# Tejasvanvekar/Sparse-optimal-control-of-Viscous-Chan-hilliard-via-Gradient-descent--1D-2D

Hardware: AMD Instinct MI355X
Metric: PGD iterations/sec (fwd Newton + adjoint + prox), 2D 512^2 grid (higher is better)
Workload: dtype f64; 1 GPU; 2D 512x512, 1000 time steps, batch 8 trajectories per GPU (8 total), seeds 42+i, targets build_targets 1/1, u0 = 0; grid=512, batch_per_gpu=8, contexts_per_gpu=2, parallelism=batch-shard x1, collective=cabi-rccl

## Files before the change

### sparse-optimal-control-of-viscous-chan-hilliard-via-gradient-descent--1d-2d_amd/csrc/vch_engine2d.hip

```cpp
#include "vch_common.h"
#include "vch_kernels2d.h"
#include "vch_gemm.h"
#include "vch_fft.h"
#include <algorithm>
#include <atomic>
#include <chrono>
#include <cmath>

thread_local char g_vch_err[512] = "";

extern "C" const char *vch_last_error(void) { return g_vch_err; }
extern "C" int vch_abi_version(void) { return 3; }
extern "C" int vch_device_count(void) {
    int n = 0;
    if (hipGetDeviceCount(&n) != hipSuccess) return -1;
    return n;
}

constexpr int J_RING = 64;

struct GuessPolicy {
    static constexpr int PROBE_EVERY = 8;
    int order, probe, since, next_dir;
    bool climbing;
    double r_base;
    void reset() { order = 1; probe = 0; since = 0; next_dir = 1; climbing = true; r_base = 1e300; }
    int choose(int avail, int cap) const { return std::max(0, std::min(std::min(order + probe, cap), avail)); }
    void report(double r, int used, int cap) {
        if (used < 1) return;
        if (climbing) {
            if (r > 0.7) {
                order = std::max(1, used - 1);
                r_base = 1e300;
                if (used > 1) climbing = false;
                return;
            }
            if (r_base < 1e299 && r > 0.5 * r_base) {
                order = std::max(1, used - 1);
                climbing = false;
                return;
            }
            r_base = r;
            order = used;
            if (used >= cap) climbing = false;
            else order = used + 1;
            return;
        }
        if (probe == 0) {
            r_base = r;
            if (r > 0.7 && order > 1) { --order; since = 0; return; }
            if (++since >= PROBE_EVERY) {
                since = 0;
                probe = next_dir;
                next_dir = -next_dir;
                if (order + probe < 1 || order + probe > cap) probe = 0;
            }
            return;
        }
        if (probe > 0 ? r < 0.5 * r_base : r <= r_base) order = used;
        probe = 0;
    }
};

struct vch2d_ctx {
    vch2d_params prm;
    int B, Mmax, device;
    Geom G;
    Phys P;
    double hx, hy;
    hipStream_t stream;
    hipEvent_t ev0, ev1;
    dim3 grid;
    int nblk;
    long slot_stride;
    double *phi_s, *mu_s, *Rphi_s, *rhs_s, *D_s;
    double *w, *wnew, *mu0, *cphi, *cmu, *x, *r, *dmu, *t1, *t2;
    double *cg_p[2], *cg_v, *cg_q;
    double *cg_z2;
    double *xf;
    int cg_last;
    bool cheb_on;
    int spec_form[4];
    bool debug_guess;
    bool adj_guess_off, adj_safe;
    long redo_iters;
    bool fused_on;
    int fused_mode;
    unsigned *fin_counter;
    int cheb_enq, spec_chn[4], cheb_margin, cheb_max;
    double pgd_adj_tol;
    double eta1_factor;
    double cg_scale_ratio;
    double *dprev[GUESS_RING], *x0g;
    bool guess_on;
    int guess_wr, guess_step;
    int guess_max;
    std::vector<GuessPolicy> pol1, pol2;
    std::vector<int> used1, used2, run2;
    GuessPolicy pol1_all, pol2_all;
    int run2_all;
    GuessArgs gtab1, gtab2;
    unsigned gmask1, gmask2;
    double *dprev2[GUESS_RING];
    bool guess2_on;
    double *gpart2;
    double *gpart3;
    double *gpart;
    int gnblk;
    double *tmp[6];
    double *wts_mass, *W_cost;
    double *part;
    double *part_mass;
    bool post_fold;
    bool post_pending;
    double *post_hist;
    TrajState *st, *st_host;
    TrajState *st_pub;
    unsigned long long *seq_pub, seq_next;
    bool look_spin;
    int *frozen_dev;
    double *hist_dev, *hist_host;
    double *Q1f, *Q2f, *Q1s, *Q2s, *mf, *ms;
    bool use_fft;
    int cols_c;
    FftAxis fax, sax;
    FftAxis fax_h, sax_h;
    double2 *tw_fh = nullptr, *tw_sh = nullptr;
    bool half_f = false, half_s = false;
    double2 *tw_f, *tw_s;
    double *phi_hist, *u_hist, *u_trial, *phi_trial, *phiQ, *r_hist, *p_hist, *q_hist;
    double *phiT, *phi0;
    double *cost_part, *cost_lvl;
    double *cost_lvl_host;
    double *alpha_dev;
    int M_res;
    int u_rows_res;
    bool pgd_ready;
    bool ramp;
    double rampT;
    std::vector<double> t_hist, dt, xg, yg, tfrac;
    double *tfrac_dev;
    vch_opt_params opt;
    std::vector<double> pgd_cost, pgd_alpha_prev, pgd_J;
    std::vector<int> pgd_plateau, pgd_done, pgd_k;
    std::vector<std::vector<double>> pgd_cost_hist;
    std::vector<double> pgd_denQ2, pgd_denT2, pgd_trk, pgd_trm;
    double pgd_rms;
    int pgd_err_n;
    double *J_dev;
    double *J_ring_dev, *J_ring_host;
    std::atomic<long> pgd_iter_total;
    long tot_launch, tot_sync;
    bool prof_on;
    std::vector<hipEvent_t> prof_ev;
    std::vector<int> prof_cls;
    size_t prof_used;
    int lin_maxit;
    double lin_tol;
    double lin_eta;
    bool spec;
    int spec_slots, spec_cgb[4];
    long n_launch, n_sync;
};

enum { PC_SCHUR_P = 0, PC_GEMM = 1, PC_RESIDUAL = 2, PC_ADJ_Q = 3, PC_CG_UPDATE = 4, PC_ADJ_RHS = 5, PC_COST = 6,
       PC_PROX = 7, PC_DCT_R0 = 8, PC_DCT_C = 9, PC_DCT_R3 = 10, PC_SCHUR_P1 = 11, PC_CG_ROWS = 12, PC_CG_ROWS1 = 13,
       PC_NOOP = 14, PC_GUESS = 15, PC_ADJ_GUESS = 16, PC_CHEB_ROWS = 17, PC_CHEB_ROWS0 = 18, PC_RESIDUAL0 = 19,
       PC_NCLS = 20 };

__global__ void k_noop() {}

static bool launch_begin(vch2d_ctx *c, int cls) {
    const bool rec = cls >= 0 && c->prof_on && c->prof_used + 2 <= c->prof_ev.size();
    if (rec) hipEventRecord(c->prof_ev[c->prof_used], c->stream);
    return rec;
}
static void launch_end(vch2d_ctx *c, int cls, bool rec) {
    c->n_launch++;
    if (rec) {
        hipEventRecord(c->prof_ev[c->prof_used + 1], c->stream);
        c->prof_cls.push_back(cls);
        c->prof_used += 2;
    }
}
#define LAUNCHC(cls, kern, grid, block, ...) LAUNCH_LDS(cls, kern, grid, block, 0, __VA_ARGS__)

static int dalloc(double **p, size_t n, hipStream_t s) {
    *p = nullptr;
    HIPCHK(hipMalloc((void **)p, n * sizeof(double)));
    HIPCHK(hipMemsetAsync(*p, 0, n * sizeof(double), s));
    return 0;
}

static int h2d(vch2d_ctx *c, double *dev, const double *host, long nplanes) {
    HIPCHK(hipMemcpy2DAsync(dev, (size_t)c->G.pitch * 8, host, (size_t)c->G.nf * 8, (size_t)c->G.nf * 8,
                            (size_t)c->G.ns * nplanes, hipMemcpyHostToDevice, c->stream));
    return 0;
}
static int d2h(vch2d_ctx *c, double *host, const double *dev, long nplanes) {
    HIPCHK(hipMemcpy2DAsync(host, (size_t)c->G.nf * 8, dev, (size_t)c->G.pitch * 8, (size_t)c->G.nf * 8,
                            (size_t)c->G.ns * nplanes, hipMemcpyDeviceToHost, c->stream));
    HIPCHK(hipStreamSynchronize(c->stream));
    return 0;
}
static int h2d_hist(vch2d_ctx *c, double *dev, const double *host, int rows) {
    const long hs = (long)(c->Mmax + 1) * c->G.plane;
    for (int b = 0; b < c->B; ++b)
        VCHCHK(h2d(c, dev + b * hs, host + (long)b * rows * c->G.nf * c->G.ns, rows));
    return 0;
}
static int d2h_hist(vch2d_ctx *c, double *host, const double *dev, int rows) {
    const long hs = (long)(c->Mmax + 1) * c->G.plane;
    for (int b = 0; b < c->B; ++b) {
        HIPCHK(hipMemcpy2DAsync(host + (long)b * rows * c->G.nf * c->G.ns, (size_t)c->G.nf * 8, dev + b * hs,
                                (size_t)c->G.pitch * 8, (size_t)c->G.nf * 8, (size_t)c->G.ns * rows,
                                hipMemcpyDeviceToHost, c->stream));
    }
    HIPCHK(hipStreamSynchronize(c->stream));
    return 0;
}
static int ensure_hist(vch2d_ctx *c, double **p) {
    if (*p) return 0;
    size_t n = (size_t)c->B * (c->Mmax + 1) * c->G.plane;
    hipError_t e = hipMalloc((void **)p, n * sizeof(double));
    if (e != hipSuccess) {
        *p = nullptr;
        return vch_fail(VCH_ERR_NOMEM, "hipMalloc of a %.2f GB history failed: %s", n * 8e-9, hipGetErrorString(e));
    }
    HIPCHK(hipMemsetAsync(*p, 0, n * sizeof(double), c->stream));
    return 0;
}
static inline long hist_stride(const vch2d_ctx *c) { return (long)(c->Mmax + 1) * c->G.plane; }

__global__ void k_publish_state(const unsigned *__restrict__ st, int nwords, unsigned *__restrict__ dst,
                                unsigned long long *seq, unsigned long long val) {
    for (int i = threadIdx.x; i < nwords; i += blockDim.x) dst[i] = st[i];
    __threadfence_system();
    __syncthreads();
    if (threadIdx.x == 0) __hip_atomic_store(seq, val, __ATOMIC_RELEASE, __HIP_MEMORY_SCOPE_SYSTEM);
}

static int sync_state(vch2d_ctx *c, bool full = true) {
    c->n_sync++;
    if (full || !c->look_spin) {
        HIPCHK(hipMemcpyAsync(c->st_host, c->st, sizeof(TrajState) * c->B, hipMemcpyDeviceToHost, c->stream));
        HIPCHK(hipStreamSynchronize(c->stream));
        return 0;
    }
    const unsigned long long want = ++c->seq_next;
    static_assert(sizeof(TrajState) % 4 == 0, "TrajState is copied in 32-bit words");
    hipLaunchKernelGGL(k_publish_state, dim3(1), dim3(256), 0, c->stream, (const unsigned *)c->st,
                       (int)(sizeof(TrajState) / 4 * c->B), (unsigned *)c->st_pub, c->seq_pub, want);
    HIPCHK(hipGetLastError());
    const auto t0 = std::chrono::steady_clock::now();
    for (unsigned spins = 1; __atomic_load_n(c->seq_pub, __ATOMIC_ACQUIRE) != want; ++spins) {
        __builtin_ia32_pause();
        if ((spins & 0x3fff) == 0) {
            const hipError_t q = hipStreamQuery(c->stream);
            if (q != hipSuccess && q != hipErrorNotReady) return vch_fail(VCH_ERR_HIP, "sync_state: %s", hipGetErrorString(q));
            if (q == hipSuccess && __atomic_load_n(c->seq_pub, __ATOMIC_ACQUIRE) != want)
                return vch_fail(VCH_ERR_STATE, "sync_state: stream drained but the state was not published");
            if (std::chrono::steady_clock::now() - t0 > std::chrono::seconds(120))
                return vch_fail(VCH_ERR_STATE, "sync_state: no state from the device after 120 s");
        }
    }
    memcpy(c->st_host, c->st_pub, sizeof(TrajState) * c->B);
    return 0;
}

static void dct_tables(int N, double h, std::vector<double> &Q1, std::vector<double> &Q2, std::vector<double> &m) {
    const int n = N + 1;
    Q1.assign((size_t)n * n, 0.0);
    Q2.assign((size_t)n * n, 0.0);
    m.assign(n, 0.0);
    const long double pi = 3.14159265358979323846264338327950288L;
    const long double sc = sqrtl(2.0L / N), is2 = 1.0L / sqrtl(2.0L);
    for (int j = 0; j < n; ++j) {
        long double sj = (j == 0 || j == N) ? is2 : 1.0L;
        for (int k = 0; k < n; ++k) {
            long double sk = (k == 0 || k == N) ? is2 : 1.0L;
            long long jk = ((long long)j * k) % (2LL * N);
            long double cv = cosl(pi * (long double)jk / (long double)N);
            Q1[(size_t)j * n + k] = (double)(sc * sj * sj * sk * cv);
            Q2[(size_t)j * n + k] = (double)(sc * sj * cv);
        }
        m[j] = (double)((2.0L - 2.0L * cosl(pi * j / (long double)N)) / ((long double)h * h));
    }
}

extern "C" vch2d_ctx *vch2d_create(const vch2d_params *p, int batch, int max_steps, int device) {
    if (!p || p->Nx < 2 || p->Ny < 2 || batch < 1 || max_steps < 1 || !(p->Lx > 0) || !(p->Ly > 0)) {
        vch_fail(VCH_ERR_ARG, "vch2d_create: bad arguments (Nx,Ny >= 2, batch >= 1, max_steps >= 1)");
        return nullptr;
    }
    if (hipSetDevice(device) != hipSuccess) {
        (void)hipGetLastError();
        vch_fail(VCH_ERR_HIP, "hipSetDevice(%d) failed", device);
        return nullptr;
    }
    vch2d_ctx *c = new vch2d_ctx();
    c->prm = *p;
    c->B = batch;
    c->Mmax = max_steps;
    c->device = device;
    c->hx = p->Lx / p->Nx;
    c->hy = p->Ly / p->Ny;
    Geom &G = c->G;
    G.nf = p->Nx + 1;
    G.ns = p->Ny + 1;
    G.pitch = (G.nf + 7) / 8 * 8;
    G.plane = (long)G.ns * G.pitch;
    G.tiles_f = (G.nf + TX - 1) / TX;
    G.tiles_s = (G.ns + TY - 1) / TY;
    G.ax = 1.0 / (c->hx * c->hx);
    G.ay = 1.0 / (c->hy * c->hy);
    c->P = Phys{p->tau, p->gamma, p->c1, p->c2, p->kappa, p->Lx * p->Ly};
    c->grid = dim3(G.tiles_f, G.tiles_s, batch);
    c->nblk = G.tiles_f * G.tiles_s;
    c->slot_stride = (long)batch * G.plane;
    c->M_res = -1;
    c->u_rows_res = 0;
    c->pgd_ready = false;
    c->prof_on = false;
    c->prof_used = 0;
    c->lin_maxit = 4000;
    c->lin_tol = 1e-15;
    if (const char *e = getenv("VCH_LIN_TOL")) c->lin_tol = atof(e);
    c->lin_eta = 0.05 * NEWTON_TOL;
    if (const char *e = getenv("VCH_LIN_ETA")) c->lin_eta = atof(e);
    c->cols_c = 1024;
    if (const char *e = getenv("VCH_COLS_C")) c->cols_c = atoi(e);
    c->spec = getenv("VCH_NO_SPEC") == nullptr;
    c->spec_slots = 2;
    for (int &n : c->spec_cgb) n = 12;
    c->cheb_on = !(getenv("VCH_CHEB") && atoi(getenv("VCH_CHEB")) == 0);
    for (int &f : c->spec_form) f = 3;
    c->debug_guess = getenv("VCH_DEBUG_GUESS") != nullptr;
    c->adj_guess_off = c->adj_safe = false;
    c->redo_iters = 0;
    c->cheb_enq = -1;
    c->fused_mode = getenv("VCH_FUSED") ? atoi(getenv("VCH_FUSED")) : 2;
    c->fused_on = c->fused_mode != 0;
    c->post_fold = true;
    if (const char *e = getenv("VCH_POST_FOLD")) c->post_fold = atoi(e) != 0;
    c->post_pending = false;
    c->post_hist = nullptr;
    c->fin_counter = nullptr;
    for (int &n : c->spec_chn) n = 2;
    c->cheb_margin = 1;
    if (const char *e = getenv("VCH_CHEB_MARGIN")) c->cheb_margin = std::max(0, atoi(e));
    c->cheb_max = 6;
    if (const char *e = getenv("VCH_CHEB_MAX")) c->cheb_max = std::max(0, atoi(e));
    c->pgd_adj_tol = 1e-12;
    if (const char *e = getenv("VCH_ADJ_TOL")) c->pgd_adj_tol = atof(e);
    c->eta1_factor = 1e-2;
    if (const char *e = getenv("VCH_ETA1")) c->eta1_factor = atof(e);
    c->cg_scale_ratio = 4.0;
    if (const char *e = getenv("VCH_CG_SCALE")) c->cg_scale_ratio = atof(e);
    c->n_launch = c->n_sync = 0;
    auto fail = [&](const char *what) {
        vch_fail(VCH_ERR_HIP, "vch2d_create: %s failed: %s", what, hipGetErrorString(hipGetLastError()));
        return (vch2d_ctx *)nullptr;
    };
    if (hipStreamCreate(&c->stream) != hipSuccess) return fail("hipStreamCreate");
    hipEventCreate(&c->ev0);
    hipEventCreate(&c->ev1);
    const size_t bp = (size_t)batch * G.plane;
    double **two[] = {&c->phi_s, &c->mu_s, &c->Rphi_s, &c->rhs_s, &c->D_s};
    for (auto q : two)
        if (dalloc(q, 2 * bp, c->stream)) return fail("hipMalloc");
    double **one[] = {&c->w, &c->wnew, &c->mu0, &c->cphi, &c->cmu, &c->x, &c->r, &c->dmu, &c->t1, &c->t2,
                      &c->cg_p[0], &c->cg_p[1], &c->cg_v, &c->cg_q, &c->cg_z2, &c->xf, &c->dprev[0], &c->dprev[1], &c->dprev[2], &c->dprev[3], &c->dprev[4], &c->dprev[5], &c->dprev[6], &c->dprev[7], &c->dprev2[0], &c->dprev2[1], &c->dprev2[2], &c->dprev2[3], &c->dprev2[4], &c->dprev2[5], &c->dprev2[6], &c->dprev2[7], &c->x0g, &c->tmp[0], &c->tmp[1], &c->tmp[2], &c->tmp[3], &c->tmp[4], &c->tmp[5], &c->phiT, &c->phi0};
    for (auto q : one)
        if (dalloc(q, bp, c->stream)) return fail("hipMalloc");
    if (dalloc(&c->wts_mass, G.plane, c->stream) || dalloc(&c->W_cost, G.plane, c->stream)) return fail("hipMalloc");
    if (dalloc(&c->part, (size_t)batch * c->nblk * NPART, c->stream)) return fail("hipMalloc");
    if (dalloc(&c->part_mass, (size_t)batch * c->nblk * NPART, c->stream)) return fail("hipMalloc");
    c->gnblk = ((G.nf + GN - 1) / GN) * ((G.ns + GM - 1) / GM);
    if (dalloc(&c->gpart, 2 * (size_t)batch * (c->gnblk + G.ns), c->stream)) return fail("hipMalloc");
    c->gpart2 = c->gpart + (size_t)batch * (c->gnblk + G.ns);
    if (dalloc(&c->gpart3, 4 * (size_t)batch * (c->gnblk + G.ns), c->stream)) return fail("hipMalloc");
    if (dalloc(&c->hist_dev, (size_t)batch * HIST_CAP, c->stream)) return fail("hipMalloc");
    if (dalloc(&c->alpha_dev, batch, c->stream) || dalloc(&c->J_dev, 5 * (size_t)batch, c->stream)) return fail("hipMalloc");
    if (dalloc(&c->J_ring_dev, (size_t)J_RING * 5 * batch, c->stream)) return fail("hipMalloc");
    if (hipHostMalloc((void **)&c->J_ring_host, sizeof(double) * J_RING * 5 * batch) != hipSuccess) return fail("hipHostMalloc");
    c->pgd_iter_total = 0;
    c->tot_launch = c->tot_sync = 0;
    if (hipMalloc((void **)&c->st, sizeof(TrajState) * batch) != hipSuccess) return fail("hipMalloc");
    hipMemsetAsync(c->st, 0, sizeof(TrajState) * batch, c->stream);
    if (hipMalloc((void **)&c->frozen_dev, sizeof(int) * batch) != hipSuccess) return fail("hipMalloc");
    if (hipMalloc((void **)&c->fin_counter, sizeof(unsigned) * batch) != hipSuccess) return fail("hipMalloc");
    hipMemsetAsync(c->fin_counter, 0, sizeof(unsigned) * batch, c->stream);
    if (hipHostMalloc((void **)&c->st_host, sizeof(TrajState) * batch) != hipSuccess) return fail("hipHostMalloc");
    c->st_pub = nullptr;
    c->seq_pub = nullptr;
    c->seq_next = 0;
    c->look_spin = !(getenv("VCH_LOOK_SPIN") && atoi(getenv("VCH_LOOK_SPIN")) == 0);
    if (c->look_spin) {
        if (hipHostMalloc((void **)&c->st_pub, sizeof(TrajState) * batch, hipHostMallocMapped | hipHostMallocCoherent) != hipSuccess ||
            hipHostMalloc((void **)&c->seq_pub, 64, hipHostMallocMapped | hipHostMallocCoherent) != hipSuccess) {
            (void)hipGetLastError();
            if (c->st_pub) hipHostFree(c->st_pub);
            c->st_pub = nullptr;
            c->seq_pub = nullptr;
            c->look_spin = false;
        } else {
            *c->seq_pub = 0;
        }
    }
    if (hipHostMalloc((void **)&c->hist_host, sizeof(double) * batch * HIST_CAP) != hipSuccess) return fail("hipHostMalloc");
    c->phi_hist = c->u_hist = c->u_trial = c->phi_trial = c->phiQ = c->r_hist = c->p_hist = c->q_hist = nullptr;
    c->cost_part = c->cost_lvl = nullptr;
    c->cost_lvl_host = nullptr;
    c->tfrac_dev = nullptr;
    {
        std::vector<double> wm((size_t)G.plane, 0.0);
        const int nx1 = p->Nx + 1, ny1 = p->Ny + 1;
        for (int i = 0; i < nx1; ++i)
            for (int j = 0; j < ny1; ++j) {
                long f = (long)i * ny1 + j;
                double wi = (i == 0 || i == nx1 - 1) ? 0.5 : 1.0, wj = (j == 0 || j == ny1 - 1) ? 0.5 : 1.0;
                wm[(f / G.nf) * G.pitch + (f % G.nf)] = c->hx * c->hy * (wi * wj);
            }
        if (hipMemcpy(c->wts_mass, wm.data(), wm.size() * 8, hipMemcpyHostToDevice) != hipSuccess) return fail("hipMemcpy");
    }
    {
        std::vector<double> Q1, Q2, m;
        auto up = [&](double **d, const std::vector<double> &v) {
            if (hipMalloc((void **)d, v.size() * 8) != hipSuccess) return false;
            return hipMemcpy(*d, v.data(), v.size() * 8, hipMemcpyHostToDevice) == hipSuccess;
        };
        dct_tables(p->Nx, c->hx, Q1, Q2, m);
        if (!up(&c->Q1f, Q1) || !up(&c->Q2f, Q2) || !up(&c->mf, m)) return fail("DCT table upload");
        dct_tables(p->Ny, c->hy, Q1, Q2, m);
        if (!up(&c->Q1s, Q1) || !up(&c->Q2s, Q2) || !up(&c->ms, m)) return fail("DCT table upload");
    }
    {
        auto pow2 = [](int n) { return n >= 16 && n <= 2048 && (n & (n - 1)) == 0; };
        c->use_fft = pow2(p->Nx) && pow2(p->Ny) && getenv("VCH_FORCE_GEMM_DCT") == nullptr;
        c->tw_f = c->tw_s = nullptr;
        if (c->use_fft) {
            auto mk = [&](int N, double2 **tw, FftAxis &ax) {
                const int L = 2 * N;
                std::vector<double2> t(L);
                const long double pi = 3.14159265358979323846264338327950288L;
                for (int m = 0; m < L; ++m) {
                    long double a = -2.0L * pi * m / L;
                    t[m] = make_double2((double)cosl(a), (double)sinl(a));
                }
                if (hipMalloc((void **)tw, sizeof(double2) * L) != hipSuccess) return false;
                if (hipMemcpy(*tw, t.data(), sizeof(double2) * L, hipMemcpyHostToDevice) != hipSuccess) return false;
                int lg = 0;
                while ((1 << lg) < L) ++lg;
                ax = FftAxis{N, L, lg, *tw};
                return true;
            };
            if (!mk(p->Nx, &c->tw_f, c->fax) || !mk(p->Ny, &c->tw_s, c->sax)) return fail("FFT twiddle upload");
            const bool want_half = getenv("VCH_DCT_HALF") != nullptr;
            if (want_half && p->Nx == HN) {
                if (!mk(HN / 2, &c->tw_fh, c->fax_h)) return fail("FFT twiddle upload");
                c->half_f = true;
            }
            if (want_half && p->Ny == HN) {
                if (!mk(HN / 2, &c->tw_sh, c->sax_h)) return fail("FFT twiddle upload");
                c->half_s = true;
            }
            if (c->half_f) {
                c->gnblk = (G.ns + 3) / 4;
            } else {
                const int Cc = c->fax.L <= 1024 ? 1024 : c->fax.L;
                const int rpw = 2 * (Cc >> c->fax.logL);
                c->gnblk = (G.ns + rpw - 1) / rpw;
            }
        }
    }
    c->guess_on = c->use_fft && !c->half_f && !c->half_s && !(getenv("VCH_GUESS") && atoi(getenv("VCH_GUESS")) == 0);
    memset(&c->gtab1, 0, sizeof(c->gtab1));
    memset(&c->gtab2, 0, sizeof(c->gtab2));
    c->gmask1 = c->gmask2 = 0;
    c->pol1.resize(batch);
    c->pol2.resize(batch);
    c->used1.assign(batch, 0);
    c->used2.assign(batch, 0);
    c->run2.assign(batch, 0);
    c->run2_all = 0;
    c->guess2_on = !(getenv("VCH_GUESS2") && atoi(getenv("VCH_GUESS2")) == 0);
    c->guess_wr = -1;
    c->guess_step = 0;
    c->guess_max = 6;
    if (const char *e = getenv("VCH_GUESS_MAX")) c->guess_max = std::max(1, std::min(GUESS_ORD, atoi(e)));
    if (hipStreamSynchronize(c->stream) != hipSuccess) return fail("hipStreamSynchronize");
    return c;
}

extern "C" void vch2d_destroy(vch2d_ctx *c) {
    if (!c) return;
    hipSetDevice(c->device);
    hipStreamSynchronize(c->stream);
    double *all[] = {c->phi_s, c->mu_s, c->Rphi_s, c->rhs_s, c->D_s, c->w, c->wnew, c->mu0, c->cphi, c->cmu, c->x,
                     c->r, c->dmu, c->t1, c->t2, c->cg_p[0], c->cg_p[1], c->cg_v, c->cg_q, c->cg_z2, c->xf, c->dprev[0], c->dprev[1], c->dprev[2], c->dprev[3], c->dprev[4], c->dprev[5], c->dprev[6], c->dprev[7], c->dprev2[0], c->dprev2[1], c->dprev2[2], c->dprev2[3], c->dprev2[4], c->dprev2[5], c->dprev2[6], c->dprev2[7], c->x0g, c->gpart, c->gpart3, c->tmp[0], c->tmp[1], c->tmp[2], c->tmp[3], c->tmp[4], c->tmp[5],
                     c->phiT, c->phi0, c->wts_mass, c->W_cost, c->part, c->part_mass, c->hist_dev, c->alpha_dev, c->J_dev, c->Q1f,
                     c->Q2f, c->Q1s, c->Q2s, c->mf, c->ms, c->phi_hist, c->u_hist, c->u_trial, c->phi_trial, c->phiQ,
                     c->r_hist, c->p_hist, c->q_hist, c->cost_part, c->cost_lvl, c->tfrac_dev};
    for (double *q : all)
        if (q) hipFree(q);
    hipFree(c->st);
    hipFree(c->frozen_dev);
    if (c->fin_counter) hipFree(c->fin_counter);
    if (c->tw_fh) hipFree(c->tw_fh);
    if (c->tw_sh) hipFree(c->tw_sh);
    if (c->tw_f) hipFree(c->tw_f);
    if (c->tw_s) hipFree(c->tw_s);
    hipHostFree(c->st_host);
    if (c->st_pub) hipHostFree(c->st_pub);
    if (c->seq_pub) hipHostFree(c->seq_pub);
    hipHostFree(c->hist_host);
    hipHostFree(c->J_ring_host);
    hipFree(c->J_ring_dev);
    if (c->cost_lvl_host) hipHostFree(c->cost_lvl_host);
    for (hipEvent_t e : c->prof_ev) hipEventDestroy(e);
    hipEventDestroy(c->ev0);
    hipEventDestroy(c->ev1);
    hipStreamDestroy(c->stream);
    delete c;
}

extern "C" int vch2d_batch(const vch2d_ctx *c) { return c ? c->B : VCH_ERR_ARG; }

template <class F>
static int with_plan(const FftAxis &ax, F &&f) {
    using std::integral_constant;
    if (ax.logL == 10) return f(integral_constant<int, 1024>(), integral_constant<int, 10>());
    if (ax.logL == 9) return f(integral_constant<int, 1024>(), integral_constant<int, 9>());
    if (ax.logL < 10) return f(integral_constant<int, 1024>(), integral_constant<int, 0>());
    if (ax.logL == 11) return f(integral_constant<int, 2048>(), integral_constant<int, 11>());
    return f(integral_constant<int, 4096>(), integral_constant<int, 0>());
}

template <int EPI>
static int dct_rows(vch2d_ctx *c, const double *in, long in_slot_stride, double *out, const SpecArgs &sp, int gate) {
    return with_plan(c->fax, [&](auto C, auto LG) {
        const int rpw = 2 * (C >> c->fax.logL);
        LAUNCHC(EPI >= 3 ? PC_DCT_R3 : PC_DCT_R0, (k_dct_rows<EPI, C, LG>), dim3((c->G.ns + rpw - 1) / rpw, 1, c->B),
                dim3(FftThreads<C, LG>::T), c->G, c->fax, in, in_slot_stride, out, 1.0, sp, c->st, gate);
        return 0;
    });
}

template <int C, int LOGL>
static int dct_cols_plan(vch2d_ctx *c, const SpecArgs &sp, double scale, int gate) {
    const int cpw = 2 * (C >> c->sax.logL);
    LAUNCHC(PC_DCT_C, (k_dct_cols<C, LOGL>), dim3((c->G.nf + cpw - 1) / cpw, 1, c->B), dim3(FftThreads<C, LOGL>::T), c->G,
            c->sax, (const double *)c->t1, c->t2, scale, sp, c->st, gate);
    return 0;
}
static int dct_cols(vch2d_ctx *c, const SpecArgs &sp, double scale, int gate) {
    const int wide = c->sax.logL == 10 ? c->cols_c : 0;
    if (wide == 4096) return dct_cols_plan<4096, 10>(c, sp, scale, gate);
    if (wide == 2048) return dct_cols_plan<2048, 10>(c, sp, scale, gate);
    return with_plan(c->sax, [&](auto C, auto LG) { return dct_cols_plan<C, LG>(c, sp, scale, gate); });
}

static int cg_rows(vch2d_ctx *c, const CgSweepArgs &a, bool first) {
    return with_plan(c->fax, [&](auto C, auto LG) {
        const int rpw = 2 * (C >> c->fax.logL);
        auto k_rows = first ? k_cg_rows_fwd<1, C, LG> : k_cg_rows_fwd<0, C, LG>;
        LAUNCHC(first ? PC_CG_ROWS1 : PC_CG_ROWS, k_rows, dim3((c->G.ns + rpw - 1) / rpw, 1, c->B), dim3(FftThreads<C, LG>::T),
                c->G, c->fax, a, c->t1, c->st);
        return 0;
    });
}

static int cheb_rows(vch2d_ctx *c, const ChebSweepArgs &a, bool first) {
    return with_plan(c->fax, [&](auto C, auto LG) {
        const int rpw = 2 * (C >> c->fax.logL);
        auto k_rows = first ? k_cheb_rows<C, LG, 1> : k_cheb_rows<C, LG, 0>;
        LAUNCHC(first ? PC_CHEB_ROWS0 : PC_CHEB_ROWS, k_rows, dim3((c->G.ns + rpw - 1) / rpw, 1, c->B), dim3(FftThreads<C, LG>::T),
                c->G, c->fax, a, (const double *)c->t2, c->t1, (const TrajState *)c->st);
        return 0;
    });
}

static int adj_rows(vch2d_ctx *c, const AdjSweepArgs &a, bool first) {
    return with_plan(c->fax, [&](auto C, auto LG) {
        const int rpw = 2 * (C >> c->fax.logL);
        auto k_rows = first ? k_adj_rows_fwd<1, C, LG> : k_adj_rows_fwd<0, C, LG>;
        LAUNCHC(PC_ADJ_Q, k_rows, dim3((c->G.ns + rpw - 1) / rpw, 1, c->B), dim3(FftThreads<C, LG>::T), c->G, c->fax, a, c->t1,
                c->st);
        return 0;
    });
}

static int precond(vch2d_ctx *c, const double *in, long in_slot_stride, double *out, int last, const double *other,
                   double c0, double c1a, double c1b, double c2, int gate) {
    const Geom &G = c->G;
// ... 1445 lines not shown
```

### sparse-optimal-control-of-viscous-chan-hilliard-via-gradient-descent--1d-2d_amd/csrc/vch_fft.h

```cpp
#pragma once
#include "vch_common.h"
#include "vch_kernels2d.h"
#include "vch_gemm.h"

struct FftAxis {
    int N, L, logL;
    const double2 *tw;
};


__device__ __forceinline__ double2 cmul(double2 a, double2 b) {
    return make_double2(a.x * b.x - a.y * b.y, a.x * b.y + a.y * b.x);
}

struct SpecArgs;
template <class SP>
__device__ __forceinline__ void spec_mult2(const SP &sp, double c1, double scale, double ma, double mb, double &fa, double &fb,
                                           int mode) {
    const double pa = sp.c0 + ma * (c1 + sp.c2 * ma), pb = sp.c0 + mb * (c1 + sp.c2 * mb);
    const double na = scale * (mode == 2 ? -(sp.c0 + sp.c2 * ma * ma) : (mode ? ma : 1.0));
    const double nb = scale * (mode == 2 ? -(sp.c0 + sp.c2 * mb * mb) : (mode ? mb : 1.0));
    const double d = pa * pb;
    double r = __builtin_amdgcn_rcp(d);
    r = fma(fma(-d, r, 1.0), r, r);
// ... 76 lines not shown
            for (int h = 0; h < 2; ++h) {
                const double2 *v = h ? cc : bb;
                const double2 t0 = make_double2(v[0].x + v[2].x, v[0].y + v[2].y), t1 = make_double2(v[0].x - v[2].x, v[0].y - v[2].y);
                const double2 t2 = make_double2(v[1].x + v[3].x, v[1].y + v[3].y);
                const double2 t3 = make_double2(v[1].y - v[3].y, -(v[1].x - v[3].x));
                o[h + 0] = make_double2(t0.x + t2.x, t0.y + t2.y);
                o[h + 2] = make_double2(t1.x + t3.x, t1.y + t3.y);
                o[h + 4] = make_double2(t0.x - t2.x, t0.y - t2.y);
                o[h + 6] = make_double2(t1.x - t3.x, t1.y - t3.y);
            }
            const int wb = fb + ((j >> lNs) << (lNs + 3)) + k;
            if (REGMODE == 1 && 3 * (ps + 1) == LOGL) {
#pragma unroll
                for (int r = 0; r < 8; ++r) xr[r] = o[r];
            } else if (EMIT && 3 * (ps + 1) == LOGL) {
                if (Emit::TO_LDS) __syncthreads();
#pragma unroll
                for (int r = 0; r < 8; ++r) emit(wb + r * Ns, o[r]);
                if (Emit::TO_LDS) __syncthreads();
            } else {
                if (!(INGEST && ps == 0)) __syncthreads();
#pragma unroll
                for (int r = 0; r < 8; ++r) buf[swz<LOGL>(wb + r * Ns)] = o[r];
                __syncthreads();
            }
        }
        logNs = 3 * NR8;
    }
    const int logQ = logL - 2, Q = L >> 2;
#pragma unroll
    for (; logNs + 2 <= logL; logNs += 2) {
        const int Ns = 1 << logNs;
        double2 v[NB4][4];
        int wbase[NB4];
        const bool shared_tw = Ns <= T;
        double2 w1 = make_double2(1.0, 0.0), w2 = w1, w3 = w1;
        if (logNs > 0 && shared_tw) {
            const int ti = (tid & (Ns - 1)) << (logL - logNs - 2);
            w1 = ax.tw[ti];
            w2 = ax.tw[2 * ti];
            w3 = ax.tw[3 * ti];
        }
#pragma unroll
        for (int i = 0; i < NB4; ++i) {
            const int idx = tid + i * T;
            const int f = idx >> logQ, j = idx & (Q - 1), k = j & (Ns - 1);
            const int fb = f * L;
            double2 a = buf[swz<LOGL>(fb + j)], b = buf[swz<LOGL>(fb + j + Q)], c = buf[swz<LOGL>(fb + j + 2 * Q)],
                    d = buf[swz<LOGL>(fb + j + 3 * Q)];
            if (logNs > 0) {
                if (!shared_tw) {
                    const int ti = k << (logL - logNs - 2);
                    w1 = ax.tw[ti];
                    w2 = ax.tw[2 * ti];
                    w3 = ax.tw[3 * ti];
                }
                b = cmul(b, w1);
                c = cmul(c, w2);
                d = cmul(d, w3);
            }
            double2 t0 = make_double2(a.x + c.x, a.y + c.y), t1 = make_double2(a.x - c.x, a.y - c.y);
            double2 t2 = make_double2(b.x + d.x, b.y + d.y);
            double2 t3 = make_double2(b.y - d.y, -(b.x - d.x));
            v[i][0] = make_double2(t0.x + t2.x, t0.y + t2.y);
            v[i][1] = make_double2(t1.x + t3.x, t1.y + t3.y);
            v[i][2] = make_double2(t0.x - t2.x, t0.y - t2.y);
            v[i][3] = make_double2(t1.x - t3.x, t1.y - t3.y);
            wbase[i] = f * L + ((j >> logNs) << (logNs + 2)) + k;
        }
        if (REGMODE == 1 && logNs + 2 == logL) {
            static_assert(REGMODE != 1 || LOGL == 9 || NB4 == 2, "two radix-4 butterflies per thread");
#pragma unroll
            for (int i = 0; i < NB4; ++i)
#pragma unroll
                for (int r = 0; r < 4; ++r) xr[(i + 2 * r) & 7] = v[i][r];
        } else if (EMIT && logNs + 2 == logL) {
            if (Emit::TO_LDS) __syncthreads();
#pragma unroll
            for (int i = 0; i < NB4; ++i)
#pragma unroll
                for (int r = 0; r < 4; ++r) emit(wbase[i] + r * Ns, v[i][r]);
            if (Emit::TO_LDS) __syncthreads();
        } else {
            __syncthreads();
#pragma unroll
            for (int i = 0; i < NB4; ++i)
#pragma unroll
                for (int r = 0; r < 4; ++r) buf[swz<LOGL>(wbase[i] + r * Ns)] = v[i][r];
            __syncthreads();
        }
    }
    if (logNs < logL) {
        const int Ns = 1 << logNs, H = L >> 1, logH = logL - 1;
        double2 v[NB2][2];
        int wbase[NB2];
#pragma unroll
        for (int i = 0; i < NB2; ++i) {
            const int idx = tid + i * T;
            const int f = idx >> logH, j = idx & (H - 1), k = j & (Ns - 1);
            const int fb = f * L;
            double2 a = buf[swz<LOGL>(fb + j)], b = cmul(buf[swz<LOGL>(fb + j + H)], ax.tw[k << (logL - logNs - 1)]);
            v[i][0] = make_double2(a.x + b.x, a.y + b.y);
            v[i][1] = make_double2(a.x - b.x, a.y - b.y);
            wbase[i] = f * L + ((j >> logNs) << (logNs + 1)) + k;
        }
        __syncthreads();
#pragma unroll
        for (int i = 0; i < NB2; ++i) {
            buf[swz<LOGL>(wbase[i])] = v[i][0];
            buf[swz<LOGL>(wbase[i] + Ns)] = v[i][1];
        }
        __syncthreads();
    }
}

template <int EPI, int C, int LOGL>
__global__ __launch_bounds__((FftThreads<C, LOGL>::T)) void k_dct_rows(Geom G, FftAxis ax, const double *__restrict__ in,
                                                  long in_slot_stride, double *__restrict__ out, double scale,
                                                  SpecArgs sp, const TrajState *__restrict__ st, int gate) {
    const int b = blockIdx.z;
    if (gate && !gate_open(st[b], gate)) return;
    __shared__ double2 buf[C];
    constexpr int T = FftThreads<C, LOGL>::T;
    const int tid = threadIdx.x;
    const int logL = LOGL ? LOGL : ax.logL, L = 1 << logL, N = L >> 1, nfft = C >> logL;
    const int row0 = blockIdx.x * 2 * nfft;
    const double *ib = in + b * G.plane + (in_slot_stride ? st[b].slot * in_slot_stride : 0);
    const int n1 = N + 1;
    const float inv_n1 = 1.0f / (float)n1;
    constexpr bool DIRECT = LOGL >= 9 && LOGL <= 11;
    if (!DIRECT) {
        for (int idx = tid; idx < nfft * n1; idx += T) {
            const int f = nfft == 1 ? 0 : (int)(((float)idx + 0.5f) * inv_n1), j = idx - f * n1;
            const int ra = row0 + 2 * f, rb = ra + 1;
            double2 v = make_double2(ra < G.ns ? ib[(long)ra * G.pitch + j] : 0.0,
                                     rb < G.ns ? ib[(long)rb * G.pitch + j] : 0.0);
            buf[swz<LOGL>(f * L + j)] = v;
            if (j > 0 && j < N) buf[swz<LOGL>(f * L + L - j)] = v;
        }
        __syncthreads();
    }
    double dot = 0.0, dot2 = 0.0, dbar = 0.0;
    const double *Dp = nullptr, *Ob = nullptr;
    int scaled = 0;
    if (EPI >= 3) {
        dbar = st[b].dbar;
        scaled = (EPI != 5) ? st[b].scaled : 0;
        Dp = sp.Dslot + st[b].slot * sp.d_slot_stride + b * G.plane;
        Ob = sp.other ? sp.other + b * G.plane : nullptr;
    }
    double *ob = out + b * G.plane;
    auto put = [&](int row, int k, double e) {
        double v = scale * e;
        const long o = (long)row * G.pitch + k;
        if (EPI == 4) v += Ob[o];
        if (EPI == 5) {
            const double dl = Dp[o] - dbar, pv = Ob[o];
            v = pv + sp.epi_c * dl * v;
            ob[o] = v;
            const double wd = wdev(row, k, G) / dl;
            dot += wd * (pv * v);
            dot2 += wd * (v * v);
            return;
        }
        ob[o] = v;
        if (EPI >= 3) {
            const double wd = wdev(row, k, G) * cg_weight(Dp[o], dbar, scaled);
            dot += wd * ((Ob ? Ob[o] : v) * v);
            dot2 += wd * (v * v);
        }
    };
    if (DIRECT) {
        struct RowEmit {
            enum { ACTIVE = 1, TO_LDS = 0 };
            decltype(put) &put_;
            int row0_, ns_;
            __device__ __forceinline__ void operator()(int idx, double2 v) const {
                constexpr int LL = 1 << (LOGL ? LOGL : 1);
                const int f = idx >> (LOGL ? LOGL : 1), k = idx & (LL - 1);
                if (k <= LL / 2) {
                    const int ra = row0_ + 2 * f;
                    if (ra < ns_) put_(ra, k, v.x);
                    if (ra + 1 < ns_) put_(ra + 1, k, v.y);
                }
            }
        };
        struct RowIngest {
            enum { ACTIVE = 1 };
            const double *ib_;
            long pitch_;
            int row0_, ns_;
            __device__ __forceinline__ double2 operator()(int idx) const {
                constexpr int LL = 1 << (LOGL ? LOGL : 1);
                const int f = idx >> (LOGL ? LOGL : 1), i = idx & (LL - 1), m = i <= LL / 2 ? i : LL - i;
                const int ra = row0_ + 2 * f;
                const double *p = ib_ + (long)ra * pitch_ + m;
                return make_double2(ra < ns_ ? p[0] : 0.0, ra + 1 < ns_ ? p[pitch_] : 0.0);
            }
        };
        fft_lds<C, LOGL>(buf, ax, RowEmit{put, row0, G.ns}, RowIngest{ib, (long)G.pitch, row0, G.ns});
    } else {
        fft_lds<C, LOGL>(buf, ax);
        for (int idx = tid; idx < 2 * nfft * n1; idx += T) {
            const int rr = nfft == 1 ? (idx >= n1 ? 1 : 0) : (int)(((float)idx + 0.5f) * inv_n1), k = idx - rr * n1;
            const int row = row0 + rr;
            if (row < G.ns) {
                const double2 c = buf[swz<LOGL>((rr >> 1) * L + k)];
                put(row, k, (rr & 1) ? c.y : c.x);
            }
        }
    }
    if (EPI >= 3) {
        dot = wave_sum(dot);
        dot2 = wave_sum(dot2);
        __syncthreads();
        double *sred = reinterpret_cast<double *>(buf);
        if ((tid & 63) == 0) {
            sred[tid >> 6] = dot;
            sred[T / 64 + (tid >> 6)] = dot2;
        }
        __syncthreads();
        if (tid == 0) {
            double tot = 0.0, tot2 = 0.0;
            for (int w = 0; w < T / 64; ++w) {
                tot += sred[w];
                tot2 += sred[T / 64 + w];
            }
            sp.gpart[(long)b * gridDim.x + blockIdx.x] = tot;
            sp.gpart2[(long)b * gridDim.x + blockIdx.x] = tot2;
        }
    }
}

struct CgSweepArgs {
    const double *z, *q, *p_old;
    double *x, *z_new, *p_new;
    const double *Dslot;
    long d_slot_stride;
    const double *gpart, *gpart2;
    double *gpart3;
    int it, maxit, nbatch;
    const double *x0;
};

template <int T>
__device__ __forceinline__ void cg_sums3(const double *__restrict__ g1, const double *__restrict__ g2,
                                         const double *__restrict__ g3, int n, int b, double *s3) {
    const int wv = threadIdx.x >> 6, lane = threadIdx.x & 63;
    for (int k = wv; k < 3; k += T / 64) {
        const double *src = k == 0 ? g1 : (k == 1 ? g2 : g3);
        double a = 0.0;
        if (src)
            for (int t = lane; t < n; t += 64) a += src[(long)b * n + t];
        a = wave_sum(a);
        if (lane == 0) s3[k] = a;
    }
    __syncthreads();
}

struct FinSolveArgs {
    const double *gpart, *gpart2, *gpart3_rd;
    int gnblk, direct, rd, maxit;
    const double *p_last;
    int cheb_enq;
};
__global__ __launch_bounds__(NTH) void k_dmu_ceiling_fin(Geom G, Phys P, TrajState *__restrict__ st, long slot_stride,
                                                         const double *__restrict__ x, FinSolveArgs f,
                                                         const double *__restrict__ phi_s, const double *__restrict__ D_s,
                                                         const double *__restrict__ Rphi_s, double *__restrict__ dmu,
                                                         double *__restrict__ x_out, double *__restrict__ part,
                                                         double *__restrict__ x_keep, double *__restrict__ x_keep2) {
    TILE_COORDS;
    if (!st[b].newton_active || st[b].need_trial) return;
    if (st[b].use_cheb) return;
    __shared__ double sx[(TY + 2) * (TX + 2)];
    __shared__ double sred[NPART * 4];
    __shared__ double s3[3];
    double *const keepp = st[b].iters == 1 ? x_keep : (st[b].iters == 2 ? x_keep2 : nullptr);
    const bool keep = keepp != nullptr;
    constexpr int W = TX + 2;
    const long pb = b * G.plane;
    const int slot = st[b].slot;
    double alpha = 0.0;
    if (f.cheb_enq >= 0) {
        if (st[b].lin_active && st[b].cheb_n > f.cheb_enq) return;
    } else if (st[b].lin_active) {
        if (!st[b].ci_active[f.rd]) {
            if (blk == 0 && threadIdx.x == 0) st[b].ci_active[f.rd ^ 1] = 0;
        } else {
            const double gamma0 = st[b].cg_gamma0, gamma_old = st[b].ci_gamma[f.rd], tol = st[b].lin_reltol;
            const int it_old = st[b].ci_it[f.rd];
            cg_sums3<NTH>(f.gpart, f.gpart2, f.direct ? f.gpart3_rd : nullptr, f.gnblk, b, s3);
            const CgNext n = cg_next(s3[0], s3[1], f.direct ? s3[2] : gamma_old, gamma0, it_old, tol, f.maxit);
            if (blk == 0 && threadIdx.x == 0) cg_record(st[b], n, f.rd ^ 1);
            alpha = n.breakdown ? 0.0 : n.alpha;
        }
    }
    if (alpha != 0.0) load_tile_axpy<1>(sx, x + pb, f.p_last + pb, alpha, G, c0, r0);
    else load_tile<1>(sx, x + pb, G, c0, r0);
    if (st[b].scaled) {
        __syncthreads();
        const double dbar = st[b].dbar;
        const double *Dp = D_s + slot * slot_stride + pb;
        for (int e = threadIdx.x; e < W * (TY + 2); e += NTH) {
            int ly = e / W, lxx = e - ly * W;
            int gr = refl(r0 - 1 + ly, G.ns), gc = refl(c0 - 1 + lxx, G.nf);
            sx[e] *= dbar / Dp[(long)gr * G.pitch + gc];
        }
    }
    __syncthreads();
    double acc[1] = {1e300};
    for (int k = 0; k < TY / 4; ++k) {
        int ly = ly0 + 4 * k, r = r0 + ly, c = c0 + lx;
        if (r < G.ns && c < G.nf) {
            int p = (ly + 1) * W + lx + 1;
            long o = pb + (long)r * G.pitch + c, os = slot * slot_stride + o;
            double d = sx[p];
            x_out[o] = d;
            if (keep) keepp[o] = d;
            dmu[o] = 2.0 * ((-0.5 * P.kappa * lap_at<W>(sx, p, G.ax, G.ay) + D_s[os] * d) + Rphi_s[os]);
            double ph = phi_s[os];
            if (d > 0.0) acc[0] = fmin(acc[0], (1.0 - DELTA_SEP - ph) / d);
            else if (d < 0.0) acc[0] = fmin(acc[0], (-1.0 + DELTA_SEP - ph) / d);
        }
    }
    const int op[1] = {1};
    block_reduce_store<1>(acc, op, sred, part + ((long)b * nblk + blk) * NPART);
}

template <int FIRST, int C, int LOGL>
__global__ __launch_bounds__((FftThreads<C, LOGL>::T)) void k_cg_rows_fwd(Geom G, FftAxis ax, CgSweepArgs a, double *__restrict__ out,
                                                                         TrajState *__restrict__ st) {
    const int b = blockIdx.z;
    __shared__ double2 buf[C];
    __shared__ double s3[4];
    constexpr int T = FftThreads<C, LOGL>::T;
    const int tid = threadIdx.x;
    const int logL = LOGL ? LOGL : ax.logL, L = 1 << logL, N = L >> 1, nfft = C >> logL;
    const int row0 = blockIdx.x * 2 * nfft, n1 = N + 1;
    const int rd = (a.it + 1) & 1, wr = a.it & 1;
    const long pb = b * G.plane;
    double alpha = 0.0, beta = 0.0;
    if (FIRST) {
        const int active = st[b].lin_active && !st[b].use_cheb;
        if (blockIdx.x == 0 && tid < 64) {
            double g = 0.0;
            if (active)
                for (int t = tid; t < (int)gridDim.x; t += 64) g += a.gpart[(long)b * gridDim.x + t];
            g = wave_sum(g);
            if (tid == 0) {
                TrajState &S = st[b];
                S.cg_pending = 0;
                if (!active) {
                    S.ci_active[0] = 0;
                } else {
                    S.cg_gamma = S.cg_gamma0 = g;
                    S.cg_beta = 0.0;
                    S.lin_it = 0;
                    S.lin_rel = 1.0;
                    S.ci_active[0] = 1;
                    S.ci_it[0] = 0;
                    S.ci_gamma[0] = g;
                }
            }
        }
        if (!active) return;
    } else {
        if (!st[b].ci_active[rd]) {
            if (blockIdx.x == 0 && tid == 0) {
                st[b].ci_active[wr] = 0;
                st[b].ci_it[wr] = st[b].ci_it[rd];
                st[b].ci_gamma[wr] = st[b].ci_gamma[rd];
            }
            return;
        }
        const double gamma0 = st[b].cg_gamma0, gamma_old = st[b].ci_gamma[rd], tol = st[b].lin_reltol;
        const int it_old = st[b].ci_it[rd], n = gridDim.x;
        cg_sums3<T>(a.gpart, a.gpart2, a.it >= 2 ? a.gpart3 + (long)rd * a.nbatch * n : nullptr, n, b, s3);
        const CgNext nx = cg_next(s3[0], s3[1], a.it >= 2 ? s3[2] : gamma_old, gamma0, it_old, tol, a.maxit);
        if (blockIdx.x == 0 && tid == 0) cg_record(st[b], nx, wr);
        alpha = nx.alpha;
        beta = nx.beta;
        if (!nx.active) {
            if (!nx.breakdown)
                for (int idx = tid; idx < 2 * nfft * n1; idx += T) {
                    const int rr = idx / n1, k = idx - rr * n1, row = row0 + rr;
                    if (row < G.ns) {
                        const long o = pb + (long)row * G.pitch + k;
                        a.x[o] += alpha * a.p_old[o];
                    }
                }
            return;
        }
    }
    const double dbar = st[b].dbar;
    const int scaled = st[b].scaled;
    const double *Dp = a.Dslot + st[b].slot * a.d_slot_stride + pb;
    const bool primed = FIRST && a.x0 && st[b].x_primed;
    double acc = 0.0;
    auto node = [&](int row, int m, bool owner) -> double {
        if (row >= G.ns) return 0.0;
        const long o = (long)row * G.pitch + m;
        const double dl = cg_weight(Dp[o], dbar, scaled);
        double pn;
        if (FIRST) {
            pn = a.z[pb + o];
            if (owner) {
                a.x[pb + o] = primed ? (scaled ? a.x0[pb + o] * (Dp[o] / dbar) : a.x0[pb + o]) : 0.0;
                a.p_new[pb + o] = pn;
            }
        } else {
            const double po = a.p_old[pb + o];
            const double zn = a.z[pb + o] - alpha * a.q[pb + o];
            pn = zn + beta * po;
            if (owner) {
                a.x[pb + o] += alpha * po;
                a.z_new[pb + o] = zn;
                a.p_new[pb + o] = pn;
                acc += wdev(row, m, G) * dl * (zn * zn);
            }
        }
        return dl * pn;
    };
    double *ob = out + pb;
    auto put = [&](int row, int k, double e) { ob[(long)row * G.pitch + k] = e; };
    constexpr bool DIRECT = LOGL >= 9 && LOGL <= 11;
    if (DIRECT) {
        struct Emit {
            enum { ACTIVE = 1, TO_LDS = 0 };
            decltype(put) &put_;
            int row0_, ns_;
            __device__ __forceinline__ void operator()(int idx, double2 v) const {
                constexpr int LL = 1 << (LOGL ? LOGL : 1);
                const int f = idx >> (LOGL ? LOGL : 1), k = idx & (LL - 1);
                if (k <= LL / 2) {
                    const int ra = row0_ + 2 * f;
                    if (ra < ns_) put_(ra, k, v.x);
                    if (ra + 1 < ns_) put_(ra + 1, k, v.y);
                }
            }
        };
        for (int idx = tid; idx < nfft * n1; idx += T) {
            const int f = nfft == 1 ? 0 : idx / n1, j = idx - f * n1;
            const int ra = row0 + 2 * f;
            const double2 v = make_double2(node(ra, j, true), node(ra + 1, j, true));
            buf[swz<LOGL>(f * L + j)] = v;
            if (j > 0 && j < N) buf[swz<LOGL>(f * L + L - j)] = v;
        }
        __syncthreads();
        fft_lds<C, LOGL>(buf, ax, Emit{put, row0, G.ns});
    } else {
        const float inv_n1 = 1.0f / (float)n1;
        for (int idx = tid; idx < nfft * n1; idx += T) {
            const int f = nfft == 1 ? 0 : (int)(((float)idx + 0.5f) * inv_n1), j = idx - f * n1;
            const int ra = row0 + 2 * f;
            const double2 v = make_double2(node(ra, j, true), node(ra + 1, j, true));
            buf[swz<LOGL>(f * L + j)] = v;
            if (j > 0 && j < N) buf[swz<LOGL>(f * L + L - j)] = v;
        }
        __syncthreads();
        fft_lds<C, LOGL>(buf, ax);
        for (int idx = tid; idx < 2 * nfft * n1; idx += T) {
            const int rr = nfft == 1 ? (idx >= n1 ? 1 : 0) : (int)(((float)idx + 0.5f) * inv_n1), k = idx - rr * n1;
            const int row = row0 + rr;
            if (row < G.ns) {
                const double2 c = buf[swz<LOGL>((rr >> 1) * L + k)];
                put(row, k, (rr & 1) ? c.y : c.x);
            }
        }
    }
    if (!FIRST) {
        acc = wave_sum(acc);
        __syncthreads();
        double *sred = reinterpret_cast<double *>(buf);
        if ((tid & 63) == 0) sred[tid >> 6] = acc;
        __syncthreads();
        if (tid == 0) {
            double tot = 0.0;
            for (int w = 0; w < T / 64; ++w) tot += sred[w];
            a.gpart3[((long)wr * a.nbatch + b) * gridDim.x + blockIdx.x] = tot;
        }
    }
}

struct ChebSweepArgs {
    const double *bt_in;
    double *bt_out;
    const double *y_cur, *y_prev;
    double *y_new;
    double *x_out;
    const double *x0;
    const double *Dslot;
    long d_slot_stride;
    double *gpart;
    int j;
    double scale;
    const double *phi_s;
    double *cmin;
    double *keep1, *keep2;
};

#ifndef CHEB_MINW
#define CHEB_MINW 1
#endif
template <int C, int LOGL, int FIRST>
__global__ __launch_bounds__((FftThreads<C, LOGL>::T), CHEB_MINW) void k_cheb_rows(Geom G, FftAxis ax, ChebSweepArgs a_, const double *__restrict__ in,
                                                                       double *__restrict__ out, const TrajState *__restrict__ st) {
    const int b = blockIdx.z;
    ChebSweepArgs a = a_;
    if (FIRST) a.j = 0;
    if (!st[b].lin_active || !st[b].use_cheb || a.j > st[b].cheb_n) return;
    const bool last = a.j == st[b].cheb_n;
    __shared__ double2 buf[C];
    constexpr int T = FftThreads<C, LOGL>::T;
    const int tid = threadIdx.x;
    const int logL = LOGL ? LOGL : ax.logL, L = 1 << logL, N = L >> 1, nfft = C >> logL;
    const int row0 = blockIdx.x * 2 * nfft, n1 = N + 1;
    const long pb = b * G.plane;
    const double theta = st[b].cheb_theta, delta = st[b].cheb_delta;
    double cj = 0.0, ej = 1.0 / theta;
    {
        double rho_prev = delta / theta;
        for (int i = 1; i <= a.j; ++i) {
            ej = 2.0 / (2.0 * theta - delta * rho_prev);
            const double rho = 0.5 * delta * ej;
            cj = rho * rho_prev;
            rho_prev = rho;
        }
    }
    const double dbar = st[b].dbar;
    const double *Dp = a.Dslot + st[b].slot * a.d_slot_stride + pb;
    const bool primed = a.x0 && st[b].x_primed;
    const bool need_norm = !(last && a.j == 0);
    double acc = 0.0, cmin = 1e300;
    const double *php = a.phi_s + st[b].slot * a.d_slot_stride + pb;
    double *const keepp = st[b].iters == 1 ? a.keep1 : (st[b].iters == 2 ? a.keep2 : nullptr);
    auto upd = [&](int row, int k, double g) -> double {
        const long o = (long)row * G.pitch + k;
        const double gg = a.scale * g;
        double z, yn, dl = 0.0;
        if (need_norm || !last) dl = Dp[o] - dbar;
        if (a.j == 0) {
            z = gg;
            yn = ej * z;
            if (!last) a.bt_out[pb + o] = gg;
        } else {
            const double yc = a.y_cur[pb + o], yp = a.j >= 2 ? a.y_prev[pb + o] : 0.0;
            z = a.bt_in[pb + o] - yc - gg;
            yn = yc + cj * (yc - yp) + ej * z;
        }
        if (need_norm) acc += wdev(row, k, G) * dl * (z * z);
        if (last) {
            const double d = primed ? a.x0[pb + o] + yn : yn, ph = php[o];
            a.x_out[pb + o] = d;
            if (keepp) keepp[pb + o] = d;
            if (d > 0.0) cmin = fmin(cmin, (1.0 - DELTA_SEP - ph) / d);
            else if (d < 0.0) cmin = fmin(cmin, (-1.0 + DELTA_SEP - ph) / d);
        } else {
            a.y_new[pb + o] = yn;
        }
        return dl * yn;
    };
    const double *ib = in + pb;
    double *ob = out + pb;
    auto put = [&](int row, int k, double e) { ob[(long)row * G.pitch + k] = e; };
    constexpr bool DIRECT = LOGL >= 9 && LOGL <= 11;
    if (DIRECT) {
        constexpr int LL = 1 << (LOGL ? LOGL : 1), LG = LOGL ? LOGL : 1;
        struct RowIngest {
            enum { ACTIVE = 1 };
            const double *ib_;
            long pitch_;
            int row0_, ns_;
            __device__ __forceinline__ double2 operator()(int idx) const {
                const int f = idx >> LG, i = idx & (LL - 1), m = i <= LL / 2 ? i : LL - i;
                const int ra = row0_ + 2 * f;
                const double *p = ib_ + (long)ra * pitch_ + m;
                return make_double2(ra < ns_ ? p[0] : 0.0, ra + 1 < ns_ ? p[pitch_] : 0.0);
            }
        };
        struct UpdEmit {
            enum { ACTIVE = 1, TO_LDS = 1 };
            decltype(upd) &upd_;
            double2 *buf_;
            int row0_, ns_;
            bool last_;
            __device__ __forceinline__ void operator()(int idx, double2 v) const {
                const int f = idx >> LG, k = idx & (LL - 1);
                if (k > LL / 2) return;
                const int ra = row0_ + 2 * f;
                double2 w = make_double2(0.0, 0.0);
                if (ra < ns_) w.x = upd_(ra, k, v.x);
                if (ra + 1 < ns_) w.y = upd_(ra + 1, k, v.y);
                if (!last_) {
                    buf_[swz<LOGL>(idx)] = w;
                    if (k > 0 && k < LL / 2) buf_[swz<LOGL>(f * LL + LL - k)] = w;
                }
            }
        };
        struct RowEmit {
            enum { ACTIVE = 1, TO_LDS = 0 };
            decltype(put) &put_;
            int row0_, ns_;
            __device__ __forceinline__ void operator()(int idx, double2 v) const {
                const int f = idx >> LG, k = idx & (LL - 1);
                if (k <= LL / 2) {
                    const int ra = row0_ + 2 * f;
                    if (ra < ns_) put_(ra, k, v.x);
                    if (ra + 1 < ns_) put_(ra + 1, k, v.y);
                }
            }
// ... 665 lines not shown
```

### sparse-optimal-control-of-viscous-chan-hilliard-via-gradient-descent--1d-2d_amd/csrc/vch_kernels2d.h

```cpp
#pragma once
#include "vch_common.h"

struct TrajState {
    int slot;
    int newton_active;
    int need_trial;
    int trial_no;
    int force_accept;
    int iters;
    int nsolves;
    int ntrials;
    int stuck;
    int frozen;
    double normR;
    double alpha;
    double best_norm, best_alpha;
    double Dmin, Dmax, dbar;
    double rho;
    double kT;
    long newton_total;
    int lin_active, lin_it;
    long lin_total;
    double lin_r0, lin_prev, lin_rel, lin_maxrel;
    double cg_gamma, cg_gamma0, cg_alpha, cg_beta;
    int lin_budget;
    double lin_reltol, lin_maxabs;
    int x_primed, guess_pad;
    double lin_rscale;
    double guess_ratio;
    double guess_ratio2;
    int step_solves, step_lin_max;
    int step_lin[4];
    double step_tol[4], step_kT[4];
    int step_chn[4];
    int cheb_n;
    int use_cheb;
    double cheb_theta, cheb_delta;
    int step_form[4];
    int scaled, scaled_pad;
    double step_R[4];
    double R1_hist[3];
    int lin_took, lin_unconv;
    int cg_pending, cg_pbuf, cg_pad;
    int ci_active[2], ci_it[2];
    double ci_gamma[2];
    double mass0, mass_err, Wint;
    double aux[4];
};

__device__ __forceinline__ bool gate_open(const TrajState &S, int gate) {
    if (gate >= 16) return S.lin_active != 0 && S.use_cheb != 0 && gate - 16 <= S.cheb_n;
    if (gate == 5) return S.lin_active != 0 && S.use_cheb == 0;
    if (gate == 8) return S.lin_active != 0 && S.use_cheb != 0;
    return gate == 1 ? S.lin_active != 0 : (gate == 4 ? S.lin_took != 0 : S.ci_active[gate - 2] != 0);
}

struct Phys {
    double tau, gamma, c1, c2, kappa;
    double LxLy;
};

__device__ __forceinline__ int refl(int i, int n) {
    i = i < 0 ? -i : i;
    i = i >= n ? 2 * (n - 1) - i : i;
    return i < 0 ? 0 : i;
}

template <int H>
__device__ __forceinline__ void load_tile(double *s, const double *__restrict__ g, const Geom &G,
                                          int c0, int r0) {
    constexpr int W = TX + 2 * H, HT = TY + 2 * H;
    for (int e = threadIdx.x; e < W * HT; e += NTH) {
        int ly = e / W, lx = e - ly * W;
        int gr = refl(r0 - H + ly, G.ns), gc = refl(c0 - H + lx, G.nf);
        s[e] = g[(long)gr * G.pitch + gc];
    }
}

template <int H>
__device__ __forceinline__ void load_tile_axpy(double *s, const double *__restrict__ a,
                                               const double *__restrict__ d, double alpha,
                                               const Geom &G, int c0, int r0) {
    constexpr int W = TX + 2 * H, HT = TY + 2 * H;
    for (int e = threadIdx.x; e < W * HT; e += NTH) {
        int ly = e / W, lx = e - ly * W;
        int gr = refl(r0 - H + ly, G.ns), gc = refl(c0 - H + lx, G.nf);
        long o = (long)gr * G.pitch + gc;
        s[e] = a[o] + alpha * d[o];
    }
}

template <int W>
__device__ __forceinline__ double lap_at(const double *s, int p, double ax, double ay) {
    double c = s[p];
    return ax * ((s[p - 1] + s[p + 1]) - 2.0 * c) + ay * ((s[p - W] + s[p + W]) - 2.0 * c);
}

__device__ __forceinline__ double reglog(double phi) {
    const double eps = 0.5 * DELTA_SEP;
    double p = fmin(fmax(phi, -1.0 + eps), 1.0 - eps);
    return log((1.0 + p) / (1.0 - p));
}

__device__ __forceinline__ double jac_diag(double phi, double tau_dt, double c1) {
    double psq = fmin(fmax(phi * phi, 0.0), 1.0 - DELTA_SEP * DELTA_SEP);
    return tau_dt + 2.0 * c1 / (1.0 - psq);
}

__device__ __forceinline__ double fpp_log(double phi, double c1, double c2) {
    double p = fmin(fmax(phi, -1.0 + 1e-8), 1.0 - 1e-8);
    return 2.0 * c1 / (1.0 - p * p) - 2.0 * c2;
}

__device__ __forceinline__ double wdev(int r, int c, const Geom &G) {
    return ((r == 0 || r == G.ns - 1) ? 0.5 : 1.0) * ((c == 0 || c == G.nf - 1) ? 0.5 : 1.0);
}

__device__ __forceinline__ double wave_sum(double v) {
    for (int o = 32; o > 0; o >>= 1) v += __shfl_down(v, o, 64);
    return v;
}
__device__ __forceinline__ double wave_min(double v) {
    for (int o = 32; o > 0; o >>= 1) v = fmin(v, __shfl_down(v, o, 64));
    return v;
}
__device__ __forceinline__ double wave_max(double v) {
    for (int o = 32; o > 0; o >>= 1) v = fmax(v, __shfl_down(v, o, 64));
    return v;
}

template <int N>
__device__ __forceinline__ void block_reduce_store(double (&v)[N], const int (&op)[N], double *sred,
                                                   double *part) {
    int lane = threadIdx.x & 63, wv = threadIdx.x >> 6;
#pragma unroll
    for (int k = 0; k < N; ++k) {
        double r = op[k] == 0 ? wave_sum(v[k]) : (op[k] == 1 ? wave_min(v[k]) : wave_max(v[k]));
        if (lane == 0) sred[k * 4 + wv] = r;
    }
    __syncthreads();
    if (threadIdx.x == 0) {
#pragma unroll
        for (int k = 0; k < N; ++k) {
            double a = sred[k * 4], b = sred[k * 4 + 1], c = sred[k * 4 + 2], d = sred[k * 4 + 3];
            part[k] = op[k] == 0 ? (a + b) + (c + d)
                                 : (op[k] == 1 ? fmin(fmin(a, b), fmin(c, d)) : fmax(fmax(a, b), fmax(c, d)));
        }
    }
}

__device__ __forceinline__ int xcd_remap(int bid, int n) {
    const int q = n >> 3, r = n & 7, xcd = bid & 7, idx = bid >> 3;
    return (xcd < r ? xcd * (q + 1) : r * (q + 1) + (xcd - r) * q) + idx;
}

#define TILE_COORDS                                   \
    const int b = blockIdx.z;                         \
    const int nblk = gridDim.x * gridDim.y;           \
    const int blk = xcd_remap(blockIdx.y * gridDim.x + blockIdx.x, nblk); \
    const int c0 = (blk / (int)gridDim.y) * TX, r0 = (blk % (int)gridDim.y) * TY; \
    const int lx = threadIdx.x & 63, ly0 = threadIdx.x >> 6; \
    (void)blk; (void)nblk; (void)lx; (void)ly0

__global__ __launch_bounds__(NTH) void k_lap(Geom G, const double *__restrict__ v, double *__restrict__ out) {
    TILE_COORDS;
    __shared__ double s[(TY + 2) * (TX + 2)];
    constexpr int W = TX + 2;
    load_tile<1>(s, v + b * G.plane, G, c0, r0);
    __syncthreads();
    for (int k = 0; k < TY / 4; ++k) {
        int ly = ly0 + 4 * k, r = r0 + ly, c = c0 + lx;
        if (r < G.ns && c < G.nf)
            out[b * G.plane + (long)r * G.pitch + c] = lap_at<W>(s, (ly + 1) * W + lx + 1, G.ax, G.ay);
    }
}

__global__ __launch_bounds__(NTH) void k_init_mu(Geom G, Phys P, const double *__restrict__ phi,
                                                 const double *__restrict__ w, double *__restrict__ mu) {
    TILE_COORDS;
    __shared__ double s[(TY + 2) * (TX + 2)];
    constexpr int W = TX + 2;
    load_tile<1>(s, phi + b * G.plane, G, c0, r0);
    __syncthreads();
    for (int k = 0; k < TY / 4; ++k) {
        int ly = ly0 + 4 * k, r = r0 + ly, c = c0 + lx;
        if (r < G.ns && c < G.nf) {
            int p = (ly + 1) * W + lx + 1;
            long o = b * G.plane + (long)r * G.pitch + c;
            double ph = s[p];
            mu[o] = -P.kappa * lap_at<W>(s, p, G.ax, G.ay) + (P.c1 * reglog(ph) - 2.0 * P.c2 * ph) - w[o];
        }
    }
}

__device__ __forceinline__ void newton_begin(TrajState &S) {
    if (S.frozen) {
        S.newton_active = S.need_trial = S.lin_active = 0;
        return;
    }
    S.newton_active = 1;
    S.need_trial = 1;
    S.trial_no = 0;
    S.force_accept = 1;
    S.iters = 0;
    S.stuck = 0;
    S.alpha = 0.0;
    S.lin_active = 0;
    S.step_solves = 0;
    S.step_lin_max = 0;
    S.step_lin[0] = S.step_lin[1] = S.step_lin[2] = S.step_lin[3] = 0;
    S.step_chn[0] = S.step_chn[1] = S.step_chn[2] = S.step_chn[3] = 0;
    S.step_form[0] = S.step_form[1] = S.step_form[2] = S.step_form[3] = 0;
    S.use_cheb = 0;
    S.scaled = 0;
    S.x_primed = 0;
    S.lin_rscale = 1.0;
    S.guess_ratio = 1.0;
    S.guess_ratio2 = 0.0;
}

__global__ __launch_bounds__(NTH) void k_prepare(Geom G, Phys P, TrajState *__restrict__ st,
                                                 long slot_stride, const double *__restrict__ phi_s,
                                                 const double *__restrict__ mu_s, const double *__restrict__ w,
                                                 const double *__restrict__ un, const double *__restrict__ unp1,
                                                 long u_stride, const double *__restrict__ wnew_in, double dt,
                                                 double *__restrict__ wnew,
                                                 double *__restrict__ mu0, double *__restrict__ cphi,
                                                 double *__restrict__ cmu) {
    TILE_COORDS;
    __shared__ double sp[(TY + 2) * (TX + 2)];
    __shared__ double sm[(TY + 2) * (TX + 2)];
    constexpr int W = TX + 2;
    if (blk == 0 && threadIdx.x == 0) newton_begin(st[b]);
    if (st[b].frozen) return;
    const int slot = st[b].slot;
    load_tile<1>(sp, phi_s + slot * slot_stride + b * G.plane, G, c0, r0);
    load_tile<1>(sm, mu_s + slot * slot_stride + b * G.plane, G, c0, r0);
    __syncthreads();
    const double gdt = P.gamma / dt;
    for (int k = 0; k < TY / 4; ++k) {
        int ly = ly0 + 4 * k, r = r0 + ly, c = c0 + lx;
        if (r < G.ns && c < G.nf) {
            int p = (ly + 1) * W + lx + 1;
            long o = (long)r * G.pitch + c;
            long ob = b * G.plane + o;
            double u0 = un ? un[b * u_stride + o] : 0.0, u1 = unp1 ? unp1[b * u_stride + o] : 0.0;
            double wo = w[ob];
            double wn = wnew_in ? wnew_in[ob] : ((gdt - 0.5) * wo + 0.5 * (u1 + u0)) / (gdt + 0.5);
            double ph = sp[p], lp = lap_at<W>(sp, p, G.ax, G.ay), lm = lap_at<W>(sm, p, G.ax, G.ay);
            wnew[ob] = wn;
            mu0[ob] = -P.kappa * lp + (P.c1 * reglog(ph) - 2.0 * P.c2 * ph) - wn;
            cphi[ob] = -(P.tau / dt) * ph - 0.5 * P.kappa * lp - 2.0 * P.c2 * ph - 0.5 * sm[p] - 0.5 * (wn + wo);
            cmu[ob] = -ph / dt - 0.5 * lm;
        }
    }
}

template <int MODE>
__global__ __launch_bounds__(NTH) void k_residual(Geom G, Phys P, const TrajState *__restrict__ st,
                                                  long slot_stride, double *__restrict__ phi_s,
                                                  double *__restrict__ mu_s, double *__restrict__ Rphi_s,
                                                  double *__restrict__ rhs_s, double *__restrict__ D_s,
                                                  const double *__restrict__ mu0, const double *__restrict__ dphi,
                                                  const double *__restrict__ dmu, const double *__restrict__ cphi,
                                                  const double *__restrict__ cmu, double dt,
                                                  double *__restrict__ part) {
    TILE_COORDS;
    const TrajState S = st[b];
    if (!S.newton_active || !S.need_trial) return;
    __shared__ double sp[(TY + 4) * (TX + 4)];
    __shared__ double sm[(TY + 2) * (TX + 2)];
    __shared__ double sr[(TY + 2) * (TX + 2)];
    __shared__ double sred[NPART * 4];
    constexpr int W2 = TX + 4, W1 = TX + 2;
    const long pb = b * G.plane;
    const int src = S.slot, dst = MODE == 0 ? S.slot : 1 - S.slot;
    if (MODE == 0) {
        load_tile<2>(sp, phi_s + src * slot_stride + pb, G, c0, r0);
        load_tile<1>(sm, mu0 + pb, G, c0, r0);
    } else {
        load_tile_axpy<2>(sp, phi_s + src * slot_stride + pb, dphi + pb, S.alpha, G, c0, r0);
        load_tile_axpy<1>(sm, mu_s + src * slot_stride + pb, dmu + pb, S.alpha, G, c0, r0);
    }
    __syncthreads();
    const double tdt = P.tau / dt;
    for (int e = threadIdx.x; e < (TY + 2) * W1; e += NTH) {
        int ly = e / W1, lxx = e - ly * W1;
        int gr = refl(r0 - 1 + ly, G.ns), gc = refl(c0 - 1 + lxx, G.nf);
        int p2 = (ly + 1) * W2 + lxx + 1;
        double ph = sp[p2];
        sr[e] = tdt * ph - 0.5 * P.kappa * lap_at<W2>(sp, p2, G.ax, G.ay) + P.c1 * reglog(ph) - 0.5 * sm[e] +
                cphi[pb + (long)gr * G.pitch + gc];
    }
    __syncthreads();
    double acc[4] = {0.0, 0.0, 1e300, -1e300};
    for (int k = 0; k < TY / 4; ++k) {
        int ly = ly0 + 4 * k, r = r0 + ly, c = c0 + lx;
        if (r < G.ns && c < G.nf) {
            int p1 = (ly + 1) * W1 + lx + 1, p2 = (ly + 2) * W2 + lx + 2;
            long o = pb + (long)r * G.pitch + c;
            double ph = sp[p2], rp = sr[p1];
            double rm = ph / dt - 0.5 * lap_at<W1>(sm, p1, G.ax, G.ay) + cmu[o];
            double rh = -rm + lap_at<W1>(sr, p1, G.ax, G.ay);
            double d = jac_diag(ph, tdt, P.c1);
            long od = dst * slot_stride + o;
            if (MODE == 1) phi_s[od] = ph;
            mu_s[od] = sm[p1];
            Rphi_s[od] = rp;
            rhs_s[od] = rh;
            D_s[od] = d;
            acc[0] += rp * rp + rm * rm;
            acc[1] += rh * rh;
            acc[2] = fmin(acc[2], d);
            acc[3] = fmax(acc[3], d);
        }
    }
    const int op[4] = {0, 0, 1, 2};
    block_reduce_store<4>(acc, op, sred, part + ((long)b * nblk + blk) * NPART);
}

__global__ __launch_bounds__(NTH) void k_residual2(Geom G, Phys P, const TrajState *__restrict__ st, long slot_stride,
                                                   double *__restrict__ phi_s, double *__restrict__ mu_s,
                                                   double *__restrict__ Rphi_s, double *__restrict__ rhs_s,
                                                   double *__restrict__ D_s, const double *__restrict__ dphi,
                                                   const double *__restrict__ cphi, const double *__restrict__ cmu, double dt,
                                                   double *__restrict__ part) {
    TILE_COORDS;
    const TrajState S = st[b];
    if (!S.newton_active || !S.need_trial) return;
    __shared__ double sp[(TY + 4) * (TX + 4)];
    __shared__ double sd[(TY + 4) * (TX + 4)];
    __shared__ double sm[(TY + 2) * (TX + 2)];
    __shared__ double sred[NPART * 4];
    constexpr int W2 = TX + 4, W1 = TX + 2;
    const long pb = b * G.plane;
    const int src = S.slot, dst = 1 - S.slot;
    const double *phi_o = phi_s + src * slot_stride + pb, *mu_o = mu_s + src * slot_stride + pb;
    const double *D_o = D_s + src * slot_stride + pb, *R_o = Rphi_s + src * slot_stride + pb;
    for (int e = threadIdx.x; e < W2 * (TY + 4); e += NTH) {
        int ly = e / W2, lxx = e - ly * W2;
        int gr = refl(r0 - 2 + ly, G.ns), gc = refl(c0 - 2 + lxx, G.nf);
        long o = (long)gr * G.pitch + gc;
        const double d = dphi[pb + o];
        sd[e] = d;
        sp[e] = phi_o[o] + S.alpha * d;
    }
    __syncthreads();
    for (int e = threadIdx.x; e < (TY + 2) * W1; e += NTH) {
        int ly = e / W1, lxx = e - ly * W1;
        int gr = refl(r0 - 1 + ly, G.ns), gc = refl(c0 - 1 + lxx, G.nf);
        int p2 = (ly + 1) * W2 + lxx + 1;
        long o = (long)gr * G.pitch + gc;
        const double dm = 2.0 * ((-0.5 * P.kappa * lap_at<W2>(sd, p2, G.ax, G.ay) + D_o[o] * sd[p2]) + R_o[o]);
        sm[e] = mu_o[o] + S.alpha * dm;
    }
    __syncthreads();
    const double tdt = P.tau / dt;
    double rm[TY / 4], mt[TY / 4];
    for (int k = 0; k < TY / 4; ++k) {
        int ly = ly0 + 4 * k, r = r0 + ly, c = c0 + lx;
        rm[k] = mt[k] = 0.0;
        if (r < G.ns && c < G.nf) {
            int p1 = (ly + 1) * W1 + lx + 1, p2 = (ly + 2) * W2 + lx + 2;
            rm[k] = sp[p2] / dt - 0.5 * lap_at<W1>(sm, p1, G.ax, G.ay) + cmu[pb + (long)r * G.pitch + c];
            mt[k] = sm[p1];
        }
    }
    __syncthreads();
    for (int e = threadIdx.x; e < (TY + 2) * W1; e += NTH) {
        int ly = e / W1, lxx = e - ly * W1;
        int gr = refl(r0 - 1 + ly, G.ns), gc = refl(c0 - 1 + lxx, G.nf);
        int p2 = (ly + 1) * W2 + lxx + 1;
        double ph = sp[p2];
        sm[e] = tdt * ph - 0.5 * P.kappa * lap_at<W2>(sp, p2, G.ax, G.ay) + P.c1 * reglog(ph) - 0.5 * sm[e] +
                cphi[pb + (long)gr * G.pitch + gc];
    }
    __syncthreads();
    double acc[4] = {0.0, 0.0, 1e300, -1e300};
    for (int k = 0; k < TY / 4; ++k) {
        int ly = ly0 + 4 * k, r = r0 + ly, c = c0 + lx;
        if (r < G.ns && c < G.nf) {
            int p1 = (ly + 1) * W1 + lx + 1, p2 = (ly + 2) * W2 + lx + 2;
            long od = dst * slot_stride + pb + (long)r * G.pitch + c;
            double ph = sp[p2], rp = sm[p1];
            double rh = -rm[k] + lap_at<W1>(sm, p1, G.ax, G.ay);
            double d = jac_diag(ph, tdt, P.c1);
            phi_s[od] = ph;
            mu_s[od] = mt[k];
            Rphi_s[od] = rp;
            rhs_s[od] = rh;
            D_s[od] = d;
            acc[0] += rp * rp + rm[k] * rm[k];
            acc[1] += rh * rh;
            acc[2] = fmin(acc[2], d);
            acc[3] = fmax(acc[3], d);
        }
    }
    const int op[4] = {0, 0, 1, 2};
    block_reduce_store<4>(acc, op, sred, part + ((long)b * nblk + blk) * NPART);
}

__global__ __launch_bounds__(NTH) void k_schur(Geom G, Phys P, const TrajState *__restrict__ st,
                                               long slot_stride, const double *__restrict__ x,
                                               const double *__restrict__ D_s, double dt, double *__restrict__ out) {
    TILE_COORDS;
    const int slot = st ? st[b].slot : 0;
    __shared__ double sx[(TY + 4) * (TX + 4)];
    __shared__ double stt[(TY + 2) * (TX + 2)];
    constexpr int W2 = TX + 4, W1 = TX + 2;
    const long pb = b * G.plane;
    load_tile<2>(sx, x + pb, G, c0, r0);
    __syncthreads();
    const double *Dp = D_s + slot * slot_stride + pb;
    for (int e = threadIdx.x; e < (TY + 2) * W1; e += NTH) {
        int ly = e / W1, lxx = e - ly * W1;
        int gr = refl(r0 - 1 + ly, G.ns), gc = refl(c0 - 1 + lxx, G.nf);
        int p2 = (ly + 1) * W2 + lxx + 1;
        stt[e] = -0.5 * P.kappa * lap_at<W2>(sx, p2, G.ax, G.ay) + Dp[(long)gr * G.pitch + gc] * sx[p2];
    }
    __syncthreads();
    const double idt = 1.0 / dt;
    for (int k = 0; k < TY / 4; ++k) {
        int ly = ly0 + 4 * k, r = r0 + ly, c = c0 + lx;
        if (r < G.ns && c < G.nf) {
            int p1 = (ly + 1) * W1 + lx + 1, p2 = (ly + 2) * W2 + lx + 2;
            out[pb + (long)r * G.pitch + c] = sx[p2] * idt - lap_at<W1>(stt, p1, G.ax, G.ay);
        }
    }
}

constexpr int GUESS_RING = 8;
constexpr int GUESS_ORD = 8;
#ifndef VCH_GUESS_BMAX
#define VCH_GUESS_BMAX 32
#endif
constexpr int GUESS_BMAX = VCH_GUESS_BMAX;
struct GuessArgs {
    const double *d[GUESS_ORD];
    double c[GUESS_BMAX][GUESS_ORD];
    int per_traj;
    __host__ __device__ const double *row(int b) const { return c[per_traj ? b : 0]; }
};
__host__ __device__ inline unsigned guess_bit(unsigned mask, int b) { return (mask >> (b & 31)) & 1u; }
__global__ __launch_bounds__(NTH) void k_guess(Geom G, Phys P, const TrajState *__restrict__ st, long slot_stride,
                                               GuessArgs ga, const double *__restrict__ D_s, double dt,
                                               double *__restrict__ rhs_s, double *__restrict__ x0, double *__restrict__ part,
                                               int which) {
    TILE_COORDS;
    const TrajState S = st[b];
    if (!S.newton_active || !S.need_trial) return;
    if (which == 1 && S.iters != 1) return;
    const double *gcf = ga.row(b);
    if (gcf[0] == 0.0) return;
    const int slot = which == 1 ? 1 - S.slot : S.slot;
    __shared__ double sx[(TY + 4) * (TX + 4)];
    __shared__ double stt[(TY + 2) * (TX + 2)];
    __shared__ double sred[4];
    constexpr int W2 = TX + 4, W1 = TX + 2;
    const long pb = b * G.plane;
    for (int e = threadIdx.x; e < W2 * (TY + 4); e += NTH) {
        int ly = e / W2, lxx = e - ly * W2;
        int gr = refl(r0 - 2 + ly, G.ns), gc = refl(c0 - 2 + lxx, G.nf);
        long o = pb + (long)gr * G.pitch + gc;
        double v = gcf[0] * ga.d[0][o];
#pragma unroll
        for (int j = 1; j < GUESS_ORD; ++j)
            if (gcf[j] != 0.0) v += gcf[j] * ga.d[j][o];
        sx[e] = isfinite(v) ? v : 0.0;
    }
    __syncthreads();
    const double *Dp = D_s + slot * slot_stride + pb;
    for (int e = threadIdx.x; e < (TY + 2) * W1; e += NTH) {
        int ly = e / W1, lxx = e - ly * W1;
        int gr = refl(r0 - 1 + ly, G.ns), gc = refl(c0 - 1 + lxx, G.nf);
        int p2 = (ly + 1) * W2 + lxx + 1;
        stt[e] = -0.5 * P.kappa * lap_at<W2>(sx, p2, G.ax, G.ay) + Dp[(long)gr * G.pitch + gc] * sx[p2];
    }
    __syncthreads();
    const double idt = 1.0 / dt;
    double acc = 0.0;
    for (int k = 0; k < TY / 4; ++k) {
        int ly = ly0 + 4 * k, r = r0 + ly, c = c0 + lx;
        if (r < G.ns && c < G.nf) {
            int p1 = (ly + 1) * W1 + lx + 1, p2 = (ly + 2) * W2 + lx + 2;
            long o = pb + (long)r * G.pitch + c, os = slot * slot_stride + o;
            const double rh = rhs_s[os] - (sx[p2] * idt - lap_at<W1>(stt, p1, G.ax, G.ay));
            rhs_s[os] = rh;
            x0[o] = sx[p2];
            acc += rh * rh;
        }
    }
    acc = wave_sum(acc);
    if ((threadIdx.x & 63) == 0) sred[threadIdx.x >> 6] = acc;
    __syncthreads();
    if (threadIdx.x == 0) {
        double *pp = part + ((long)b * nblk + blk) * NPART;
        pp[4] = pp[1];
        pp[1] = (sred[0] + sred[1]) + (sred[2] + sred[3]);
    }
}

__global__ __launch_bounds__(NTH) void k_dmu_ceiling(Geom G, Phys P, const TrajState *__restrict__ st,
                                                     long slot_stride, const double *__restrict__ x,
                                                     const double *__restrict__ phi_s,
                                                     const double *__restrict__ D_s,
                                                     const double *__restrict__ Rphi_s, double *__restrict__ dmu,
                                                     double *__restrict__ x_out, double *__restrict__ part) {
    TILE_COORDS;
    const TrajState S = st[b];
    if (!S.newton_active || S.need_trial) return;
    __shared__ double sx[(TY + 2) * (TX + 2)];
    __shared__ double sred[NPART * 4];
    constexpr int W = TX + 2;
    const long pb = b * G.plane;
    load_tile<1>(sx, x + pb, G, c0, r0);
    __syncthreads();
    double acc[1] = {1e300};
    for (int k = 0; k < TY / 4; ++k) {
        int ly = ly0 + 4 * k, r = r0 + ly, c = c0 + lx;
        if (r < G.ns && c < G.nf) {
            int p = (ly + 1) * W + lx + 1;
            long o = pb + (long)r * G.pitch + c, os = S.slot * slot_stride + o;
            double d = sx[p];
            x_out[o] = d;
            dmu[o] = 2.0 * ((-0.5 * P.kappa * lap_at<W>(sx, p, G.ax, G.ay) + D_s[os] * d) + Rphi_s[os]);
            double ph = phi_s[os];
            if (d > 0.0) acc[0] = fmin(acc[0], (1.0 - DELTA_SEP - ph) / d);
            else if (d < 0.0) acc[0] = fmin(acc[0], (-1.0 + DELTA_SEP - ph) / d);
        }
    }
    const int op[1] = {1};
    block_reduce_store<1>(acc, op, sred, part + ((long)b * nblk + blk) * NPART);
}

__global__ __launch_bounds__(NTH) void k_jac_apply(Geom G, Phys P, const double *__restrict__ phi,
                                                   const double *__restrict__ dphi, const double *__restrict__ dmu,
                                                   double dt, double *__restrict__ op_, double *__restrict__ om_) {
    TILE_COORDS;
    __shared__ double sa[(TY + 2) * (TX + 2)];
    __shared__ double sb[(TY + 2) * (TX + 2)];
    constexpr int W = TX + 2;
    const long pb = b * G.plane;
    load_tile<1>(sa, dphi + pb, G, c0, r0);
    load_tile<1>(sb, dmu + pb, G, c0, r0);
    __syncthreads();
    for (int k = 0; k < TY / 4; ++k) {
        int ly = ly0 + 4 * k, r = r0 + ly, c = c0 + lx;
        if (r < G.ns && c < G.nf) {
            int p = (ly + 1) * W + lx + 1;
            long o = pb + (long)r * G.pitch + c;
            double d = jac_diag(phi[o], P.tau / dt, P.c1);
            op_[o] = -0.5 * P.kappa * lap_at<W>(sa, p, G.ax, G.ay) + d * sa[p] - 0.5 * sb[p];
            om_[o] = sa[p] / dt - 0.5 * lap_at<W>(sb, p, G.ax, G.ay);
        }
    }
}

__global__ __launch_bounds__(NTH) void k_residual_plain(Geom G, Phys P, const double *__restrict__ pn,
                                                        const double *__restrict__ po, const double *__restrict__ mn,
                                                        const double *__restrict__ mo, const double *__restrict__ wn,
                                                        const double *__restrict__ wo, double dt,
                                                        double *__restrict__ Rp, double *__restrict__ Rm,
                                                        double *__restrict__ part) {
    TILE_COORDS;
    __shared__ double s[4][(TY + 2) * (TX + 2)];
    __shared__ double sred[NPART * 4];
    constexpr int W = TX + 2;
    const long pb = b * G.plane;
    load_tile<1>(s[0], pn + pb, G, c0, r0);
    load_tile<1>(s[1], po + pb, G, c0, r0);
    load_tile<1>(s[2], mn + pb, G, c0, r0);
    load_tile<1>(s[3], mo + pb, G, c0, r0);
    __syncthreads();
    double acc[1] = {0.0};
    for (int k = 0; k < TY / 4; ++k) {
        int ly = ly0 + 4 * k, r = r0 + ly, c = c0 + lx;
        if (r < G.ns && c < G.nf) {
            int p = (ly + 1) * W + lx + 1;
            long o = pb + (long)r * G.pitch + c;
            double rp = (P.tau * (s[0][p] - s[1][p]) / dt) -
                        0.5 * P.kappa * (lap_at<W>(s[0], p, G.ax, G.ay) + lap_at<W>(s[1], p, G.ax, G.ay)) +
                        (P.c1 * reglog(s[0][p]) + (-2.0 * P.c2 * s[1][p])) - 0.5 * (s[2][p] + s[3][p]) -
                        0.5 * (wn[o] + wo[o]);
            double rm = (s[0][p] - s[1][p]) / dt - 0.5 * (lap_at<W>(s[2], p, G.ax, G.ay) + lap_at<W>(s[3], p, G.ax, G.ay));
            Rp[o] = rp;
            Rm[o] = rm;
            acc[0] += rp * rp + rm * rm;
        }
    }
    const int op[1] = {0};
    block_reduce_store<1>(acc, op, sred, part + ((long)b * nblk + blk) * NPART);
}

__global__ __launch_bounds__(NTH) void k_mass(Geom G, const TrajState *__restrict__ st, long slot_stride,
                                              const double *__restrict__ phi_s, const double *__restrict__ wts,
                                              int do_clip, double *__restrict__ part) {
    TILE_COORDS;
    __shared__ double sred[NPART * 4];
    if (st[b].frozen) return;
    const int slot = st[b].slot;
    const double hi = 1.0 - DELTA_SEP;
    double acc[2] = {0.0, 0.0};
    for (int k = 0; k < TY / 4; ++k) {
        int r = r0 + ly0 + 4 * k, c = c0 + lx;
        if (r < G.ns && c < G.nf) {
            long o = (long)r * G.pitch + c;
            double ph = phi_s[slot * slot_stride + b * G.plane + o];
            if (do_clip) ph = fmin(fmax(ph, -hi), hi);
            double w = wts[o];
            acc[0] += w * ph;
            if (fabs(ph) < hi - 5e-3) acc[1] += w;
        }
    }
    const int op[2] = {0, 0};
    block_reduce_store<2>(acc, op, sred, part + ((long)b * nblk + blk) * NPART);
}

__device__ __forceinline__ void post_sums(const double *__restrict__ part, int nblk, int b, double *sm2) {
    if (threadIdx.x < 64) {
        double a0 = 0.0, a1 = 0.0;
        for (int t = threadIdx.x; t < nblk; t += 64) {
            a0 += part[((long)b * nblk + t) * NPART];
            a1 += part[((long)b * nblk + t) * NPART + 1];
        }
        a0 = wave_sum(a0);
        a1 = wave_sum(a1);
        if (threadIdx.x == 0) {
            sm2[0] = a0;
            sm2[1] = a1;
        }
    }
}
struct PostFix {
    double shift, hi;
    bool fix, interior_ok;
    __device__ __forceinline__ PostFix(const double *sm2, double mass0, double LxLy) {
        const double mass_err = sm2[0] - mass0, Wint = sm2[1];
        hi = 1.0 - DELTA_SEP;
        fix = fabs(mass_err) > 1e-16;
        interior_ok = Wint > 0.0;
        shift = fix ? (interior_ok ? mass_err / Wint : mass_err / LxLy) : 0.0;
    }
    __device__ __forceinline__ double apply(double v) const {
        double ph = fmin(fmax(v, -hi), hi);
        if (fix) {
            if (interior_ok) {
                if (fabs(ph) < hi - 5e-3) ph -= shift;
            } else {
                ph = fmin(fmax(ph - shift, -hi), hi);
            }
        }
        return ph;
    }
};
struct PostArgs {
    const double *part;
    double *hist;
    long hist_stride;
};

__global__ __launch_bounds__(NTH) void k_post(Geom G, Phys P, const TrajState *__restrict__ st, long slot_stride,
                                              double *__restrict__ phi_s, double *__restrict__ hist_level,
                                              long hist_stride, const double *__restrict__ part) {
    TILE_COORDS;
    const TrajState S = st[b];
    if (S.frozen) return;
    __shared__ double sm[2];
    post_sums(part, nblk, b, sm);
    __syncthreads();
    const PostFix pf(sm, S.mass0, P.LxLy);
    for (int k = 0; k < TY / 4; ++k) {
        int r = r0 + ly0 + 4 * k, c = c0 + lx;
        if (r < G.ns && c < G.nf) {
            long o = (long)r * G.pitch + c;
            long os = S.slot * slot_stride + b * G.plane + o;
            const double ph = pf.apply(phi_s[os]);
            phi_s[os] = ph;
            if (hist_level) hist_level[b * hist_stride + o] = ph;
        }
    }
}

__global__ __launch_bounds__(NTH) void k_adj_rhs(Geom G, Phys P, const double *__restrict__ p,
                                                 const double *__restrict__ q, const double *__restrict__ phin,
                                                 const double *__restrict__ phin1, const double *__restrict__ qn,
                                                 const double *__restrict__ qn1, long hist_stride, double dt,
                                                 double b1, double *__restrict__ rhs, double *__restrict__ Dn,
                                                 double *__restrict__ part) {
    TILE_COORDS;
    __shared__ double sq[(TY + 2) * (TX + 2)];
    __shared__ double sred[NPART * 4];
    constexpr int W = TX + 2;
    const long pb = b * G.plane;
    load_tile<1>(sq, q + pb, G, c0, r0);
    __syncthreads();
    double acc[3] = {1e300, -1e300, 0.0};
    for (int k = 0; k < TY / 4; ++k) {
        int ly = ly0 + 4 * k, r = r0 + ly, c = c0 + lx;
        if (r < G.ns && c < G.nf) {
            int pp = (ly + 1) * W + lx + 1;
            long o = (long)r * G.pitch + c, oh = b * hist_stride + o;
            double f0 = phin[oh], f1 = phin1[oh];
            double t0 = qn ? qn[oh] : 0.0, t1 = qn1 ? qn1[oh] : 0.0;
            double src = 0.5 * dt * b1 * ((f0 - t0) + (f1 - t1));
            double dplus = fpp_log(f1, P.c1, P.c2), dn = fpp_log(f0, P.c1, P.c2);
            double v = p[pb + o] + (P.tau - 0.5 * dt * dplus) * sq[pp] + 0.5 * dt * lap_at<W>(sq, pp, G.ax, G.ay) + src;
            rhs[pb + o] = v;
            Dn[pb + o] = dn;
            acc[0] = fmin(acc[0], dn);
            acc[1] = fmax(acc[1], dn);
            acc[2] += v * v;
        }
    }
    const int op[3] = {1, 2, 0};
    block_reduce_store<3>(acc, op, sred, part + ((long)b * nblk + blk) * NPART);
}

template <int MODE>
__global__ __launch_bounds__(NTH) void k_adj_op(Geom G, Phys P, const TrajState *__restrict__ st,
                                                const double *__restrict__ x, const double *__restrict__ Dn,
                                                const double *__restrict__ rhs, double dt,
                                                double *__restrict__ out, double *__restrict__ part) {
    TILE_COORDS;
    if (MODE == 1 && !st[b].lin_active) return;
    const double dbar = MODE == 1 ? st[b].dbar : 0.0;
    __shared__ double sx[(TY + 4) * (TX + 4)];
    __shared__ double stt[(TY + 2) * (TX + 2)];
    __shared__ double sred[NPART * 4];
    constexpr int W2 = TX + 4, W1 = TX + 2;
    const long pb = b * G.plane;
    load_tile<2>(sx, x + pb, G, c0, r0);
    __syncthreads();
    for (int e = threadIdx.x; e < (TY + 2) * W1; e += NTH) {
        int ly = e / W1, lxx = e - ly * W1;
        stt[e] = -lap_at<W2>(sx, (ly + 1) * W2 + lxx + 1, G.ax, G.ay);
    }
    __syncthreads();
    double acc[2] = {0.0, 0.0};
    const double sgn = MODE == 2 ? -1.0 : 1.0;
    for (int k = 0; k < TY / 4; ++k) {
        int ly = ly0 + 4 * k, r = r0 + ly, c = c0 + lx;
        if (r < G.ns && c < G.nf) {
            int p1 = (ly + 1) * W1 + lx + 1, p2 = (ly + 2) * W2 + lx + 2;
            long o = pb + (long)r * G.pitch + c;
            double t = stt[p1], mt = -lap_at<W1>(stt, p1, G.ax, G.ay);
            double ax_ = sx[p2] + (P.tau + sgn * 0.5 * dt * Dn[o]) * t + sgn * 0.5 * dt * mt;
            if (MODE == 1) {
                double rr = rhs[o] - ax_;
                out[o] = rr;
                acc[0] += wdev(r, c, G) / (Dn[o] - dbar) * (rr * rr);
                acc[1] += rr * rr;
            } else {
                out[o] = ax_;
            }
        }
    }
    if (MODE == 1) {
        const int op[2] = {0, 0};
        block_reduce_store<2>(acc, op, sred, part + ((long)b * nblk + blk) * NPART);
    }
}

__global__ __launch_bounds__(NTH) void k_adj_finish(Geom G, const double *__restrict__ p,
                                                    const double *__restrict__ q_old, double *__restrict__ q_new,
                                                    double *__restrict__ r_cur, double gb, double gs,
                                                    double *__restrict__ r_hist, double *__restrict__ p_hist,
                                                    double *__restrict__ q_hist, long hist_stride) {
    TILE_COORDS;
    __shared__ double s[(TY + 2) * (TX + 2)];
    constexpr int W = TX + 2;
    const long pb = b * G.plane;
    load_tile<1>(s, p + pb, G, c0, r0);
    __syncthreads();
    for (int k = 0; k < TY / 4; ++k) {
        int ly = ly0 + 4 * k, r = r0 + ly, c = c0 + lx;
        if (r < G.ns && c < G.nf) {
            int pp = (ly + 1) * W + lx + 1;
            long o = (long)r * G.pitch + c, oh = b * hist_stride + o;
            double qn = -lap_at<W>(s, pp, G.ax, G.ay);
            double rn = q_old ? gb * r_cur[pb + o] + gs * (qn + q_old[pb + o]) : 0.0;
            q_new[pb + o] = qn;
            r_cur[pb + o] = rn;
            if (r_hist) r_hist[oh] = rn;
            if (p_hist) p_hist[oh] = s[pp];
            if (q_hist) q_hist[oh] = qn;
        }
    }
}

__global__ __launch_bounds__(NTH) void k_scaled_diff(Geom G, const double *__restrict__ x, long xs,
                                                     const double *__restrict__ y, long ys, double a,
                                                     double *__restrict__ out, double *__restrict__ part) {
    TILE_COORDS;
    __shared__ double sred[NPART * 4];
    double acc[1] = {0.0};
    for (int k = 0; k < TY / 4; ++k) {
        int r = r0 + ly0 + 4 * k, c = c0 + lx;
        if (r < G.ns && c < G.nf) {
            long o = (long)r * G.pitch + c;
            double v = a * (x[b * xs + o] - (y ? y[b * ys + o] : 0.0));
            out[b * G.plane + o] = v;
            acc[0] += v * v;
        }
    }
    const int op[1] = {0};
    block_reduce_store<1>(acc, op, sred, part + ((long)b * nblk + blk) * NPART);
}

__global__ __launch_bounds__(NTH) void k_copy_plane(Geom G, const double *__restrict__ src, long ss,
                                                    double *__restrict__ dst, long ds) {
    TILE_COORDS;
    for (int k = 0; k < TY / 4; ++k) {
        int r = r0 + ly0 + 4 * k, c = c0 + lx;
        if (r < G.ns && c < G.nf) {
            long o = (long)r * G.pitch + c;
            dst[b * ds + o] = src[b * ss + o];
        }
    }
}

__global__ __launch_bounds__(NTH) void k_cost(Geom G, int tiles_f, const double *__restrict__ phi,
                                              const double *__restrict__ u, const double *__restrict__ pq,
                                              const double *__restrict__ pt, const double *__restrict__ phi0,
                                              const double *__restrict__ tfrac, long hist_stride, int last_level,
                                              const double *__restrict__ W, double *__restrict__ part) {
    const int b = blockIdx.z, lvl = blockIdx.y;
    const int tf = blockIdx.x % tiles_f, ts = blockIdx.x / tiles_f;
    const int c0 = tf * TX, r0 = ts * TY;
    const int lx = threadIdx.x & 63, ly0 = threadIdx.x >> 6;
    __shared__ double sred[NPART * 4];
    double acc[4] = {0.0, 0.0, 0.0, 0.0};
    const long lb = b * hist_stride + (long)lvl * G.plane;
    const double tf_ = tfrac ? tfrac[lvl] : 0.0;
    for (int k = 0; k < TY / 4; ++k) {
        int r = r0 + ly0 + 4 * k, c = c0 + lx;
        if (r < G.ns && c < G.nf) {
            long o = (long)r * G.pitch + c;
            double w = W[o], ph = phi[lb + o];
            double uu = u ? u[lb + o] : 0.0;
            double tq;
            if (pq) tq = pq[lb + o];
            else if (tfrac) tq = (1.0 - tf_) * phi0[b * G.plane + o] + tf_ * pt[b * G.plane + o];
            else tq = 0.0;
            double e = ph - tq;
            acc[0] += w * (e * e);
            acc[2] += w * (uu * uu);
            acc[3] += w * fabs(uu);
            if (lvl == last_level) {
                double e2 = ph - (pt ? pt[b * G.plane + o] : 0.0);
                acc[1] += w * (e2 * e2);
            }
        }
    }
    const int op[4] = {0, 0, 0, 0};
    block_reduce_store<4>(acc, op, sred, part + (((long)b * gridDim.y + lvl) * gridDim.x + blockIdx.x) * 4);
}

__global__ __launch_bounds__(NTH) void k_energy(Geom G, int A0, int A1, double c1, double c2, double eps,
                                                const double *__restrict__ phi, const double *__restrict__ w,
                                                long hist_stride, double *__restrict__ part) {
    __shared__ double sred[NPART * 4];
    const int b = blockIdx.z, lvl = blockIdx.y;
    const long base = b * hist_stride + (long)lvl * G.plane;
    const double *ph = phi + base;
    const double *wp = w ? w + base : nullptr;
    auto at = [&](const double *p, int f) { return p[(long)(f / G.nf) * G.pitch + (f % G.nf)]; };
    double acc[4] = {0.0, 0.0, 0.0, 0.0};
    const int total = A0 * A1;
    for (int k = 0; k < 4; ++k) {
        const int f = blockIdx.x * 1024 + k * NTH + threadIdx.x;
        if (f < total) {
            const int i = f / A1, j = f - i * A1;
            const double a = at(ph, f);
            if (i + 1 < A0) { const double d = at(ph, f + A1) - a; acc[0] += d * d; }
            if (j + 1 < A1) { const double d = at(ph, f + 1) - a; acc[1] += d * d; }
            const double wt = ((i == 0 || i == A0 - 1) ? 0.5 : 1.0) * ((j == 0 || j == A1 - 1) ? 0.5 : 1.0);
            const double p = fmin(fmax(a, -1.0 + eps), 1.0 - eps);
            const double psi = c1 * ((1.0 + p) * log(1.0 + p) + (1.0 - p) * log(1.0 - p)) - c2 * (p * p);
            acc[2] += wt * psi;
            if (wp) acc[3] += wt * at(wp, f) * a;
        }
    }
    const int op[4] = {0, 0, 0, 0};
    block_reduce_store<4>(acc, op, sred, part + (((long)b * gridDim.y + lvl) * gridDim.x + blockIdx.x) * 4);
}

__global__ void k_cost_fin(int ntiles, const double *__restrict__ part, double *__restrict__ out) {
    const long idx = (long)blockIdx.x;
    double a[4] = {0, 0, 0, 0};
    for (int t = threadIdx.x; t < ntiles; t += 64)
        for (int k = 0; k < 4; ++k) a[k] += part[(idx * ntiles + t) * 4 + k];
    for (int k = 0; k < 4; ++k) {
        double v = wave_sum(a[k]);
        if (threadIdx.x == 0) out[idx * 4 + k] = v;
    }
}

__global__ __launch_bounds__(NTH) void k_grad_prox(Geom G, int tiles_f, const double *__restrict__ u,
                                                   const double *__restrict__ r, long hist_stride,
                                                   const double *__restrict__ alpha, double b3, double ks,
                                                   double umin, double umax, double *__restrict__ uout,
                                                   double *__restrict__ part) {
    const int b = blockIdx.z, lvl = blockIdx.y;
    const int tf = blockIdx.x % tiles_f, ts = blockIdx.x / tiles_f;
    const int c0 = tf * TX, r0 = ts * TY;
    const int lx = threadIdx.x & 63, ly0 = threadIdx.x >> 6;
    __shared__ double sred[NPART * 4];
    const double al = alpha[b];
    const long lb = b * hist_stride + (long)lvl * G.plane;
    double acc[2] = {0.0, 0.0};
    for (int k = 0; k < TY / 4; ++k) {
        int rr = r0 + ly0 + 4 * k, c = c0 + lx;
        if (rr < G.ns && c < G.nf) {
            long o = lb + (long)rr * G.pitch + c;
            double uu = u[o];
            double v = uu - al * (r[o] + b3 * uu);
            double sgn = v > 0.0 ? 1.0 : (v < 0.0 ? -1.0 : 0.0);
            double s = sgn * fmax(fabs(v) - al * ks, 0.0);
            double un = fmin(fmax(s, umin), umax);
            uout[o] = un;
            acc[0] += (un - uu) * (un - uu);
            acc[1] += uu * uu;
        }
    }
    if (part) {
        const int op[2] = {0, 0};
        block_reduce_store<2>(acc, op, sred, part + (((long)b * gridDim.y + lvl) * gridDim.x + blockIdx.x) * 4);
    }
}

__device__ __forceinline__ void fin_reduce(const double *part, int nblk, int b, double (&out)[NPART],
                                           const int (&op)[NPART], int n) {
    double a[NPART];
#pragma unroll
    for (int k = 0; k < NPART; ++k) a[k] = op[k] == 0 ? 0.0 : (op[k] == 1 ? 1e300 : -1e300);
    for (int t = threadIdx.x; t < nblk; t += 64) {
        const double *p = part + ((long)b * nblk + t) * NPART;
#pragma unroll
        for (int k = 0; k < NPART; ++k)
            if (k < n) {
                const double v = p[k];
                a[k] = op[k] == 0 ? a[k] + v : (op[k] == 1 ? fmin(a[k], v) : fmax(a[k], v));
            }
    }
#pragma unroll
    for (int k = 0; k < NPART; ++k)
        if (k < n) out[k] = op[k] == 0 ? wave_sum(a[k]) : (op[k] == 1 ? wave_min(a[k]) : wave_max(a[k]));
}

__device__ __forceinline__ void traj_copy_in(TrajState &dst, const TrajState *src) {
    const unsigned *s = reinterpret_cast<const unsigned *>(src);
    unsigned *d = reinterpret_cast<unsigned *>(&dst);
    for (int i = threadIdx.x; i < (int)(sizeof(TrajState) / 4); i += 64) d[i] = s[i];
    __syncthreads();
}
__device__ __forceinline__ void traj_copy_out(TrajState *dst, const TrajState &src) {
    __syncthreads();
    const unsigned *s = reinterpret_cast<const unsigned *>(&src);
    unsigned *d = reinterpret_cast<unsigned *>(dst);
    for (int i = threadIdx.x; i < (int)(sizeof(TrajState) / 4); i += 64) d[i] = s[i];
}

constexpr int HIST_CAP = 512;
constexpr double NEWTON_TOL = 1e-6;
constexpr int NEWTON_MAXIT = 500;
constexpr double ARMIJO_ETA = 1e-4;
constexpr int ARMIJO_TRIALS = 12;

__global__ void k_set_frozen(TrajState *st, const int *__restrict__ flags, int B) {
    int b = blockIdx.x * blockDim.x + threadIdx.x;
    if (b < B) st[b].frozen = flags[b];
}

__device__ __forceinline__ void cg_setup(TrajState &S, double g0, double cscale, double tol) {
    const double range = S.Dmax - S.Dmin;
    S.dbar = S.Dmin - fmax(1e-12, 0.05 * fmin(range, fabs(S.Dmin) + 1.0));
    const double den = cscale * S.dbar + g0;
    double kT = den > 0.0 ? 1.0 + cscale * (S.Dmax - S.dbar) / den : 1e12;
    const double sq = sqrt(kT);
    const double rate = (sq - 1.0) / (sq + 1.0);
    S.kT = kT;
    S.rho = rate;
    double k = rate > 1e-300 ? log(2.0 / tol) / -log(rate) : 1.0;
    S.lin_budget = (int)fmin(4000.0, ceil(k) + 2.0);
}

__device__ __forceinline__ double newton_lin_tol(double r0, double lin_tol, double eta) {
    if (!(eta > 0.0) || !(r0 > 0.0)) return lin_tol;
    if (r0 > 1e8) return fmax(lin_tol, 1e-12);
    return fmin(fmax(lin_tol, eta / r0), 0.5);
}

struct SolveOpts {
    int cheb_max;
    double scale_ratio;
    double eta1_factor;
};

__device__ __forceinline__ double cg_weight(double D, double dbar, int scaled) {
    const double dl = D - dbar;
    return scaled ? dl / D : dl;
}

constexpr int CHEB_NCAP = 200;
__device__ __forceinline__ void cheb_plan(TrajState &S, double tol) {
    const double kT = S.kT > 1.0 ? S.kT : 1.0;
    S.cheb_theta = 0.5 * (kT + 1.0);
    S.cheb_delta = 0.5 * (kT - 1.0);
    int n = 0;
    if (S.cheb_delta > 0.0) {
        const double sigma = S.cheb_theta / S.cheb_delta;
        double tkm1 = 1.0, tk = sigma;
        while (n < CHEB_NCAP && !(1.0 / tk <= tol)) {
            const double tn = 2.0 * sigma * tk - tkm1;
            tkm1 = tk;
            tk = tn;
            ++n;
        }
    }
    S.cheb_n = n;
}
__device__ __forceinline__ double cheb_last_factor(double theta, double delta, int n) {
    if (!(delta > 0.0)) return 0.0;
    const double sigma = theta / delta;
    double tkm1 = 1.0, tk = sigma;
    for (int k = 0; k < n; ++k) {
        const double tn = 2.0 * sigma * tk - tkm1;
        tkm1 = tk;
        tk = tn;
        if (!(tk < 1e280)) return 1.0 / (2.0 * sigma);
    }
    return tkm1 / tk;
}

template <int MODE>
__device__ __forceinline__ void fin_residual_update(TrajState &S, const double (&v)[NPART], bool primed, double *__restrict__ hist,
                                                    double kappa, double dt, double lin_tol, double eta, SolveOpts so);

template <int MODE>
__global__ void k_fin_residual(TrajState *st, const double *__restrict__ part, int nblk,
                               double *__restrict__ hist, double kappa, double dt, double lin_tol, double eta, int guess,
                               SolveOpts so) {
    const int b = blockIdx.x;
    __shared__ TrajState S;
    traj_copy_in(S, st + b);
    if (MODE == 2) {
        if (S.frozen) return;
        if (threadIdx.x == 0) {
            newton_begin(S);
            S.slot = 1 - S.slot;
        }
        __syncthreads();
    }
    if (!S.newton_active || !S.need_trial) return;
    double v[NPART];
    const int op[NPART] = {0, 0, 1, 2, 0, 0};
    const bool primed = guess_bit((unsigned)guess, b) && (MODE != 1 || S.iters == 1);
    fin_reduce(part, nblk, b, v, op, primed ? 5 : 4);
    if (threadIdx.x == 0)
        fin_residual_update<(MODE == 1 ? 1 : 0)>(S, v, primed, hist + (long)b * HIST_CAP, kappa, dt, lin_tol, eta, so);
    traj_copy_out(st + b, S);
}

template <int MODE>
__device__ __forceinline__ void fin_residual_update(TrajState &S, const double (&v)[NPART], bool primed, double *__restrict__ hist,
                                                    double kappa, double dt, double lin_tol, double eta, SolveOpts so) {
    const double nt = sqrt(v[0]);
    bool accept;
    if (MODE == 0) {
        accept = true;
    } else {
        S.ntrials++;
        if (S.force_accept) {
            accept = true;
        } else {
            if (nt < S.best_norm) { S.best_norm = nt; S.best_alpha = S.alpha; }
            accept = nt <= (1.0 - ARMIJO_ETA * S.alpha) * S.normR;
        }
    }
    if (accept) {
        if (MODE == 1) S.slot = 1 - S.slot;
        S.normR = nt;
        S.need_trial = 0;
        S.force_accept = 0;
        if (S.iters < HIST_CAP) hist[S.iters] = nt;
        if (S.iters < 4) S.step_R[S.iters] = nt;
        if (S.iters == 1) {
            S.R1_hist[2] = S.R1_hist[1];
            S.R1_hist[1] = S.R1_hist[0];
            S.R1_hist[0] = nt;
        }
        S.iters++;
        S.newton_total++;
        if (!(nt >= NEWTON_TOL) || S.iters > NEWTON_MAXIT) {
            if (S.iters > NEWTON_MAXIT) S.iters = NEWTON_MAXIT;
            S.newton_active = 0;
            return;
        }
        S.Dmin = v[2];
        S.Dmax = v[3];
        S.lin_r0 = sqrt(v[1]);
        S.x_primed = primed ? 1 : 0;
        S.lin_rscale = (primed && v[4] > 0.0) ? fmin(1.0, sqrt(v[1] / v[4])) : 1.0;
        if (MODE == 0) S.guess_ratio = (primed && v[4] > 0.0) ? sqrt(v[1] / v[4]) : 1.0;
        else if (primed) S.guess_ratio2 = v[4] > 0.0 ? sqrt(v[1] / v[4]) : 1.0;
        double eta_eff = eta;
        if (MODE == 0 && eta > 0.0 && so.eta1_factor > 0.0 && S.R1_hist[0] > 0.0 && S.R1_hist[1] > 0.0 && S.R1_hist[2] > 0.0)
            eta_eff = fmax(eta, so.eta1_factor * fmin(S.R1_hist[0], fmin(S.R1_hist[1], S.R1_hist[2])));
        S.lin_reltol = newton_lin_tol(S.lin_r0, lin_tol, eta_eff);
        cg_setup(S, 2.0 * sqrt(0.5 * kappa / dt), 1.0, S.lin_reltol);
        cheb_plan(S, S.lin_reltol);
        S.use_cheb = (so.cheb_max >= 0 && S.cheb_n <= so.cheb_max) ? 1 : 0;
        S.scaled = (!S.use_cheb && so.scale_ratio > 0.0 && S.Dmax > so.scale_ratio * S.Dmin) ? 1 : 0;
        S.lin_active = 1;
        S.lin_it = 0;
        S.lin_prev = 1e300;
        S.lin_rel = 1.0;
        S.nsolves++;
        S.step_solves++;
        if (S.step_solves <= 4) {
            S.step_tol[S.step_solves - 1] = S.lin_reltol;
            S.step_kT[S.step_solves - 1] = S.kT;
            S.step_chn[S.step_solves - 1] = S.cheb_n;
            S.step_form[S.step_solves - 1] = S.use_cheb;
        }
    } else {
        S.alpha *= 0.5;
        S.trial_no++;
        if (S.trial_no >= ARMIJO_TRIALS) {
            if (S.best_norm < S.normR) {
                S.alpha = S.best_alpha;
                S.force_accept = 1;
            } else {
                S.stuck = 1;
                S.need_trial = 0;
                while (S.iters < NEWTON_MAXIT) {
                    if (S.iters < HIST_CAP) hist[S.iters] = S.normR;
                    S.iters++;
                }
                S.newton_active = 0;
            }
        }
    }
}

struct EvalFin {
    unsigned *counter;
    double *hist;
    double kappa, lin_tol, eta;
    SolveOpts so;
};

__device__ __forceinline__ void store_agent(double *p, double v) { __hip_atomic_store(p, v, __ATOMIC_RELAXED, __HIP_MEMORY_SCOPE_AGENT); }
__device__ __forceinline__ double load_agent(const double *p) {
    return __hip_atomic_load(p, __ATOMIC_RELAXED, __HIP_MEMORY_SCOPE_AGENT);
}

__device__ __forceinline__ void fin_reduce_agent(const double *part, int nblk, int b, double (&out)[NPART], const int (&op)[NPART], int n) {
    double a[NPART];
#pragma unroll
    for (int k = 0; k < NPART; ++k) a[k] = op[k] == 0 ? 0.0 : (op[k] == 1 ? 1e300 : -1e300);
    for (int t = threadIdx.x; t < nblk; t += 64) {
        const double *p = part + ((long)b * nblk + t) * NPART;
#pragma unroll
        for (int k = 0; k < NPART; ++k)
            if (k < n) {
                const double v = load_agent(p + k);
                a[k] = op[k] == 0 ? a[k] + v : (op[k] == 1 ? fmin(a[k], v) : fmax(a[k], v));
            }
    }
#pragma unroll
    for (int k = 0; k < NPART; ++k)
        if (k < n) out[k] = op[k] == 0 ? wave_sum(a[k]) : (op[k] == 1 ? wave_min(a[k]) : wave_max(a[k]));
}

#ifndef EVAL_MINBLK
#define EVAL_MINBLK 5
#endif
template <int MODE, bool FIN_INSIDE>
__global__ __launch_bounds__(NTH, EVAL_MINBLK) void k_eval(Geom G, Phys P, TrajState *st, long slot_stride, double *phi_s, double *mu_s,
                                              double *Rphi_s, double *rhs_s, double *D_s, const double *dphi, double *cphi,
                                              double *cmu, double dt, double *part, const double *w, const double *un,
                                              const double *unp1, long u_stride, double *wnew, GuessArgs ga, double *x0,
                                              EvalFin fin, PostArgs post) {
    TILE_COORDS;
    const int S_slot = st[b].slot, S_iters = MODE == 0 ? 0 : st[b].iters;
    const double S_alpha = MODE == 0 ? 0.0 : st[b].alpha;
    if (MODE == 0) {
        if (st[b].frozen) {
            if (blk == 0 && threadIdx.x == 0) st[b].newton_active = st[b].need_trial = st[b].lin_active = 0;
            return;
        }
    } else {
        if (!st[b].newton_active || !st[b].need_trial) return;
    }
    __shared__ double sp[(TY + 4) * (TX + 4)];
    __shared__ double sd[MODE == 2 ? (TY + 4) * (TX + 4) : 1];
    __shared__ double sm[(TY + 2) * (TX + 2)];
    __shared__ double sr[MODE == 0 ? (TY + 2) * (TX + 2) : 1];
    __shared__ double sred[NPART * 4];
    __shared__ int s_last;
    constexpr int W2 = TX + 4, W1 = TX + 2;
    const long pb = b * G.plane;
    const int src = S_slot, dst = 1 - S_slot;
    const double tdt = P.tau / dt;
    const double *gcf = ga.row(b);
    const bool do_guess = gcf[0] != 0.0 && (MODE == 0 || S_iters == 1);
    double rm[TY / 4], rh[TY / 4];
    double acc[5] = {0.0, 0.0, 1e300, -1e300, 0.0};
    if (MODE == 0) {
        constexpr int N1 = (TY + 2) * W1, I1 = (N1 + NTH - 1) / NTH;
        if (post.part) {
            __shared__ double s_post[2];
            constexpr int I2 = (W2 * (TY + 4) + NTH - 1) / NTH;
            double raw[I2];
#pragma unroll
            for (int i = 0; i < I2; ++i) {
                const int e = threadIdx.x + i * NTH;
                raw[i] = 0.0;
                if (e < W2 * (TY + 4)) {
                    int ly = e / W2, lxx = e - ly * W2;
                    int gr = refl(r0 - 2 + ly, G.ns), gc = refl(c0 - 2 + lxx, G.nf);
                    raw[i] = phi_s[src * slot_stride + pb + (long)gr * G.pitch + gc];
                }
            }
            post_sums(post.part, nblk, (int)b, s_post);
            __syncthreads();
            const PostFix pf(s_post, st[b].mass0, P.LxLy);
#pragma unroll
            for (int i = 0; i < I2; ++i) {
                const int e = threadIdx.x + i * NTH;
                if (e < W2 * (TY + 4)) sp[e] = pf.apply(raw[i]);
            }
        } else {
            load_tile<2>(sp, phi_s + src * slot_stride + pb, G, c0, r0);
        }
        load_tile<1>(sm, mu_s + src * slot_stride + pb, G, c0, r0);
        double vW[I1], vU0[I1], vU1[I1];
#pragma unroll
        for (int i = 0; i < I1; ++i) {
            const int e = threadIdx.x + i * NTH;
            vW[i] = vU0[i] = vU1[i] = 0.0;
            if (e < N1) {
                int ly = e / W1, lxx = e - ly * W1;
                int gr = refl(r0 - 1 + ly, G.ns), gc = refl(c0 - 1 + lxx, G.nf);
                long o = (long)gr * G.pitch + gc;
                vW[i] = w[pb + o];
                vU0[i] = un ? un[b * u_stride + o] : 0.0;
                vU1[i] = unp1 ? unp1[b * u_stride + o] : 0.0;
            }
        }
        __syncthreads();
        for (int k = 0; k < TY / 4; ++k) {
            int ly = ly0 + 4 * k, r = r0 + ly, c = c0 + lx;
            rm[k] = 0.0;
            if (r < G.ns && c < G.nf) {
                int p1 = (ly + 1) * W1 + lx + 1, p2 = (ly + 2) * W2 + lx + 2;
                const double cm = -sp[p2] / dt - 0.5 * lap_at<W1>(sm, p1, G.ax, G.ay);
                cmu[pb + (long)r * G.pitch + c] = cm;
                rm[k] = cm;
            }
        }
        __syncthreads();
        const double gdt = P.gamma / dt;
#pragma unroll
        for (int i = 0; i < I1; ++i) {
            const int e = threadIdx.x + i * NTH;
            if (e >= N1) continue;
            int ly = e / W1, lxx = e - ly * W1;
            int rr = r0 - 1 + ly, cc = c0 - 1 + lxx;
            int gr = refl(rr, G.ns), gc = refl(cc, G.nf);
            int p2 = (ly + 1) * W2 + lxx + 1;
            long o = (long)gr * G.pitch + gc, ob = pb + o;
            const double u0 = vU0[i], u1 = vU1[i], wo = vW[i];
            const double wn = ((gdt - 0.5) * wo + 0.5 * (u1 + u0)) / (gdt + 0.5);
            const double ph = sp[p2], lp = lap_at<W2>(sp, p2, G.ax, G.ay);
            const double m0 = -P.kappa * lp + (P.c1 * reglog(ph) - 2.0 * P.c2 * ph) - wn;
            const double cp = -(P.tau / dt) * ph - 0.5 * P.kappa * lp - 2.0 * P.c2 * ph - 0.5 * sm[e] - 0.5 * (wn + wo);
            sr[e] = tdt * ph - 0.5 * P.kappa * lp + P.c1 * reglog(ph) - 0.5 * m0 + cp;
            sm[e] = m0;
            if (ly >= 1 && ly <= TY && lxx >= 1 && lxx <= TX && rr < G.ns && cc < G.nf) {
                wnew[ob] = wn;
                cphi[ob] = cp;
            }
        }
        __syncthreads();
        for (int k = 0; k < TY / 4; ++k) {
            int ly = ly0 + 4 * k, r = r0 + ly, c = c0 + lx;
            rh[k] = 0.0;
            if (r < G.ns && c < G.nf) {
                int p1 = (ly + 1) * W1 + lx + 1, p2 = (ly + 2) * W2 + lx + 2;
                long od = dst * slot_stride + pb + (long)r * G.pitch + c;
                const double ph = sp[p2], rp = sr[p1];
                const double rmv = ph / dt - 0.5 * lap_at<W1>(sm, p1, G.ax, G.ay) + rm[k];
                const double rhv = -rmv + lap_at<W1>(sr, p1, G.ax, G.ay);
                const double d = jac_diag(ph, tdt, P.c1);
                phi_s[od] = ph;
                if (post.part && post.hist) post.hist[b * post.hist_stride + (long)r * G.pitch + c] = ph;
                mu_s[od] = sm[p1];
                Rphi_s[od] = rp;
                D_s[od] = d;
                rh[k] = rhv;
                acc[0] += rp * rp + rmv * rmv;
                acc[2] = fmin(acc[2], d);
                acc[3] = fmax(acc[3], d);
            }
        }
    } else {
        const double *phi_o = phi_s + src * slot_stride + pb, *mu_o = mu_s + src * slot_stride + pb;
        const double *D_o = D_s + src * slot_stride + pb, *R_o = Rphi_s + src * slot_stride + pb;
        constexpr int N1 = (TY + 2) * W1, I1 = (N1 + NTH - 1) / NTH;
        double pd[(W2 * (TY + 4) + NTH - 1) / NTH], pp[(W2 * (TY + 4) + NTH - 1) / NTH];
        {
            int i = 0;
#pragma unroll
            for (int e = threadIdx.x; e < W2 * (TY + 4); e += NTH, ++i) {
                int ly = e / W2, lxx = e - ly * W2;
                int gr = refl(r0 - 2 + ly, G.ns), gc = refl(c0 - 2 + lxx, G.nf);
                long o = (long)gr * G.pitch + gc;
                pd[i] = dphi[pb + o];
                pp[i] = phi_o[o];
            }
        }
        double vD[I1], vR[I1], vM[I1], vC[I1], vcm[TY / 4];
#pragma unroll
        for (int i = 0; i < I1; ++i) {
            const int e = threadIdx.x + i * NTH;
            vD[i] = vR[i] = vM[i] = vC[i] = 0.0;
            if (e < N1) {
                int ly = e / W1, lxx = e - ly * W1;
                int gr = refl(r0 - 1 + ly, G.ns), gc = refl(c0 - 1 + lxx, G.nf);
                long o = (long)gr * G.pitch + gc;
                vD[i] = D_o[o];
                vR[i] = R_o[o];
                vM[i] = mu_o[o];
                vC[i] = cphi[pb + o];
            }
        }
#pragma unroll
        for (int k = 0; k < TY / 4; ++k) {
            int r = r0 + ly0 + 4 * k, c = c0 + lx;
            vcm[k] = (r < G.ns && c < G.nf) ? cmu[pb + (long)r * G.pitch + c] : 0.0;
        }
        {
            int i = 0;
#pragma unroll
            for (int e = threadIdx.x; e < W2 * (TY + 4); e += NTH, ++i) {
                sd[e] = pd[i];
                sp[e] = pp[i] + S_alpha * pd[i];
            }
        }
        __syncthreads();
#pragma unroll
        for (int i = 0; i < I1; ++i) {
            const int e = threadIdx.x + i * NTH;
            if (e < N1) {
                int ly = e / W1, lxx = e - ly * W1;
                int p2 = (ly + 1) * W2 + lxx + 1;
                const double Dv = vD[i], Rv = vR[i], Mv = vM[i];
                const double dm = 2.0 * ((-0.5 * P.kappa * lap_at<W2>(sd, p2, G.ax, G.ay) + Dv * sd[p2]) + Rv);
                sm[e] = Mv + S_alpha * dm;
            }
        }
        __syncthreads();
        double mt[TY / 4];
        for (int k = 0; k < TY / 4; ++k) {
            int ly = ly0 + 4 * k, r = r0 + ly, c = c0 + lx;
            rm[k] = mt[k] = 0.0;
            if (r < G.ns && c < G.nf) {
                int p1 = (ly + 1) * W1 + lx + 1, p2 = (ly + 2) * W2 + lx + 2;
                const double cm = vcm[k];
                rm[k] = sp[p2] / dt - 0.5 * lap_at<W1>(sm, p1, G.ax, G.ay) + cm;
                mt[k] = sm[p1];
            }
        }
        __syncthreads();
#pragma unroll
        for (int i = 0; i < I1; ++i) {
            const int e = threadIdx.x + i * NTH;
            if (e < N1) {
                int ly = e / W1, lxx = e - ly * W1;
                int p2 = (ly + 1) * W2 + lxx + 1;
                const double cp = vC[i];
                double ph = sp[p2];
                sm[e] = tdt * ph - 0.5 * P.kappa * lap_at<W2>(sp, p2, G.ax, G.ay) + P.c1 * reglog(ph) - 0.5 * sm[e] + cp;
            }
        }
        __syncthreads();
        for (int k = 0; k < TY / 4; ++k) {
            int ly = ly0 + 4 * k, r = r0 + ly, c = c0 + lx;
            rh[k] = 0.0;
            if (r < G.ns && c < G.nf) {
                int p1 = (ly + 1) * W1 + lx + 1, p2 = (ly + 2) * W2 + lx + 2;
                long od = dst * slot_stride + pb + (long)r * G.pitch + c;
                double ph = sp[p2], rp = sm[p1];
                double rhv = -rm[k] + lap_at<W1>(sm, p1, G.ax, G.ay);
                double d = jac_diag(ph, tdt, P.c1);
                phi_s[od] = ph;
                mu_s[od] = mt[k];
                Rphi_s[od] = rp;
                D_s[od] = d;
                rh[k] = rhv;
                acc[0] += rp * rp + rm[k] * rm[k];
                acc[2] = fmin(acc[2], d);
                acc[3] = fmax(acc[3], d);
            }
        }
    }
    if (do_guess) {
        double *X = MODE == 0 ? sp : sd;
        double *STT = MODE == 0 ? sr : sp;
        __syncthreads();
        for (int e = threadIdx.x; e < (TY + 2) * W1; e += NTH) {
            int ly = e / W1, lxx = e - ly * W1;
            sm[e] = jac_diag(sp[(ly + 1) * W2 + lxx + 1], tdt, P.c1);
        }
        __syncthreads();
        for (int e = threadIdx.x; e < W2 * (TY + 4); e += NTH) {
            int ly = e / W2, lxx = e - ly * W2;
            int gr = refl(r0 - 2 + ly, G.ns), gc = refl(c0 - 2 + lxx, G.nf);
            long o = pb + (long)gr * G.pitch + gc;
            double v = gcf[0] * ga.d[0][o];
#pragma unroll
            for (int j = 1; j < GUESS_ORD; ++j)
                if (gcf[j] != 0.0) v += gcf[j] * ga.d[j][o];
            X[e] = isfinite(v) ? v : 0.0;
        }
        __syncthreads();
        for (int e = threadIdx.x; e < (TY + 2) * W1; e += NTH) {
            int ly = e / W1, lxx = e - ly * W1;
            int p2 = (ly + 1) * W2 + lxx + 1;
            STT[e] = -0.5 * P.kappa * lap_at<W2>(X, p2, G.ax, G.ay) + sm[e] * X[p2];
        }
        double xv[TY / 4];
        for (int k = 0; k < TY / 4; ++k) xv[k] = X[(ly0 + 4 * k + 2) * W2 + lx + 2];
        __syncthreads();
        const double idt = 1.0 / dt;
        for (int k = 0; k < TY / 4; ++k) {
            int ly = ly0 + 4 * k, r = r0 + ly, c = c0 + lx;
            if (r < G.ns && c < G.nf) {
                int p1 = (ly + 1) * W1 + lx + 1;
                const double full = rh[k];
                const double defl = full - (xv[k] * idt - lap_at<W1>(STT, p1, G.ax, G.ay));
                x0[pb + (long)r * G.pitch + c] = xv[k];
                acc[4] += full * full;
                rh[k] = defl;
            }
        }
    }
    for (int k = 0; k < TY / 4; ++k) {
        int r = r0 + ly0 + 4 * k, c = c0 + lx;
        if (r < G.ns && c < G.nf) {
            rhs_s[dst * slot_stride + pb + (long)r * G.pitch + c] = rh[k];
            acc[1] += rh[k] * rh[k];
        }
    }
    {
        const int lane = threadIdx.x & 63, wv = threadIdx.x >> 6;
        const int op5[5] = {0, 0, 1, 2, 0};
#pragma unroll
        for (int k = 0; k < 5; ++k) {
            double r_ = op5[k] == 0 ? wave_sum(acc[k]) : (op5[k] == 1 ? wave_min(acc[k]) : wave_max(acc[k]));
            if (lane == 0) sred[k * 4 + wv] = r_;
        }
        __syncthreads();
        if (threadIdx.x == 0) {
            double *pp = part + ((long)b * nblk + blk) * NPART;
#pragma unroll
            for (int k = 0; k < 5; ++k) {
                const double a = sred[k * 4], bb = sred[k * 4 + 1], cc = sred[k * 4 + 2], dd = sred[k * 4 + 3];
                const double v = op5[k] == 0 ? (a + bb) + (cc + dd)
                                             : (op5[k] == 1 ? fmin(fmin(a, bb), fmin(cc, dd)) : fmax(fmax(a, bb), fmax(cc, dd)));
                if (FIN_INSIDE) store_agent(pp + k, v);
                else pp[k] = v;
            }
            if (FIN_INSIDE) {
                asm volatile("s_waitcnt vmcnt(0)" ::: "memory");
                const unsigned old = __hip_atomic_fetch_add(fin.counter + b, 1u, __ATOMIC_RELAXED, __HIP_MEMORY_SCOPE_AGENT);
                s_last = old == (unsigned)(nblk - 1) ? 1 : 0;
            }
        }
        if (!FIN_INSIDE) return;
        __syncthreads();
        if (!s_last || threadIdx.x >= 64) return;
    }
    if (FIN_INSIDE) {
        double v[NPART];
        const int op[NPART] = {0, 0, 1, 2, 0, 0};
        fin_reduce_agent(part, nblk, b, v, op, do_guess ? 5 : 4);
        if (threadIdx.x != 0) return;
        __hip_atomic_store(fin.counter + b, 0u, __ATOMIC_RELAXED, __HIP_MEMORY_SCOPE_AGENT);
        TrajState S = st[b];
        if (MODE == 0) {
            newton_begin(S);
            S.slot = dst;
        }
        fin_residual_update<(MODE == 0 ? 0 : 1)>(S, v, do_guess, fin.hist + (long)b * HIST_CAP, fin.kappa, dt, fin.lin_tol, fin.eta,
                                                 fin.so);
        st[b] = S;
    }
}

__device__ __forceinline__ double fin_sum1(const double *part, int n, int b, int stride, int k) {
    double a = 0.0;
    for (int t = threadIdx.x; t < n; t += 64) a += part[((long)b * n + t) * stride + k];
    return wave_sum(a);
}

__global__ void k_fin_cg_init(TrajState *st, const double *__restrict__ gpart, int gnblk) {
    const int b = blockIdx.x;
    TrajState &S = st[b];
    if (threadIdx.x == 0) {
        S.cg_pending = 0;
        if (!S.lin_active) S.ci_active[0] = 0;
    }
    if (!S.lin_active) return;
    double g = fin_sum1(gpart, gnblk, b, 1, 0);
    if (threadIdx.x != 0) return;
    S.cg_gamma = S.cg_gamma0 = g;
    S.cg_beta = 0.0;
    S.lin_it = 0;
    S.lin_rel = 1.0;
    S.ci_active[0] = S.lin_active;
    S.ci_it[0] = 0;
    S.ci_gamma[0] = g;
}

struct CgNext {
    int active, breakdown, it;
    double alpha, beta, gamma, rel;
};
__device__ __forceinline__ CgNext cg_next(double pq, double qq, double gamma, double gamma0, int it_old, double tol,
                                          int maxit) {
    CgNext n;
    n.it = it_old;
    if (!(pq > 0.0) || !(gamma > 0.0)) {
        n.active = 0; n.breakdown = 1; n.alpha = 0.0; n.beta = 0.0; n.gamma = fmax(gamma, 0.0);
        n.rel = gamma0 > 0.0 ? sqrt(fmax(gamma, 0.0) / gamma0) : 0.0;
        return n;
    }
    n.breakdown = 0;
    n.alpha = gamma / pq;
    double gn = n.alpha * n.alpha * qq - gamma;
    if (gn > 1e-13 * gamma) {
        n.beta = gn / gamma;
    } else {
        gn = 1e-13 * gamma;
        n.beta = 0.0;
    }
    n.gamma = gn;
    n.it = it_old + 1;
    n.rel = sqrt(gn / gamma0);
    n.active = (n.rel > tol && n.it < maxit) ? 1 : 0;
    return n;
}

__device__ __forceinline__ void cg_sums(const double *__restrict__ gpart, const double *__restrict__ gpart2, int gnblk,
                                        const double *__restrict__ part, int nblk, int pslot, int direct, int b,
                                        double *s3 ) {
    const int wv = threadIdx.x >> 6, lane = threadIdx.x & 63;
    if (wv < 3) {
        const double *src = wv == 0 ? gpart : (wv == 1 ? gpart2 : part + pslot);
        const int n = wv == 2 ? nblk : gnblk, stride = wv == 2 ? NPART : 1;
        double a = 0.0;
        if (wv < 2 || direct)
            for (int t = lane; t < n; t += 64) a += src[((long)b * n + t) * stride];
        a = wave_sum(a);
        if (lane == 0) s3[wv] = a;
    }
    __syncthreads();
}

__device__ __forceinline__ void cg_record(TrajState &S, const CgNext &n, int wr) {
    S.cg_alpha = n.alpha;
    S.cg_beta = n.beta;
    S.cg_gamma = n.gamma;
    S.lin_rel = n.rel;
    if (!n.breakdown) {
        S.lin_it = n.it;
        S.lin_total++;
    }
    if (!n.active && n.rel * S.lin_rscale > S.lin_maxrel) S.lin_maxrel = n.rel * S.lin_rscale;
    if (!n.active) S.lin_maxabs = fmax(S.lin_maxabs, n.rel * S.lin_r0);
    if (n.it > S.step_lin_max) S.step_lin_max = n.it;
    if (S.step_solves >= 1 && S.step_solves <= 4 && n.it > S.step_lin[S.step_solves - 1]) S.step_lin[S.step_solves - 1] = n.it;
    S.ci_active[wr] = n.active;
    S.ci_it[wr] = n.it;
    S.ci_gamma[wr] = n.gamma;
}

__global__ void k_fin_cg_step(TrajState *st, const double *__restrict__ gpart, const double *__restrict__ gpart2,
                              int gnblk, const double *__restrict__ part, int nblk, int pslot, int direct, int pbuf,
                              int rd, double tol, int maxit) {
    const int b = blockIdx.x;
    TrajState &S = st[b];
    __shared__ double s3[3];
    if (!S.lin_active) return;
    if (!S.ci_active[rd]) {
        if (threadIdx.x == 0) { S.lin_active = 0; S.cg_pending = 0; }
        return;
    }
    cg_sums(gpart, gpart2, gnblk, part, nblk, pslot, direct, b, s3);
    if (threadIdx.x != 0) return;
    const CgNext n = cg_next(s3[0], s3[1], direct ? s3[2] : S.ci_gamma[rd], S.cg_gamma0, S.ci_it[rd], S.lin_reltol, maxit);
    cg_record(S, n, rd ^ 1);
    S.cg_pending = n.breakdown ? 0 : 1;
    S.cg_pbuf = pbuf;
    S.lin_active = n.active;
}

__global__ void k_cg_publish(TrajState *st, int rd, int B) {
    const int b = blockIdx.x * blockDim.x + threadIdx.x;
    if (b < B && st[b].lin_active && !st[b].ci_active[rd]) st[b].lin_active = 0;
}

__global__ void k_fin_cg_alpha(TrajState *st, const double *__restrict__ part, int n, int stride, int k) {
    const int b = blockIdx.x;
    TrajState &S = st[b];
    if (!S.lin_active) return;
    double pq = fin_sum1(part, n, b, stride, k);
    if (threadIdx.x != 0) return;
    if (!(pq > 0.0)) {
        S.lin_active = 0;
        S.cg_alpha = 0.0;
        if (S.lin_rel > S.lin_maxrel) S.lin_maxrel = S.lin_rel;
        return;
    }
    S.cg_alpha = S.cg_gamma / pq;
}

__global__ void k_fin_cg_beta(TrajState *st, const double *__restrict__ part, int nblk, int mode, double tol,
                              int maxit, int init) {
    const int b = blockIdx.x;
    TrajState &S = st[b];
    if (!S.lin_active) return;
    double gn = fin_sum1(part, nblk, b, NPART, 0);
    double rr = mode == 1 ? fin_sum1(part, nblk, b, NPART, 1) : 0.0;
    if (threadIdx.x != 0) return;
    if (init) {
        S.cg_gamma = S.cg_gamma0 = gn;
        S.cg_beta = 0.0;
        S.lin_it = 0;
    } else {
        S.cg_beta = S.cg_gamma > 0.0 ? gn / S.cg_gamma : 0.0;
        S.cg_gamma = gn;
        S.lin_it++;
        S.lin_total++;
    }
    S.lin_rel = mode == 1 ? (S.lin_r0 > 0.0 ? sqrt(rr) / S.lin_r0 : 0.0)
                          : (S.cg_gamma0 > 0.0 ? sqrt(gn / S.cg_gamma0) : 0.0);
    if (!(S.lin_rel > tol) || S.lin_it >= maxit) {
        S.lin_active = 0;
        if (S.lin_rel > S.lin_maxrel) S.lin_maxrel = S.lin_rel;
    }
}

struct ChebFin {
    int enq, gnblk;
    const double *g0, *gn;
    const double *cmin;
};
__global__ void k_fin_ceiling(TrajState *st, const double *__restrict__ part, int nblk, int strict, int fin_copy, ChebFin cheb) {
    const int b = blockIdx.x;
    __shared__ TrajState S;
    traj_copy_in(S, st + b);
    if (!S.newton_active || S.need_trial) return;
    if ((cheb.enq >= 0) != (S.use_cheb != 0)) return;
    int lin_active = S.lin_active;
    if (cheb.enq >= 0 && lin_active) {
        if (S.cheb_n > cheb.enq) return;
        double rel = 1.0;
        if (S.cheb_n >= 1) {
            const double g0 = fin_sum1(cheb.g0, cheb.gnblk, b, 1, 0), gn = fin_sum1(cheb.gn, cheb.gnblk, b, 1, 0);
            rel = g0 > 0.0 ? sqrt(fmax(gn, 0.0) / g0) : 0.0;
        }
        if (threadIdx.x == 0) {
            rel *= cheb_last_factor(S.cheb_theta, S.cheb_delta, S.cheb_n);
            S.lin_rel = rel;
            S.lin_it = S.cheb_n;
            S.lin_total += S.cheb_n;
            if (rel * S.lin_rscale > S.lin_maxrel) S.lin_maxrel = rel * S.lin_rscale;
            S.lin_maxabs = fmax(S.lin_maxabs, rel * S.lin_r0);
            if (S.cheb_n > S.step_lin_max) S.step_lin_max = S.cheb_n;
            if (S.step_solves >= 1 && S.step_solves <= 4) S.step_lin[S.step_solves - 1] = S.cheb_n;
        }
        lin_active = 0;
    }
    if (fin_copy >= 0 && lin_active) {
        lin_active = fin_copy == 0 ? S.ci_active[0] : S.ci_active[1];
        if (strict && lin_active) {
            if (threadIdx.x == 0) st[b].lin_active = lin_active;
            return;
        }
    }
    if (strict && lin_active) return;
    double v[NPART];
    const int op[NPART] = {1, 0, 0, 0, 0, 0};
    if (cheb.enq >= 0 && cheb.cmin) {
        double a = 1e300;
        for (int t = threadIdx.x; t < cheb.gnblk; t += 64) a = fmin(a, cheb.cmin[(long)b * cheb.gnblk + t]);
        v[0] = wave_min(a);
    } else {
        fin_reduce(part, nblk, b, v, op, 1);
    }
    if (threadIdx.x == 0) {
        double amax = 2.0;
        if (v[0] < 1e299) amax = fmin(amax, 0.9 * v[0]);
        if (!isfinite(amax) || amax <= 0.0) amax = 1.0;
        S.alpha = fmin(1.0, amax);
        if (lin_active && S.lin_rel > S.lin_maxrel) S.lin_maxrel = S.lin_rel;
        S.lin_active = 0;
        S.need_trial = 1;
        S.trial_no = 0;
        S.force_accept = 0;
        S.best_norm = 1e300;
        S.best_alpha = S.alpha;
    }
    traj_copy_out(st + b, S);
}

__global__ void k_fin_mass(TrajState *st, const double *__restrict__ part, int nblk, int init) {
    const int b = blockIdx.x;
    TrajState &S = st[b];
    if (S.frozen) return;
    double v[NPART];
    const int op[NPART] = {0, 0, 0, 0, 0, 0};
    fin_reduce(part, nblk, b, v, op, 2);
    if (threadIdx.x != 0) return;
    if (init) {
        S.mass0 = v[0];
        S.mass_err = 0.0;
    } else {
        S.mass_err = v[0] - S.mass0;
    }
    S.Wint = v[1];
}

__global__ void k_fin_lin_begin(TrajState *st, const double *__restrict__ part, int nblk, int mode,
                                double tau, double kappa, double dt, double lin_tol) {
    const int b = blockIdx.x;
    TrajState &S = st[b];
    if (threadIdx.x == 0 && S.lin_active) {
        S.lin_unconv++;
        if (S.lin_rel > S.lin_maxrel) S.lin_maxrel = S.lin_rel;
    }
    double v[NPART];
    const int op0[NPART] = {1, 2, 0, 0, 0, 0};
    const int op1[NPART] = {0, 0, 0, 0, 0, 0};
    const int op2[NPART] = {0, 0, 1, 2, 0, 0};
    if (mode == 0) fin_reduce(part, nblk, b, v, op0, 3);
    else if (mode == 1) fin_reduce(part, nblk, b, v, op1, 1);
    else fin_reduce(part, nblk, b, v, op2, 4);
    if (threadIdx.x != 0) return;
    double dmin = 0.0, dmax = 0.0, r0;
    if (mode == 0) { dmin = v[0]; dmax = v[1]; r0 = sqrt(v[2]); }
    else if (mode == 1) { r0 = sqrt(v[0]); }
    else { dmin = v[2]; dmax = v[3]; r0 = sqrt(v[1]); }
    S.Dmin = dmin;
    S.Dmax = dmax;
    if (mode == 2) cg_setup(S, 2.0 * sqrt(0.5 * kappa / dt), 1.0, lin_tol);
    else cg_setup(S, tau + 2.0 * sqrt(0.5 * dt), 0.5 * dt, lin_tol);
    S.lin_r0 = r0;
    S.lin_active = (mode == 2 || r0 > 0.0) ? 1 : 0;
    S.lin_it = 0;
    S.lin_prev = 1e300;
    S.lin_rel = 1.0;
    S.lin_reltol = lin_tol;
    S.use_cheb = 0;
    S.scaled = 0;
    S.nsolves++;
}

__global__ __launch_bounds__(NTH) void k_solve_setup(Geom G, Phys P, const double *__restrict__ a,
                                                     const double *__restrict__ bv, const double *__restrict__ phi,
                                                     double dt, double *__restrict__ Rphi, double *__restrict__ rhs,
                                                     double *__restrict__ D, double *__restrict__ part) {
    TILE_COORDS;
    __shared__ double s[(TY + 2) * (TX + 2)];
    __shared__ double sred[NPART * 4];
    constexpr int W = TX + 2;
    const long pb = b * G.plane;
    load_tile<1>(s, a + pb, G, c0, r0);
    __syncthreads();
    double acc[4] = {0.0, 0.0, 1e300, -1e300};
    for (int k = 0; k < TY / 4; ++k) {
        int ly = ly0 + 4 * k, r = r0 + ly, c = c0 + lx;
        if (r < G.ns && c < G.nf) {
            int p = (ly + 1) * W + lx + 1;
            long o = pb + (long)r * G.pitch + c;
            double rh = bv[o] - lap_at<W>(s, p, G.ax, G.ay);
            double d = jac_diag(phi[o], P.tau / dt, P.c1);
            Rphi[o] = -s[p];
            rhs[o] = rh;
            D[o] = d;
            acc[1] += rh * rh;
            acc[2] = fmin(acc[2], d);
            acc[3] = fmax(acc[3], d);
        }
    }
    const int op[4] = {0, 0, 1, 2};
    block_reduce_store<4>(acc, op, sred, part + ((long)b * nblk + blk) * NPART);
}

__global__ __launch_bounds__(NTH) void k_adj_setup(Geom G, Phys P, const double *__restrict__ phi,
                                                   const double *__restrict__ rhs, double *__restrict__ Dn,
                                                   double *__restrict__ part) {
    TILE_COORDS;
    __shared__ double sred[NPART * 4];
    double acc[3] = {1e300, -1e300, 0.0};
    for (int k = 0; k < TY / 4; ++k) {
        int r = r0 + ly0 + 4 * k, c = c0 + lx;
        if (r < G.ns && c < G.nf) {
            long o = b * G.plane + (long)r * G.pitch + c;
            double d = phi ? fpp_log(phi[o], P.c1, P.c2) : 0.0;
            Dn[o] = d;
            acc[0] = fmin(acc[0], d);
            acc[1] = fmax(acc[1], d);
            if (rhs) acc[2] += rhs[o] * rhs[o];
        }
    }
    const int op[3] = {1, 2, 0};
    block_reduce_store<3>(acc, op, sred, part + ((long)b * nblk + blk) * NPART);
}

__global__ __launch_bounds__(NTH) void k_solve_w(Geom G, const double *__restrict__ w, const double *__restrict__ un,
                                                 const double *__restrict__ unp1, double gdt, double *__restrict__ out) {
    TILE_COORDS;
    for (int k = 0; k < TY / 4; ++k) {
        int r = r0 + ly0 + 4 * k, c = c0 + lx;
        if (r < G.ns && c < G.nf) {
            long o = b * G.plane + (long)r * G.pitch + c;
            double u0 = un ? un[o] : 0.0, u1 = unp1 ? unp1[o] : 0.0;
            out[o] = ((gdt - 0.5) * w[o] + 0.5 * (u1 + u0)) / (gdt + 0.5);
        }
    }
}

__global__ __launch_bounds__(NTH) void k_adj_guess(Geom G, double *__restrict__ x, GuessArgs ga, double *__restrict__ keep) {
    TILE_COORDS;
    for (int k = 0; k < TY / 4; ++k) {
        int r = r0 + ly0 + 4 * k, c = c0 + lx;
        if (r < G.ns && c < G.nf) {
            const long o = b * G.plane + (long)r * G.pitch + c;
            const double p1 = x[o];
            const double *gcf = ga.row(b);
            double v = gcf[0] * p1;
#pragma unroll
            for (int j = 1; j < GUESS_ORD; ++j)
                if (gcf[j] != 0.0) v += gcf[j] * ga.d[j][o];
            keep[o] = p1;
            x[o] = isfinite(v) ? v : p1;
        }
    }
}

__global__ void k_reset_longest(TrajState *st, int B) {
    const int b = blockIdx.x * blockDim.x + threadIdx.x;
    if (b < B) st[b].step_lin_max = 0;
}

__global__ __launch_bounds__(NTH) void k_fill(Geom G, double *__restrict__ x, double v) {
    TILE_COORDS;
    for (int k = 0; k < TY / 4; ++k) {
        int r = r0 + ly0 + 4 * k, c = c0 + lx;
        if (r < G.ns && c < G.nf) x[b * G.plane + (long)r * G.pitch + c] = v;
    }
}

__global__ __launch_bounds__(NTH) void k_ramp(Geom G, int tiles_f, const double *__restrict__ phi0,
                                              const double *__restrict__ phiT, const double *__restrict__ tfrac,
                                              long hist_stride, double *__restrict__ pq) {
    const int b = blockIdx.z, lvl = blockIdx.y;
    const int c0 = (blockIdx.x % tiles_f) * TX, r0 = (blockIdx.x / tiles_f) * TY;
    const int lx = threadIdx.x & 63, ly0 = threadIdx.x >> 6;
    const double tp = tfrac[lvl];
    for (int k = 0; k < TY / 4; ++k) {
        int r = r0 + ly0 + 4 * k, c = c0 + lx;
        if (r < G.ns && c < G.nf) {
            long o = (long)r * G.pitch + c;
            pq[b * hist_stride + (long)lvl * G.plane + o] = (1 - tp) * phi0[b * G.plane + o] + tp * phiT[b * G.plane + o];
        }
    }
}



template <int FIRST>
__global__ __launch_bounds__(NTH) void k_schur_p(Geom G, Phys P, TrajState *__restrict__ st,
                                                 long slot_stride, const double *__restrict__ z,
                                                 const double *__restrict__ q, const double *__restrict__ p_old,
                                                 const double *__restrict__ D_s, double dt,
                                                 double *__restrict__ x, double *__restrict__ z_new,
                                                 double *__restrict__ p_new, double *__restrict__ v,
                                                 double *__restrict__ part, const double *__restrict__ gpart,
                                                 const double *__restrict__ gpart2, int gnblk, int it, double tol,
                                                 int maxit) {
    TILE_COORDS;
    __shared__ double sx[(TY + 4) * (TX + 4)];
    __shared__ double stt[(TY + 2) * (TX + 2)];
    __shared__ double sred[NPART * 4];
    constexpr int W2 = TX + 4, W1 = TX + 2;
    const long pb = b * G.plane;
    const int rd = (it + 1) & 1, wr = it & 1;
    const int slot = st[b].slot;
    const double dbar = st[b].dbar;
    double alpha = 0.0, beta = 0.0;
    if (FIRST) {
        if (!st[b].ci_active[0]) return;
        load_tile<2>(sx, z + pb, G, c0, r0);
    } else {
        const int was_active = st[b].ci_active[rd];
        if (!was_active) {
            if (blk == 0 && threadIdx.x == 0) {
                st[b].ci_active[wr] = 0;
                st[b].ci_it[wr] = st[b].ci_it[rd];
                st[b].ci_gamma[wr] = st[b].ci_gamma[rd];
            }
            return;
        }
        const double gamma0 = st[b].cg_gamma0, gamma_old = st[b].ci_gamma[rd];
        const int it_old = st[b].ci_it[rd];
        cg_sums(gpart, gpart2, gnblk, part, nblk, rd, it >= 2, b, sred);
        const CgNext n = cg_next(sred[0], sred[1], it >= 2 ? sred[2] : gamma_old, gamma0, it_old, st[b].lin_reltol, maxit);
        __syncthreads();
        if (blk == 0 && threadIdx.x == 0) cg_record(st[b], n, wr);
        alpha = n.alpha;
        beta = n.beta;
        if (!n.active) {
            if (!n.breakdown)
                for (int k = 0; k < TY / 4; ++k) {
                    int r = r0 + ly0 + 4 * k, c = c0 + lx;
                    if (r < G.ns && c < G.nf) {
                        long o = pb + (long)r * G.pitch + c;
                        x[o] += alpha * p_old[o];
                    }
                }
            return;
        }
        for (int e = threadIdx.x; e < W2 * (TY + 4); e += NTH) {
            int ly = e / W2, lxx = e - ly * W2;
            int gr = refl(r0 - 2 + ly, G.ns), gc = refl(c0 - 2 + lxx, G.nf);
            long o = pb + (long)gr * G.pitch + gc;
            sx[e] = (z[o] - alpha * q[o]) + beta * p_old[o];
        }
    }
    __syncthreads();
    const double *Dp = D_s + slot * slot_stride + pb;
    for (int e = threadIdx.x; e < (TY + 2) * W1; e += NTH) {
        int ly = e / W1, lxx = e - ly * W1;
        int gr = refl(r0 - 1 + ly, G.ns), gc = refl(c0 - 1 + lxx, G.nf);
        int p2 = (ly + 1) * W2 + lxx + 1;
        stt[e] = -0.5 * P.kappa * lap_at<W2>(sx, p2, G.ax, G.ay) + Dp[(long)gr * G.pitch + gc] * sx[p2];
    }
    __syncthreads();
    const double idt = 1.0 / dt;
    double acc[1] = {0.0};
    for (int k = 0; k < TY / 4; ++k) {
        int ly = ly0 + 4 * k, r = r0 + ly, c = c0 + lx;
        if (r < G.ns && c < G.nf) {
            int p1 = (ly + 1) * W1 + lx + 1, p2 = (ly + 2) * W2 + lx + 2;
            long o = pb + (long)r * G.pitch + c;
            if (!FIRST) {
                double po = p_old[o];
                double zn = z[o] - alpha * q[o];
                x[o] += alpha * po;
                z_new[o] = zn;
                acc[0] += wdev(r, c, G) * (Dp[(long)r * G.pitch + c] - dbar) * (zn * zn);
            } else {
                x[o] = 0.0;
            }
            p_new[o] = sx[p2];
            v[o] = sx[p2] * idt - lap_at<W1>(stt, p1, G.ax, G.ay);
        }
    }
    if (!FIRST) {
        const int op[1] = {0};
        block_reduce_store<1>(acc, op, sred, part + ((long)b * nblk + blk) * NPART + wr);
    }
}

__global__ __launch_bounds__(NTH) void k_cg_finish(Geom G, const TrajState *__restrict__ st,
                                                   const double *__restrict__ p0, const double *__restrict__ p1,
                                                   double *__restrict__ x) {
    TILE_COORDS;
    const TrajState S = st[b];
    if (!S.cg_pending) return;
    const double *p = S.cg_pbuf ? p1 : p0;
    for (int k = 0; k < TY / 4; ++k) {
        int r = r0 + ly0 + 4 * k, c = c0 + lx;
        if (r < G.ns && c < G.nf) {
            long o = b * G.plane + (long)r * G.pitch + c;
            x[o] += S.cg_alpha * p[o];
        }
    }
}

template <int FIRST>
__global__ __launch_bounds__(NTH) void k_cg_dir(Geom G, const TrajState *__restrict__ st,
                                                const double *__restrict__ r, double *__restrict__ ph) {
    TILE_COORDS;
    const TrajState S = st[b];
    if (!S.lin_active) return;
    for (int k = 0; k < TY / 4; ++k) {
        int rr = r0 + ly0 + 4 * k, c = c0 + lx;
        if (rr < G.ns && c < G.nf) {
            long o = b * G.plane + (long)rr * G.pitch + c;
            ph[o] = FIRST ? r[o] : r[o] + S.cg_beta * ph[o];
        }
    }
}

__global__ __launch_bounds__(NTH) void k_adj_q(Geom G, Phys P, const TrajState *__restrict__ st,
                                               const double *__restrict__ pv, const double *__restrict__ Dn,
                                               const double *__restrict__ ph, double dt, double *__restrict__ q,
                                               double *__restrict__ part) {
    TILE_COORDS;
    const TrajState S = st[b];
    if (!S.lin_active) return;
    __shared__ double sx[(TY + 4) * (TX + 4)];
    __shared__ double stt[(TY + 2) * (TX + 2)];
    __shared__ double sred[NPART * 4];
    constexpr int W2 = TX + 4, W1 = TX + 2;
    const long pb = b * G.plane;
    load_tile<2>(sx, pv + pb, G, c0, r0);
    __syncthreads();
    for (int e = threadIdx.x; e < (TY + 2) * W1; e += NTH) {
        int ly = e / W1, lxx = e - ly * W1;
        stt[e] = -lap_at<W2>(sx, (ly + 1) * W2 + lxx + 1, G.ax, G.ay);
    }
    __syncthreads();
    double acc[1] = {0.0};
    for (int k = 0; k < TY / 4; ++k) {
        int ly = ly0 + 4 * k, r = r0 + ly, c = c0 + lx;
        if (r < G.ns && c < G.nf) {
            int p1 = (ly + 1) * W1 + lx + 1, p2 = (ly + 2) * W2 + lx + 2;
            long o = pb + (long)r * G.pitch + c;
            double d = Dn[o];
            double qv = sx[p2] + (P.tau + 0.5 * dt * d) * stt[p1] - 0.5 * dt * lap_at<W1>(stt, p1, G.ax, G.ay);
            q[o] = qv;
            acc[0] += wdev(r, c, G) / (d - S.dbar) * (ph[o] * qv);
        }
    }
    const int op[1] = {0};
    block_reduce_store<1>(acc, op, sred, part + ((long)b * nblk + blk) * NPART);
}

__global__ __launch_bounds__(NTH) void k_cg_update_adj(Geom G, const TrajState *__restrict__ st,
                                                       const double *__restrict__ pv, const double *__restrict__ q,
                                                       const double *__restrict__ Dn, double *__restrict__ x,
                                                       double *__restrict__ r, double *__restrict__ part) {
    TILE_COORDS;
    const TrajState S = st[b];
    if (!S.lin_active) return;
    __shared__ double sred[NPART * 4];
    double acc[2] = {0.0, 0.0};
    for (int k = 0; k < TY / 4; ++k) {
        int rr = r0 + ly0 + 4 * k, c = c0 + lx;
        if (rr < G.ns && c < G.nf) {
            long o = b * G.plane + (long)rr * G.pitch + c;
            x[o] += S.cg_alpha * pv[o];
            double rn = r[o] - S.cg_alpha * q[o];
            r[o] = rn;
            acc[0] += wdev(rr, c, G) / (Dn[o] - S.dbar) * (rn * rn);
            acc[1] += rn * rn;
        }
    }
    const int op[2] = {0, 0};
    block_reduce_store<2>(acc, op, sred, part + ((long)b * nblk + blk) * NPART);
}
```

Baseline: 5.226 PGD iterations/s.

## Walk stencil halo tiles by wavefront rows with scalar row bases

Replaces the flat element-index halo loops (which need integer division and per-element reflection) with a tile walker that maps each wavefront to a tile row. The row reflection and base pointer become wave-uniform and live in scalar registers via readfirstlane, with only a 32-bit per-lane byte offset. The few halo columns past lane 63 go into one extra slot. The per-element index arithmetic and 64-bit address math in every stencil kernel are meant to shrink. It adds a 4 GiB plane-size guard and static assumptions (TX=64, NTH=256).

Result: no change. 5.200 PGD iterations/s (-0.5%).

```diff
diff --git a/sparse-optimal-control-of-viscous-chan-hilliard-via-gradient-descent--1d-2d_amd/csrc/vch_engine2d.hip b/sparse-optimal-control-of-viscous-chan-hilliard-via-gradient-descent--1d-2d_amd/csrc/vch_engine2d.hip
--- a/sparse-optimal-control-of-viscous-chan-hilliard-via-gradient-descent--1d-2d_amd/csrc/vch_engine2d.hip
+++ b/sparse-optimal-control-of-viscous-chan-hilliard-via-gradient-descent--1d-2d_amd/csrc/vch_engine2d.hip
@@ -291,6 +291,10 @@
 extern "C" vch2d_ctx *vch2d_create(const vch2d_params *p, int batch, int max_steps, int device) {
     if (!p || p->Nx < 2 || p->Ny < 2 || batch < 1 || max_steps < 1 || !(p->Lx > 0) || !(p->Ly > 0)) {
         vch_fail(VCH_ERR_ARG, "vch2d_create: bad arguments (Nx,Ny >= 2, batch >= 1, max_steps >= 1)");
+        return nullptr;
+    }
+    if (((long)p->Ny + 1) * (((long)p->Nx + 8) / 8 * 8) >= (1L << 29)) {
+        vch_fail(VCH_ERR_ARG, "vch2d_create: grid too large (a padded plane must stay below 4 GiB)");
         return nullptr;
     }
     if (hipSetDevice(device) != hipSuccess) {
diff --git a/sparse-optimal-control-of-viscous-chan-hilliard-via-gradient-descent--1d-2d_amd/csrc/vch_fft.h b/sparse-optimal-control-of-viscous-chan-hilliard-via-gradient-descent--1d-2d_amd/csrc/vch_fft.h
--- a/sparse-optimal-control-of-viscous-chan-hilliard-via-gradient-descent--1d-2d_amd/csrc/vch_fft.h
+++ b/sparse-optimal-control-of-viscous-chan-hilliard-via-gradient-descent--1d-2d_amd/csrc/vch_fft.h
@@ -402,11 +402,9 @@
         __syncthreads();
         const double dbar = st[b].dbar;
         const double *Dp = D_s + slot * slot_stride + pb;
-        for (int e = threadIdx.x; e < W * (TY + 2); e += NTH) {
-            int ly = e / W, lxx = e - ly * W;
-            int gr = refl(r0 - 1 + ly, G.ns), gc = refl(c0 - 1 + lxx, G.nf);
-            sx[e] *= dbar / Dp[(long)gr * G.pitch + gc];
-        }
+        tile_walk<1, false>(G, c0, r0, [&](int, int, int, int e, long ro, unsigned vb) VCH_WALK_FN {
+            sx[e] *= dbar / *at(Dp, ro, vb);
+        });
     }
     __syncthreads();
     double acc[1] = {1e300};
diff --git a/sparse-optimal-control-of-viscous-chan-hilliard-via-gradient-descent--1d-2d_amd/csrc/vch_kernels2d.h b/sparse-optimal-control-of-viscous-chan-hilliard-via-gradient-descent--1d-2d_amd/csrc/vch_kernels2d.h
--- a/sparse-optimal-control-of-viscous-chan-hilliard-via-gradient-descent--1d-2d_amd/csrc/vch_kernels2d.h
+++ b/sparse-optimal-control-of-viscous-chan-hilliard-via-gradient-descent--1d-2d_amd/csrc/vch_kernels2d.h
@@ -66,28 +66,80 @@
     return i < 0 ? 0 : i;
 }
 
+#define VCH_WALK_FN __attribute__((always_inline))
+template <int H>
+struct TileWalk {
+    static constexpr int W = TX + 2 * H, HT = TY + 2 * H, X = 2 * H;
+    static constexpr int RI = HT / 4, REM = HT % 4;
+    static constexpr int NI = RI + 1;
+    static_assert(TX == 64 && NTH == 256, "a wavefront spans a tile row; four wavefronts per workgroup");
+    static_assert((X & (X - 1)) == 0 && HT * X <= (4 - REM) * 64, "the columns beyond lane 63 fit the last slot");
+};
+
+template <class T>
+using GlobalPtr = __attribute__((address_space(1))) T *;
+template <class T>
+__device__ __forceinline__ GlobalPtr<T> at(T *base, long ro, unsigned vb) {
+    const unsigned long long u = (unsigned long long)(base + ro);
+    const unsigned lo = __builtin_amdgcn_readfirstlane((unsigned)u), hi = __builtin_amdgcn_readfirstlane((unsigned)(u >> 32));
+    return (GlobalPtr<T>)((((unsigned long long)hi << 32) | lo) + vb);
+}
+
+__device__ __forceinline__ unsigned lane_off(unsigned vb) {
+    asm("" : "+v"(vb));
+    return vb;
+}
+
+__device__ __forceinline__ int wave_id() { return __builtin_amdgcn_readfirstlane((int)(threadIdx.x >> 6)); }
+
+template <int H, class F>
+__device__ __forceinline__ void tile_walk_slot(const Geom &G, int c0, int r0, int wv, int lane, unsigned cb, int i, F &f) {
+    using T = TileWalk<H>;
+    int ly = wv + 4 * i, lx = lane;
+    long ro;
+    unsigned vb;
+    bool ok = true;
+    if (i < T::RI || wv < T::REM) {
+        ro = (long)refl(r0 - H + ly, G.ns) * G.pitch;
+        vb = cb;
+    } else {
+        const unsigned x = (unsigned)(wv - T::REM) * 64u + (unsigned)lane;
+        ly = (int)(x / T::X);
+        lx = TX + (int)(x & (T::X - 1));
+        ok = x < (unsigned)(T::HT * T::X);
+        ro = 0;
+        vb = (unsigned)(refl(r0 - H + ly, G.ns) * G.pitch + refl(c0 - H + lx, G.nf)) * 8u;
+    }
+    if (ok) f(i, ly, lx, ly * T::W + lx, ro, vb);
+}
+
+template <int H, bool UNROLL = true, class F>
+__device__ __forceinline__ void tile_walk(const Geom &G, int c0, int r0, F &&f) {
+    using T = TileWalk<H>;
+    const int wv = wave_id(), lane = threadIdx.x & 63;
+    const unsigned cb = (unsigned)refl(c0 - H + lane, G.nf) * 8u;
+    if constexpr (UNROLL) {
+#pragma unroll
+        for (int i = 0; i < T::NI; ++i) tile_walk_slot<H>(G, c0, r0, wv, lane, cb, i, f);
+    } else {
+#pragma unroll 1
+        for (int i = 0; i < T::NI; ++i) tile_walk_slot<H>(G, c0, r0, wv, lane, cb, i, f);
+    }
+}
+
 template <int H>
 __device__ __forceinline__ void load_tile(double *s, const double *__restrict__ g, const Geom &G,
                                           int c0, int r0) {
-    constexpr int W = TX + 2 * H, HT = TY + 2 * H;
-    for (int e = threadIdx.x; e < W * HT; e += NTH) {
-        int ly = e / W, lx = e - ly * W;
-        int gr = refl(r0 - H + ly, G.ns), gc = refl(c0 - H + lx, G.nf);
-        s[e] = g[(long)gr * G.pitch + gc];
-    }
+    tile_walk<H>(G, c0, r0, [&](int, int, int, int e, long ro, unsigned cb) VCH_WALK_FN { s[e] = *at(g, ro, cb); });
 }
 
 template <int H>
 __device__ __forceinline__ void load_tile_axpy(double *s, const double *__restrict__ a,
                                                const double *__restrict__ d, double alpha,
                                                const Geom &G, int c0, int r0) {
-    constexpr int W = TX + 2 * H, HT = TY + 2 * H;
-    for (int e = threadIdx.x; e < W * HT; e += NTH) {
-        int ly = e / W, lx = e - ly * W;
-        int gr = refl(r0 - H + ly, G.ns), gc = refl(c0 - H + lx, G.nf);
-        long o = (long)gr * G.pitch + gc;
-        s[e] = a[o] + alpha * d[o];
-    }
+    tile_walk<H>(G, c0, r0, [&](int, int, int, int e, long ro, unsigned cb) VCH_WALK_FN {
+        s[e] = *at(a, ro, cb) + alpha * *at(d, ro, cb);
+    });
 }
 
 template <int W>
@@ -159,7 +211,7 @@
     const int nblk = gridDim.x * gridDim.y;           \
     const int blk = xcd_remap(blockIdx.y * gridDim.x + blockIdx.x, nblk); \
     const int c0 = (blk / (int)gridDim.y) * TX, r0 = (blk % (int)gridDim.y) * TY; \
-    const int lx = threadIdx.x & 63, ly0 = threadIdx.x >> 6; \
+    const int lx = threadIdx.x & 63, ly0 = wave_id();   \
     (void)blk; (void)nblk; (void)lx; (void)ly0
 
 __global__ __launch_bounds__(NTH) void k_lap(Geom G, const double *__restrict__ v, double *__restrict__ out) {
@@ -284,14 +336,12 @@
     }
     __syncthreads();
     const double tdt = P.tau / dt;
-    for (int e = threadIdx.x; e < (TY + 2) * W1; e += NTH) {
-        int ly = e / W1, lxx = e - ly * W1;
-        int gr = refl(r0 - 1 + ly, G.ns), gc = refl(c0 - 1 + lxx, G.nf);
+    tile_walk<1, false>(G, c0, r0, [&](int, int ly, int lxx, int e, long ro, unsigned vb) VCH_WALK_FN {
         int p2 = (ly + 1) * W2 + lxx + 1;
         double ph = sp[p2];
         sr[e] = tdt * ph - 0.5 * P.kappa * lap_at<W2>(sp, p2, G.ax, G.ay) + P.c1 * reglog(ph) - 0.5 * sm[e] +
-                cphi[pb + (long)gr * G.pitch + gc];
-    }
+                *at(cphi + pb, ro, vb);
+    });
     __syncthreads();
     double acc[4] = {0.0, 0.0, 1e300, -1e300};
     for (int k = 0; k < TY / 4; ++k) {
@@ -337,23 +387,17 @@
     const int src = S.slot, dst = 1 - S.slot;
     const double *phi_o = phi_s + src * slot_stride + pb, *mu_o = mu_s + src * slot_stride + pb;
     const double *D_o = D_s + src * slot_stride + pb, *R_o = Rphi_s + src * slot_stride + pb;
-    for (int e = threadIdx.x; e < W2 * (TY + 4); e += NTH) {
-        int ly = e / W2, lxx = e - ly * W2;
-        int gr = refl(r0 - 2 + ly, G.ns), gc = refl(c0 - 2 + lxx, G.nf);
-        long o = (long)gr * G.pitch + gc;
-        const double d = dphi[pb + o];
+    tile_walk<2, false>(G, c0, r0, [&](int, int, int, int e, long ro, unsigned vb) VCH_WALK_FN {
+        const double d = *at(dphi + pb, ro, vb);
         sd[e] = d;
-        sp[e] = phi_o[o] + S.alpha * d;
-    }
-    __syncthreads();
-    for (int e = threadIdx.x; e < (TY + 2) * W1; e += NTH) {
-        int ly = e / W1, lxx = e - ly * W1;
-        int gr = refl(r0 - 1 + ly, G.ns), gc = refl(c0 - 1 + lxx, G.nf);
+        sp[e] = *at(phi_o, ro, vb) + S.alpha * d;
+    });
+    __syncthreads();
+    tile_walk<1, false>(G, c0, r0, [&](int, int ly, int lxx, int e, long ro, unsigned vb) VCH_WALK_FN {
         int p2 = (ly + 1) * W2 + lxx + 1;
-        long o = (long)gr * G.pitch + gc;
-        const double dm = 2.0 * ((-0.5 * P.kappa * lap_at<W2>(sd, p2, G.ax, G.ay) + D_o[o] * sd[p2]) + R_o[o]);
-        sm[e] = mu_o[o] + S.alpha * dm;
-    }
+        const double dm = 2.0 * ((-0.5 * P.kappa * lap_at<W2>(sd, p2, G.ax, G.ay) + *at(D_o, ro, vb) * sd[p2]) + *at(R_o, ro, vb));
+        sm[e] = *at(mu_o, ro, vb) + S.alpha * dm;
+    });
     __syncthreads();
     const double tdt = P.tau / dt;
     double rm[TY / 4], mt[TY / 4];
@@ -367,14 +411,12 @@
         }
     }
     __syncthreads();
-    for (int e = threadIdx.x; e < (TY + 2) * W1; e += NTH) {
-        int ly = e / W1, lxx = e - ly * W1;
-        int gr = refl(r0 - 1 + ly, G.ns), gc = refl(c0 - 1 + lxx, G.nf);
+    tile_walk<1, false>(G, c0, r0, [&](int, int ly, int lxx, int e, long ro, unsigned vb) VCH_WALK_FN {
         int p2 = (ly + 1) * W2 + lxx + 1;
         double ph = sp[p2];
         sm[e] = tdt * ph - 0.5 * P.kappa * lap_at<W2>(sp, p2, G.ax, G.ay) + P.c1 * reglog(ph) - 0.5 * sm[e] +
-                cphi[pb + (long)gr * G.pitch + gc];
-    }
+                *at(cphi + pb, ro, vb);
+    });
     __syncthreads();
     double acc[4] = {0.0, 0.0, 1e300, -1e300};
     for (int k = 0; k < TY / 4; ++k) {
@@ -412,12 +454,10 @@
     load_tile<2>(sx, x + pb, G, c0, r0);
     __syncthreads();
     const double *Dp = D_s + slot * slot_stride + pb;
-    for (int e = threadIdx.x; e < (TY + 2) * W1; e += NTH) {
-        int ly = e / W1, lxx = e - ly * W1;
-        int gr = refl(r0 - 1 + ly, G.ns), gc = refl(c0 - 1 + lxx, G.nf);
+    tile_walk<1, false>(G, c0, r0, [&](int, int ly, int lxx, int e, long ro, unsigned vb) VCH_WALK_FN {
         int p2 = (ly + 1) * W2 + lxx + 1;
-        stt[e] = -0.5 * P.kappa * lap_at<W2>(sx, p2, G.ax, G.ay) + Dp[(long)gr * G.pitch + gc] * sx[p2];
-    }
+        stt[e] = -0.5 * P.kappa * lap_at<W2>(sx, p2, G.ax, G.ay) + *at(Dp, ro, vb) * sx[p2];
+    });
     __syncthreads();
     const double idt = 1.0 / dt;
     for (int k = 0; k < TY / 4; ++k) {
@@ -458,24 +498,19 @@
     __shared__ double sred[4];
     constexpr int W2 = TX + 4, W1 = TX + 2;
     const long pb = b * G.plane;
-    for (int e = threadIdx.x; e < W2 * (TY + 4); e += NTH) {
-        int ly = e / W2, lxx = e - ly * W2;
-        int gr = refl(r0 - 2 + ly, G.ns), gc = refl(c0 - 2 + lxx, G.nf);
-        long o = pb + (long)gr * G.pitch + gc;
-        double v = gcf[0] * ga.d[0][o];
+    tile_walk<2, false>(G, c0, r0, [&](int, int, int, int e, long ro, unsigned vb) VCH_WALK_FN {
+        double v = gcf[0] * *at(ga.d[0] + pb, ro, vb);
 #pragma unroll
         for (int j = 1; j < GUESS_ORD; ++j)
-            if (gcf[j] != 0.0) v += gcf[j] * ga.d[j][o];
+            if (gcf[j] != 0.0) v += gcf[j] * *at(ga.d[j] + pb, ro, vb);
         sx[e] = isfinite(v) ? v : 0.0;
-    }
+    });
     __syncthreads();
     const double *Dp = D_s + slot * slot_stride + pb;
-    for (int e = threadIdx.x; e < (TY + 2) * W1; e += NTH) {
-        int ly = e / W1, lxx = e - ly * W1;
-        int gr = refl(r0 - 1 + ly, G.ns), gc = refl(c0 - 1 + lxx, G.nf);
+    tile_walk<1, false>(G, c0, r0, [&](int, int ly, int lxx, int e, long ro, unsigned vb) VCH_WALK_FN {
         int p2 = (ly + 1) * W2 + lxx + 1;
-        stt[e] = -0.5 * P.kappa * lap_at<W2>(sx, p2, G.ax, G.ay) + Dp[(long)gr * G.pitch + gc] * sx[p2];
-    }
+        stt[e] = -0.5 * P.kappa * lap_at<W2>(sx, p2, G.ax, G.ay) + *at(Dp, ro, vb) * sx[p2];
+    });
     __syncthreads();
     const double idt = 1.0 / dt;
     double acc = 0.0;
@@ -731,10 +766,9 @@
     const long pb = b * G.plane;
     load_tile<2>(sx, x + pb, G, c0, r0);
     __syncthreads();
-    for (int e = threadIdx.x; e < (TY + 2) * W1; e += NTH) {
-        int ly = e / W1, lxx = e - ly * W1;
+    tile_walk<1, false>(G, c0, r0, [&](int, int ly, int lxx, int e, long, unsigned) VCH_WALK_FN {
         stt[e] = -lap_at<W2>(sx, (ly + 1) * W2 + lxx + 1, G.ax, G.ay);
-    }
+    });
     __syncthreads();
     double acc[2] = {0.0, 0.0};
     const double sgn = MODE == 2 ? -1.0 : 1.0;
@@ -1184,7 +1218,7 @@
                                               const double *unp1, long u_stride, double *wnew, GuessArgs ga, double *x0,
                                               EvalFin fin, PostArgs post) {
     TILE_COORDS;
-    const int S_slot = st[b].slot, S_iters = MODE == 0 ? 0 : st[b].iters;
+    const int S_slot = __builtin_amdgcn_readfirstlane(st[b].slot), S_iters = MODE == 0 ? 0 : st[b].iters;
     const double S_alpha = MODE == 0 ? 0.0 : st[b].alpha;
     if (MODE == 0) {
         if (st[b].frozen) {
@@ -1208,70 +1242,49 @@
     const bool do_guess = gcf[0] != 0.0 && (MODE == 0 || S_iters == 1);
     double rm[TY / 4], rh[TY / 4];
     double acc[5] = {0.0, 0.0, 1e300, -1e300, 0.0};
+    const unsigned ocb = (unsigned)(c0 + lx) * 8u;
+    const bool cin = c0 + lx < G.nf;
     if (MODE == 0) {
-        constexpr int N1 = (TY + 2) * W1, I1 = (N1 + NTH - 1) / NTH;
+        constexpr int I1 = TileWalk<1>::NI;
+        const double *phi_o = phi_s + src * slot_stride + pb;
         if (post.part) {
             __shared__ double s_post[2];
-            constexpr int I2 = (W2 * (TY + 4) + NTH - 1) / NTH;
-            double raw[I2];
-#pragma unroll
-            for (int i = 0; i < I2; ++i) {
-                const int e = threadIdx.x + i * NTH;
-                raw[i] = 0.0;
-                if (e < W2 * (TY + 4)) {
-                    int ly = e / W2, lxx = e - ly * W2;
-                    int gr = refl(r0 - 2 + ly, G.ns), gc = refl(c0 - 2 + lxx, G.nf);
-                    raw[i] = phi_s[src * slot_stride + pb + (long)gr * G.pitch + gc];
-                }
-            }
+            double raw[TileWalk<2>::NI];
+            tile_walk<2>(G, c0, r0, [&](int i, int, int, int, long ro, unsigned cb) VCH_WALK_FN { raw[i] = *at(phi_o, ro, cb); });
             post_sums(post.part, nblk, (int)b, s_post);
             __syncthreads();
             const PostFix pf(s_post, st[b].mass0, P.LxLy);
-#pragma unroll
-            for (int i = 0; i < I2; ++i) {
-                const int e = threadIdx.x + i * NTH;
-                if (e < W2 * (TY + 4)) sp[e] = pf.apply(raw[i]);
-            }
+            tile_walk<2>(G, c0, r0, [&](int i, int, int, int e, long, unsigned) VCH_WALK_FN { sp[e] = pf.apply(raw[i]); });
         } else {
-            load_tile<2>(sp, phi_s + src * slot_stride + pb, G, c0, r0);
+            load_tile<2>(sp, phi_o, G, c0, r0);
         }
         load_tile<1>(sm, mu_s + src * slot_stride + pb, G, c0, r0);
         double vW[I1], vU0[I1], vU1[I1];
+        {
+            const double *w_b = w + pb, *un_b = un ? un + b * u_stride : nullptr, *unp1_b = unp1 ? unp1 + b * u_stride : nullptr;
+            tile_walk<1>(G, c0, r0, [&](int i, int, int, int, long ro, unsigned cb) VCH_WALK_FN {
+                vW[i] = *at(w_b, ro, cb);
+                vU0[i] = un_b ? *at(un_b, ro, cb) : 0.0;
+                vU1[i] = unp1_b ? *at(unp1_b, ro, cb) : 0.0;
+            });
+        }
+        __syncthreads();
 #pragma unroll
-        for (int i = 0; i < I1; ++i) {
-            const int e = threadIdx.x + i * NTH;
-            vW[i] = vU0[i] = vU1[i] = 0.0;
-            if (e < N1) {
-                int ly = e / W1, lxx = e - ly * W1;
-                int gr = refl(r0 - 1 + ly, G.ns), gc = refl(c0 - 1 + lxx, G.nf);
-                long o = (long)gr * G.pitch + gc;
-                vW[i] = w[pb + o];
-                vU0[i] = un ? un[b * u_stride + o] : 0.0;
-                vU1[i] = unp1 ? unp1[b * u_stride + o] : 0.0;
-            }
-        }
-        __syncthreads();
         for (int k = 0; k < TY / 4; ++k) {
-            int ly = ly0 + 4 * k, r = r0 + ly, c = c0 + lx;
+            const int ly = ly0 + 4 * k, r = r0 + ly;
             rm[k] = 0.0;
-            if (r < G.ns && c < G.nf) {
+            if (r < G.ns && cin) {
                 int p1 = (ly + 1) * W1 + lx + 1, p2 = (ly + 2) * W2 + lx + 2;
                 const double cm = -sp[p2] / dt - 0.5 * lap_at<W1>(sm, p1, G.ax, G.ay);
-                cmu[pb + (long)r * G.pitch + c] = cm;
+                *at(cmu + pb, (long)r * G.pitch, lane_off(ocb)) = cm;
                 rm[k] = cm;
             }
         }
         __syncthreads();
         const double gdt = P.gamma / dt;
-#pragma unroll
-        for (int i = 0; i < I1; ++i) {
-            const int e = threadIdx.x + i * NTH;
-            if (e >= N1) continue;
-            int ly = e / W1, lxx = e - ly * W1;
-            int rr = r0 - 1 + ly, cc = c0 - 1 + lxx;
-            int gr = refl(rr, G.ns), gc = refl(cc, G.nf);
-            int p2 = (ly + 1) * W2 + lxx + 1;
-            long o = (long)gr * G.pitch + gc, ob = pb + o;
+        tile_walk<1>(G, c0, r0, [&](int i, int ly, int lxx, int e, long ro, unsigned cb) VCH_WALK_FN {
+            const int rr = r0 - 1 + ly, cc = c0 - 1 + lxx;
+            const int p2 = (ly + 1) * W2 + lxx + 1;
             const double u0 = vU0[i], u1 = vU1[i], wo = vW[i];
             const double wn = ((gdt - 0.5) * wo + 0.5 * (u1 + u0)) / (gdt + 0.5);
             const double ph = sp[p2], lp = lap_at<W2>(sp, p2, G.ax, G.ay);
@@ -1280,26 +1293,29 @@
             sr[e] = tdt * ph - 0.5 * P.kappa * lp + P.c1 * reglog(ph) - 0.5 * m0 + cp;
             sm[e] = m0;
             if (ly >= 1 && ly <= TY && lxx >= 1 && lxx <= TX && rr < G.ns && cc < G.nf) {
-                wnew[ob] = wn;
-                cphi[ob] = cp;
+                const unsigned ob = lane_off(cb);
+                *at(wnew + pb, ro, ob) = wn;
+                *at(cphi + pb, ro, ob) = cp;
             }
-        }
+        });
         __syncthreads();
+#pragma unroll
         for (int k = 0; k < TY / 4; ++k) {
-            int ly = ly0 + 4 * k, r = r0 + ly, c = c0 + lx;
+            const int ly = ly0 + 4 * k, r = r0 + ly;
+            const long ro = (long)r * G.pitch, dsto = dst * slot_stride + pb;
             rh[k] = 0.0;
-            if (r < G.ns && c < G.nf) {
+            if (r < G.ns && cin) {
+                const unsigned ob = lane_off(ocb);
                 int p1 = (ly + 1) * W1 + lx + 1, p2 = (ly + 2) * W2 + lx + 2;
-                long od = dst * slot_stride + pb + (long)r * G.pitch + c;
                 const double ph = sp[p2], rp = sr[p1];
                 const double rmv = ph / dt - 0.5 * lap_at<W1>(sm, p1, G.ax, G.ay) + rm[k];
                 const double rhv = -rmv + lap_at<W1>(sr, p1, G.ax, G.ay);
                 const double d = jac_diag(ph, tdt, P.c1);
-                phi_s[od] = ph;
-                if (post.part && post.hist) post.hist[b * post.hist_stride + (long)r * G.pitch + c] = ph;
-                mu_s[od] = sm[p1];
-                Rphi_s[od] = rp;
-                D_s[od] = d;
+                *at(phi_s + dsto, ro, ob) = ph;
+                *at(mu_s + dsto, ro, ob) = sm[p1];
+                *at(Rphi_s + dsto, ro, ob) = rp;
+                *at(D_s + dsto, ro, ob) = d;
+                if (post.part && post.hist) *at(post.hist + b * post.hist_stride, ro, lane_off(ocb)) = ph;
                 rh[k] = rhv;
                 acc[0] += rp * rp + rmv * rmv;
                 acc[2] = fmin(acc[2], d);
@@ -1309,65 +1325,43 @@
     } else {
         const double *phi_o = phi_s + src * slot_stride + pb, *mu_o = mu_s + src * slot_stride + pb;
         const double *D_o = D_s + src * slot_stride + pb, *R_o = Rphi_s + src * slot_stride + pb;
-        constexpr int N1 = (TY + 2) * W1, I1 = (N1 + NTH - 1) / NTH;
-        double pd[(W2 * (TY + 4) + NTH - 1) / NTH], pp[(W2 * (TY + 4) + NTH - 1) / NTH];
-        {
-            int i = 0;
-#pragma unroll
-            for (int e = threadIdx.x; e < W2 * (TY + 4); e += NTH, ++i) {
-                int ly = e / W2, lxx = e - ly * W2;
-                int gr = refl(r0 - 2 + ly, G.ns), gc = refl(c0 - 2 + lxx, G.nf);
-                long o = (long)gr * G.pitch + gc;
-                pd[i] = dphi[pb + o];
-                pp[i] = phi_o[o];
-            }
-        }
+        constexpr int I1 = TileWalk<1>::NI;
+        double pd[TileWalk<2>::NI], pp[TileWalk<2>::NI];
+        tile_walk<2>(G, c0, r0, [&](int i, int, int, int, long ro, unsigned cb) VCH_WALK_FN {
+            pd[i] = *at(dphi + pb, ro, cb);
+            pp[i] = *at(phi_o, ro, cb);
+        });
         double vD[I1], vR[I1], vM[I1], vC[I1], vcm[TY / 4];
-#pragma unroll
-        for (int i = 0; i < I1; ++i) {
-            const int e = threadIdx.x + i * NTH;
-            vD[i] = vR[i] = vM[i] = vC[i] = 0.0;
-            if (e < N1) {
-                int ly = e / W1, lxx = e - ly * W1;
-                int gr = refl(r0 - 1 + ly, G.ns), gc = refl(c0 - 1 + lxx, G.nf);
-                long o = (long)gr * G.pitch + gc;
-                vD[i] = D_o[o];
-                vR[i] = R_o[o];
-                vM[i] = mu_o[o];
-                vC[i] = cphi[pb + o];
-            }
-        }
+        tile_walk<1>(G, c0, r0, [&](int i, int, int, int, long ro, unsigned cb) VCH_WALK_FN {
+            vD[i] = *at(D_o, ro, cb);
+            vR[i] = *at(R_o, ro, cb);
+            vM[i] = *at(mu_o, ro, cb);
+            vC[i] = *at(cphi + pb, ro, cb);
+        });
 #pragma unroll
         for (int k = 0; k < TY / 4; ++k) {
-            int r = r0 + ly0 + 4 * k, c = c0 + lx;
-            vcm[k] = (r < G.ns && c < G.nf) ? cmu[pb + (long)r * G.pitch + c] : 0.0;
-        }
-        {
-            int i = 0;
-#pragma unroll
-            for (int e = threadIdx.x; e < W2 * (TY + 4); e += NTH, ++i) {
-                sd[e] = pd[i];
-                sp[e] = pp[i] + S_alpha * pd[i];
-            }
-        }
+            const int r = r0 + ly0 + 4 * k;
+            vcm[k] = 0.0;
+            if (r < G.ns && cin) vcm[k] = *at(cmu + pb, (long)r * G.pitch, lane_off(ocb));
+        }
+        tile_walk<2>(G, c0, r0, [&](int i, int, int, int e, long, unsigned) VCH_WALK_FN {
+            sd[e] = pd[i];
+            sp[e] = pp[i] + S_alpha * pd[i];
+        });
         __syncthreads();
-#pragma unroll
-        for (int i = 0; i < I1; ++i) {
-            const int e = threadIdx.x + i * NTH;
-            if (e < N1) {
-                int ly = e / W1, lxx = e - ly * W1;
-                int p2 = (ly + 1) * W2 + lxx + 1;
-                const double Dv = vD[i], Rv = vR[i], Mv = vM[i];
-                const double dm = 2.0 * ((-0.5 * P.kappa * lap_at<W2>(sd, p2, G.ax, G.ay) + Dv * sd[p2]) + Rv);
-                sm[e] = Mv + S_alpha * dm;
-            }
-        }
+        tile_walk<1>(G, c0, r0, [&](int i, int ly, int lxx, int e, long, unsigned) VCH_WALK_FN {
+            const int p2 = (ly + 1) * W2 + lxx + 1;
+            const double Dv = vD[i], Rv = vR[i], Mv = vM[i];
+            const double dm = 2.0 * ((-0.5 * P.kappa * lap_at<W2>(sd, p2, G.ax, G.ay) + Dv * sd[p2]) + Rv);
+            sm[e] = Mv + S_alpha * dm;
+        });
         __syncthreads();
         double mt[TY / 4];
+#pragma unroll
         for (int k = 0; k < TY / 4; ++k) {
-            int ly = ly0 + 4 * k, r = r0 + ly, c = c0 + lx;
+            const int ly = ly0 + 4 * k, r = r0 + ly;
             rm[k] = mt[k] = 0.0;
-            if (r < G.ns && c < G.nf) {
+            if (r < G.ns && cin) {
                 int p1 = (ly + 1) * W1 + lx + 1, p2 = (ly + 2) * W2 + lx + 2;
                 const double cm = vcm[k];
                 rm[k] = sp[p2] / dt - 0.5 * lap_at<W1>(sm, p1, G.ax, G.ay) + cm;
@@ -1375,31 +1369,28 @@
             }
         }
         __syncthreads();
+        tile_walk<1>(G, c0, r0, [&](int i, int ly, int lxx, int e, long, unsigned) VCH_WALK_FN {
+            const int p2 = (ly + 1) * W2 + lxx + 1;
+            const double cp = vC[i];
+            double ph = sp[p2];
+            sm[e] = tdt * ph - 0.5 * P.kappa * lap_at<W2>(sp, p2, G.ax, G.ay) + P.c1 * reglog(ph) - 0.5 * sm[e] + cp;
+        });
+        __syncthreads();
 #pragma unroll
-        for (int i = 0; i < I1; ++i) {
-            const int e = threadIdx.x + i * NTH;
-            if (e < N1) {
-                int ly = e / W1, lxx = e - ly * W1;
-                int p2 = (ly + 1) * W2 + lxx + 1;
-                const double cp = vC[i];
-                double ph = sp[p2];
-                sm[e] = tdt * ph - 0.5 * P.kappa * lap_at<W2>(sp, p2, G.ax, G.ay) + P.c1 * reglog(ph) - 0.5 * sm[e] + cp;
-            }
-        }
-        __syncthreads();
         for (int k = 0; k < TY / 4; ++k) {
-            int ly = ly0 + 4 * k, r = r0 + ly, c = c0 + lx;
+            const int ly = ly0 + 4 * k, r = r0 + ly;
+            const long ro = (long)r * G.pitch, dsto = dst * slot_stride + pb;
             rh[k] = 0.0;
-            if (r < G.ns && c < G.nf) {
+            if (r < G.ns && cin) {
+                const unsigned ob = lane_off(ocb);
                 int p1 = (ly + 1) * W1 + lx + 1, p2 = (ly + 2) * W2 + lx + 2;
-                long od = dst * slot_stride + pb + (long)r * G.pitch + c;
                 double ph = sp[p2], rp = sm[p1];
                 double rhv = -rm[k] + lap_at<W1>(sm, p1, G.ax, G.ay);
                 double d = jac_diag(ph, tdt, P.c1);
-                phi_s[od] = ph;
-                mu_s[od] = mt[k];
-                Rphi_s[od] = rp;
-                D_s[od] = d;
+                *at(phi_s + dsto, ro, ob) = ph;
+                *at(mu_s + dsto, ro, ob) = mt[k];
+                *at(Rphi_s + dsto, ro, ob) = rp;
+                *at(D_s + dsto, ro, ob) = d;
                 rh[k] = rhv;
                 acc[0] += rp * rp + rm[k] * rm[k];
                 acc[2] = fmin(acc[2], d);
@@ -1411,47 +1402,44 @@
         double *X = MODE == 0 ? sp : sd;
         double *STT = MODE == 0 ? sr : sp;
         __syncthreads();
-        for (int e = threadIdx.x; e < (TY + 2) * W1; e += NTH) {
-            int ly = e / W1, lxx = e - ly * W1;
+        tile_walk<1, false>(G, c0, r0, [&](int, int ly, int lxx, int e, long, unsigned) VCH_WALK_FN {
             sm[e] = jac_diag(sp[(ly + 1) * W2 + lxx + 1], tdt, P.c1);
-        }
+        });
         __syncthreads();
-        for (int e = threadIdx.x; e < W2 * (TY + 4); e += NTH) {
-            int ly = e / W2, lxx = e - ly * W2;
-            int gr = refl(r0 - 2 + ly, G.ns), gc = refl(c0 - 2 + lxx, G.nf);
-            long o = pb + (long)gr * G.pitch + gc;
-            double v = gcf[0] * ga.d[0][o];
+        tile_walk<2, false>(G, c0, r0, [&](int, int, int, int e, long ro, unsigned cb) VCH_WALK_FN {
+            double v = gcf[0] * *at(ga.d[0] + pb, ro, cb);
 #pragma unroll
             for (int j = 1; j < GUESS_ORD; ++j)
-                if (gcf[j] != 0.0) v += gcf[j] * ga.d[j][o];
+                if (gcf[j] != 0.0) v += gcf[j] * *at(ga.d[j] + pb, ro, cb);
             X[e] = isfinite(v) ? v : 0.0;
-        }
+        });
         __syncthreads();
-        for (int e = threadIdx.x; e < (TY + 2) * W1; e += NTH) {
-            int ly = e / W1, lxx = e - ly * W1;
-            int p2 = (ly + 1) * W2 + lxx + 1;
+        tile_walk<1, false>(G, c0, r0, [&](int, int ly, int lxx, int e, long, unsigned) VCH_WALK_FN {
+            const int p2 = (ly + 1) * W2 + lxx + 1;
             STT[e] = -0.5 * P.kappa * lap_at<W2>(X, p2, G.ax, G.ay) + sm[e] * X[p2];
-        }
+        });
         double xv[TY / 4];
         for (int k = 0; k < TY / 4; ++k) xv[k] = X[(ly0 + 4 * k + 2) * W2 + lx + 2];
         __syncthreads();
         const double idt = 1.0 / dt;
+#pragma unroll
         for (int k = 0; k < TY / 4; ++k) {
-            int ly = ly0 + 4 * k, r = r0 + ly, c = c0 + lx;
-            if (r < G.ns && c < G.nf) {
+            const int ly = ly0 + 4 * k, r = r0 + ly;
+            if (r < G.ns && cin) {
                 int p1 = (ly + 1) * W1 + lx + 1;
                 const double full = rh[k];
                 const double defl = full - (xv[k] * idt - lap_at<W1>(STT, p1, G.ax, G.ay));
-                x0[pb + (long)r * G.pitch + c] = xv[k];
+                *at(x0 + pb, (long)r * G.pitch, lane_off(ocb)) = xv[k];
                 acc[4] += full * full;
                 rh[k] = defl;
             }
         }
     }
-    for (int k = 0; k < TY / 4; ++k) {
-        int r = r0 + ly0 + 4 * k, c = c0 + lx;
-        if (r < G.ns && c < G.nf) {
-            rhs_s[dst * slot_stride + pb + (long)r * G.pitch + c] = rh[k];
+#pragma unroll
+    for (int k = 0; k < TY / 4; ++k) {
+        const int r = r0 + ly0 + 4 * k;
+        if (r < G.ns && cin) {
+            *at(rhs_s + dst * slot_stride + pb, (long)r * G.pitch, lane_off(ocb)) = rh[k];
             acc[1] += rh[k] * rh[k];
         }
     }
@@ -1946,12 +1934,10 @@
     }
     __syncthreads();
     const double *Dp = D_s + slot * slot_stride + pb;
-    for (int e = threadIdx.x; e < (TY + 2) * W1; e += NTH) {
-        int ly = e / W1, lxx = e - ly * W1;
-        int gr = refl(r0 - 1 + ly, G.ns), gc = refl(c0 - 1 + lxx, G.nf);
+    tile_walk<1, false>(G, c0, r0, [&](int, int ly, int lxx, int e, long ro, unsigned vb) VCH_WALK_FN {
         int p2 = (ly + 1) * W2 + lxx + 1;
-        stt[e] = -0.5 * P.kappa * lap_at<W2>(sx, p2, G.ax, G.ay) + Dp[(long)gr * G.pitch + gc] * sx[p2];
-    }
+        stt[e] = -0.5 * P.kappa * lap_at<W2>(sx, p2, G.ax, G.ay) + *at(Dp, ro, vb) * sx[p2];
+    });
     __syncthreads();
     const double idt = 1.0 / dt;
     double acc[1] = {0.0};
```
